# 101001000/ElevenRender

Hardware: AMD Instinct MI355X
Metric: Msamples/sec (rays traced x bounces) at 1920x1080, 1M-tri scene (higher is better)
Workload: dtype f32; 1 GPU; C2: 1000000-triangle random soup + 2048x1024 sky HDRI, 1920x1080, max_bounces 8, 1 step = 1 spp pass (config total 256 spp), seed 12345; schedule=stream

## Files before the change

### elevenrender_amd/abi.py

```python
import ctypes as C
import os

import numpy as np

_HERE = os.path.dirname(os.path.abspath(__file__))
LIB_PATH = os.environ.get("ELEVEN_HIP_LIB") or os.path.join(_HERE, "libeleven_hip.so")

ER_OK = 0
ER_ERR_INVALID_ARG, ER_ERR_NO_DEVICE, ER_ERR_HIP, ER_ERR_STATE, ER_ERR_OOM = -1, -2, -3, -4, -5
PASS_BEAUTY, PASS_DENOISE, PASS_NORMAL, PASS_TANGENT, PASS_BITANGENT, PASS_COUNT = 0, 1, 2, 3, 4, 5
PASS_NAMES = {"beauty": 0, "denoise": 1, "normal": 2, "tangent": 3, "bitangent": 4}
FLAG_POINT_LIGHTS, FLAG_COUNTERS, FLAG_MEGAKERNEL, FLAG_PROFILE, FLAG_FUSED, FLAG_WAVEFRONT, FLAG_GPU_BUILD, FLAG_MIS, FLAG_STREAM = 1, 2, 4, 8, 16, 32, 64, 128, 256
FLAG_HOST_BUILD = 512
FLAG_MESH_LIGHTS = 1024
MAX_BOUNCES = 65535
UPDATE_CAMERA, UPDATE_GEOMETRY = 1, 2
EDIT_CAMERA, EDIT_GEOMETRY, EDIT_MATERIALS, EDIT_TEXTURES, EDIT_HDRI = 1, 2, 4, 8, 16
REBUILD_NEVER, REBUILD_ALWAYS, REBUILD_AUTO = 0, 1, 2
TOPO_REMOVE, TOPO_APPEND = 1, 2
FEATURE_ALBEDO, FEATURE_DEPTH, FEATURE_COUNT = 0, 1, 2
FEATURE_NAMES = {"albedo": 0, "depth": 1}
ID_NONE, ID_SLOTS = 0xFFFFFFFF, 4
ID_TRIANGLE, ID_OBJECT, ID_MATERIAL, ID_KIND_COUNT = 0, 1, 2, 3
ID_KIND_NAMES = {"triangle": 0, "object": 1, "material": 2}
# ... 142 lines not shown

class ErAccelCost(C.Structure):
    _fields_ = [("node_area", C.c_double), ("leaf_area", C.c_double), ("tri_area", C.c_double), ("cost", C.c_double), ("ms", C.c_float), ("builder", C.c_uint32)]


class ErUpdatePolicy(C.Structure):
    _fields_ = [("mode", C.c_uint32), ("max_cost_ratio", C.c_float)]


class ErRebuildInfo(C.Structure):
    _fields_ = [("mode", C.c_uint32), ("max_cost_ratio", C.c_float), ("rebuilds", C.c_uint32), ("last_decision", C.c_uint32), ("cost_built", C.c_double),
                ("cost_refit", C.c_double), ("cost_after", C.c_double), ("cost_ms", C.c_float), ("rebuild_ms", C.c_float)]


class ErCostSumsDebug(C.Structure):
    _fields_ = [("node_area", C.c_double), ("leaf_area", C.c_double), ("tri_area", C.c_double), ("cost", C.c_double), ("ms", C.c_float), ("reserved", C.c_uint32)]


class ErTexEntry(C.Structure):
    _fields_ = [("width", C.c_int32), ("height", C.c_int32), ("channels", C.c_int32), ("filter", C.c_int32), ("offset", C.c_uint32)]


class ErTexturePlan(C.Structure):
    _fields_ = [("texture_count", C.c_uint32), ("fused_count", C.c_uint32), ("fused_any", C.c_uint32), ("reserved", C.c_uint32), ("hdri", ErTexEntry),
                ("pool_floats", C.c_uint64)]


class ErTextureDump(C.Structure):
    _fields_ = [("texture_count", C.c_uint32), ("material_count", C.c_uint32), ("fused_count", C.c_uint32), ("cdf_count", C.c_uint32), ("guide_count", C.c_uint32),
                ("tex_pow2", C.c_uint32), ("fused_any", C.c_uint32), ("hdri_buckets", C.c_int32), ("hdri_radiance_sum", C.c_float), ("hdri_tex", ErTexEntry),
                ("pool_floats", C.c_uint64)]


TEX_DTYPE = np.dtype([("width", "<i4"), ("height", "<i4"), ("channels", "<i4"), ("filter", "<i4"), ("offset", "<u4")])
FUSED_DTYPE = np.dtype([("width", "<i4"), ("height", "<i4"), ("filter", "<i4"), ("offset", "<u4")])
assert TEX_DTYPE.itemsize == 20 and FUSED_DTYPE.itemsize == 16


class ErFeatureInfo(C.Structure):
    _fields_ = [("valid", C.c_uint32), ("samples", C.c_uint32), ("rays", C.c_uint64), ("ms", C.c_float)]


class ErDenoiseGuided(C.Structure):
    _fields_ = [("levels", C.c_uint32), ("colour_sigma", C.c_float), ("albedo_sigma", C.c_float), ("depth_sigma", C.c_float)]


class ErIdInfo(C.Structure):
    _fields_ = [("valid", C.c_uint32), ("samples", C.c_uint32), ("rays", C.c_uint64), ("ms", C.c_float), ("objects", C.c_uint32),
                ("overflow_pixels", C.c_uint32 * ID_KIND_COUNT)]


class ErHistoryParams(C.Structure):
    _fields_ = [("depth_tolerance", C.c_float), ("max_weight", C.c_float)]


class ErHistoryInfo(C.Structure):
    _fields_ = [("captured", C.c_uint32), ("resolved", C.c_uint32), ("moved_objects", C.c_uint32), ("pixels_valid", C.c_uint64), ("pixels_partial", C.c_uint64),
                ("pixels_offscreen", C.c_uint64), ("pixels_rejected", C.c_uint64), ("pixels_sky", C.c_uint64), ("capture_ms", C.c_float), ("resolve_ms", C.c_float)]


class ErVarianceInfo(C.Structure):
    _fields_ = [("folds", C.c_uint32), ("reserved", C.c_uint32), ("pixels_folded", C.c_uint64), ("pixels_known", C.c_uint64), ("fold_ms", C.c_float),
                ("filter_ms", C.c_float)]


class ErDenoiseVariance(C.Structure):
    _fields_ = [("levels", C.c_uint32), ("colour_sigma", C.c_float), ("albedo_sigma", C.c_float), ("depth_sigma", C.c_float)]


class ErHistoryVarianceInfo(C.Structure):
    _fields_ = [("captured", C.c_uint32), ("resolved", C.c_uint32), ("pixels_known_captured", C.c_uint64), ("pixels_known_history", C.c_uint64),
                ("pixels_known_blended", C.c_uint64), ("filter_ms", C.c_float)]


class ErPick(C.Structure):
    _fields_ = [("hit", C.c_uint32), ("triangle", C.c_uint32), ("object", C.c_uint32), ("material", C.c_uint32), ("distance", C.c_float),
                ("position", C.c_float * 3), ("uv", C.c_float * 2)]


class ErStreamInfo(C.Structure):
    _fields_ = [("waves", C.c_uint32), ("tracers", C.c_uint32), ("large_regions", C.c_uint32), ("deal_pending", C.c_uint32), ("launches", C.c_uint32),
                ("pixels_per_cu", C.c_uint32), ("lanes_busy", C.c_double), ("launch_ms", C.c_double), ("cost_spread", C.c_double),
                ("spec_started", C.c_uint64), ("spec_right", C.c_uint64), ("spec_wrong", C.c_uint64),
                ("form", C.c_uint32), ("reserved", C.c_uint32)]


class ErStreamBalance(C.Structure):
    _fields_ = [("blocks", C.c_uint32), ("most", C.c_uint32), ("levelled", C.c_uint32), ("counting", C.c_uint32), ("cost_tiles", C.c_uint32), ("cap", C.c_uint32),
                ("launch_ticks", C.c_uint64)]


class ErStreamForm(C.Structure):
    _fields_ = [("waves", C.c_uint32), ("tracers", C.c_uint32), ("adapt", C.c_uint32), ("keep", C.c_uint32), ("spec", C.c_uint32), ("reserved", C.c_uint32)]


class ErAccelDump(C.Structure):
    _fields_ = [("tri_count", C.c_uint32), ("node_count", C.c_uint32), ("node8_count", C.c_uint32), ("node8_pieces", C.c_uint32),
                ("attr_pieces", C.c_uint32), ("max_depth", C.c_uint32), ("max_depth8", C.c_uint32), ("builder", C.c_uint32),
                ("lo", C.c_float * 3), ("hi", C.c_float * 3), ("lift_bound", C.c_float), ("max_lift", C.c_float)]


NODE_DTYPE = np.dtype([("lo0", "<f4", 3), ("hi0", "<f4", 3), ("lo1", "<f4", 3), ("hi1", "<f4", 3), ("c0", "<i4"), ("c1", "<i4"), ("pad", "<i4", 2)])
NODE8_DTYPE = np.dtype([("p", "<f4", 3), ("e", "u1", 3), ("imask", "u1"), ("child_base", "<u4"), ("tri_base", "<u4"), ("tri_present", "<u4"),
                        ("reserved", "<u4"), ("qlo", "u1", (3, 8)), ("qhi", "u1", (3, 8))])
ISECT_DTYPE = np.dtype([("v0", "<f4", 3), ("tri_id", "<i4"), ("v1", "<f4", 3), ("lift", "<f4"), ("v2", "<f4", 3), ("sign", "<f4")])
assert NODE_DTYPE.itemsize == 64 and NODE8_DTYPE.itemsize == 80 and ISECT_DTYPE.itemsize == 48


def attr_dtype(pieces):
    dt = np.dtype([("n", "<f4", (3, 3)), ("t", "<f4", (3, 3)), ("uv", "<f4", (3, 2)), ("material", "<i4"), ("pad", "<u4", 4 * pieces - 25)])
    assert dt.itemsize == 16 * pieces
    return dt


def accel_dump_dict(info, **arrays):
    d = {n: int(getattr(info, n)) for n in ("tri_count", "node_count", "node8_count", "max_depth", "max_depth8", "builder")}
    d["lo"], d["hi"] = np.array(list(info.lo), np.float32), np.array(list(info.hi), np.float32)
    d["lift_bound"], d["max_lift"] = np.float32(info.lift_bound), np.float32(info.max_lift)
    d.update(arrays)
    return d


def debug_bvh_dump(vertices, normals, threads=0):
    lib = load()
    v = np.ascontiguousarray(vertices, np.float32).reshape(-1, 3, 3)
    nn = np.ascontiguousarray(normals, np.float32).reshape(-1, 3, 3)
    assert v.shape == nn.shape
    n = len(v)
    info = ErAccelDump()
    args = (_fptr(v), _fptr(nn), n, threads, C.byref(info))
    check(lib.er_debug_bvh_dump(*args, None, 0, None, 0, None, 0, None, 0))
    assert info.node8_pieces * 16 == NODE8_DTYPE.itemsize
    nodes, nodes8 = np.zeros(info.node_count, NODE_DTYPE), np.zeros(info.node8_count, NODE8_DTYPE)
    s2t, lift = np.zeros(n, np.uint32), np.zeros(n, np.float32)
    vp = lambda a: a.ctypes.data_as(C.c_void_p)
    check(lib.er_debug_bvh_dump(*args, vp(nodes), nodes.nbytes, vp(nodes8), nodes8.nbytes, s2t.ctypes.data_as(C.POINTER(C.c_uint32)), s2t.nbytes,
                                _fptr(lift), lift.nbytes))
    return accel_dump_dict(info, nodes=nodes, nodes8=nodes8, slot_to_tri=s2t, tri_lift=lift)


def debug_spill_levels(spilled, n, usable):
    buf = np.ascontiguousarray(spilled, np.uint32)
    levels = np.zeros(n, np.uint32)
    check(load().er_debug_spill_levels(buf.ctypes.data_as(C.c_void_p), buf.nbytes, n, usable, levels.ctypes.data_as(C.POINTER(C.c_uint32))))
    return levels


def debug_transform_apply(m, vertices, normals, tangents):
    lib = load()
    mm = np.ascontiguousarray(m, np.float32).reshape(12)
    v, n, t = (np.ascontiguousarray(a, np.float32).reshape(-1, 3, 3) for a in (vertices, normals, tangents))
    assert v.shape == n.shape == t.shape
    out = [np.empty_like(v) for _ in range(3)]
    check(lib.er_debug_transform_apply(_fptr(mm), len(v), _fptr(v), _fptr(n), _fptr(t), *(_fptr(o) for o in out)))
    return tuple(out)


def debug_id_rank(ids):
    lib = load()
    a = np.ascontiguousarray(ids, np.uint32).reshape(-1)
    oi, oc, distinct = np.zeros(ID_SLOTS, np.uint32), np.zeros(ID_SLOTS, np.uint32), C.c_uint32()
    up = lambda x: x.ctypes.data_as(C.POINTER(C.c_uint32))
    check(lib.er_debug_id_rank(up(a) if a.size else None, a.size, up(oi), up(oc), C.byref(distinct)))
    return oi, oc, distinct.value


def debug_history_camera(camera):
# ... 461 lines not shown
```

### elevenrender_amd/csrc/er_api.cpp

```cpp
#include <algorithm>
#include <chrono>

#include "er_api_stages.h"
#include <thread>
#include <system_error>

using namespace erh;

int er_abi_version(void) { return ER_ABI_VERSION; }
const char* er_last_error(void) { return g_err.c_str(); }

int er_device_count(void) {
    int n = 0;
    if (hipGetDeviceCount(&n) != hipSuccess) return 0;
    return n;
}

static int er_device_info_impl(int index, ErDeviceInfo* out) {
    if (!out) return fail(ER_ERR_INVALID_ARG, "er_device_info: out is NULL");
    int n = er_device_count();
    if (index < 0 || index >= n) return fail(ER_ERR_NO_DEVICE, "er_device_info: no such HIP device");
    hipDeviceProp_t p;
    HIP_TRY(hipGetDeviceProperties(&p, index));
    memset(out, 0, sizeof(*out));
// ... 369 lines not shown

static int begin_planes(ErScene* s, BeginStaging& B) {
    int rc;
    const size_t npx = (size_t)s->x_res * s->y_res;
    if ((rc = upload(s->d_passes, nullptr, npx * ER_PASS_COUNT, s->stream)) != ER_OK) return rc;
    if ((rc = upload(s->d_samples, nullptr, npx, s->stream)) != ER_OK) return rc;
    if ((rc = upload(s->d_rng, nullptr, npx, s->stream)) != ER_OK) return rc;
    B.owned = s->tiles_of(s->params.rank, s->params.world);
    if ((rc = upload(s->d_owned, B.owned.data(), B.owned.size(), s->stream)) != ER_OK) return rc;
    if ((rc = upload(s->d_counters, nullptr, 1, s->stream)) != ER_OK) return rc;
    HIP_TRY(hipMemsetAsync(s->d_counters.p, 0, sizeof(DevCounters), s->stream));
    return ER_OK;
}

static int begin_choose_schedule(ErScene* s, BeginStaging& B, uint32_t cus) {
    const uint32_t all = ER_FLAG_MEGAKERNEL | ER_FLAG_FUSED | ER_FLAG_WAVEFRONT | ER_FLAG_STREAM;
    uint32_t forced = s->params.flags & all;
    if (forced == ER_FLAG_FUSED) forced = ER_FLAG_STREAM;
    if (forced & (forced - 1)) return fail(ER_ERR_INVALID_ARG, "er_render_begin: more than one schedule flag");
    uint32_t sched = forced;
    if (forced == 0 || forced == ER_FLAG_STREAM) B.deal = stream_deal_owned(B.owned, s->tiles_x(), cus);
    if (forced == 0) {
        sched = ((size_t)B.deal.most * 64u > ER_STREAM_MAX_RING || s->x_res > 65535u || s->y_res > 65535u) ? ER_FLAG_WAVEFRONT : ER_FLAG_STREAM;
    }
    s->params.flags = (s->params.flags & ~all) | sched;
    return ER_OK;
}

static int begin_wavefront(ErScene* s, const std::vector<uint32_t>& owned, uint32_t cus, bool query_on) {
    int rc;
    uint32_t pools = 3;
    if (const char* e = getenv("ER_WF_POOLS")) pools = (uint32_t)std::min(8, std::max(1, atoi(e)));
    pools = std::min<uint32_t>(pools, std::max<uint32_t>(1u, (uint32_t)owned.size()));
    const size_t pool_tiles = (owned.size() + pools - 1) / pools;
    const size_t qcap = pool_tiles * 64;
    size_t slots = owned.size() * 64;
    const size_t sh = query_on ? 2 : 1;
    const size_t qs_cap = qcap * sh;
    const size_t q_words = 2 * qcap + 2 * qs_cap;
    if ((rc = upload(s->d_wf4, nullptr, slots * (7 + 4 * sh), s->stream)) != ER_OK) return rc;
    if ((rc = upload(s->d_wf1, nullptr, slots * (3 + 3 * sh) + q_words * pools + (size_t)WF_COUNTS * pools, s->stream)) != ER_OK) return rc;
    WfState W{};
    float4* f = s->d_wf4.p;
    W.ray_o = f; W.ray_d = f + slots; W.light = f + 2 * slots; W.reduc = f + 3 * slots;
    W.aov_n = f + 4 * slots; W.aov_t = f + 5 * slots; W.aov_b = f + 6 * slots;
    W.sh_o = f + 7 * slots; W.sh_d = W.sh_o + sh * slots; W.c_vis = W.sh_d + sh * slots; W.c_occ = W.c_vis + sh * slots;
    uint32_t* u = s->d_wf1.p;
    W.hit = (int*)u; W.left = u + slots; W.hit2 = (int*)(u + 2 * slots);
    W.occluded = (int*)(u + 3 * slots); W.occ_a = W.occluded + sh * slots; W.occ_b = W.occ_a + sh * slots;
    uint32_t* qbase = u + (3 + 3 * sh) * slots;
    uint32_t* cbase = qbase + q_words * pools;
    W.pools = pools;
    W.slots = (uint32_t)slots;
    s->trace_blocks = cus * 12;
    s->shade_blocks = cus * 5;
    if (const char* e = getenv("ER_TRACE_WAVES_PER_CU")) s->trace_blocks = cus * (uint32_t)std::max(1, atoi(e));
    if (const char* e = getenv("ER_SHADE_WAVES_PER_CU")) s->shade_blocks = cus * (uint32_t)std::max(1, atoi(e));
    const size_t trace_spill = (size_t)s->trace_blocks * ER_STACK8 * 64;
    const size_t spill_per_pool = trace_spill + (size_t)s->shade_blocks * ER_BVH_MAX_DEPTH * 32;
    if ((rc = upload(s->d_spill, nullptr, spill_per_pool * pools, s->stream)) != ER_OK) return rc;
    s->wf.clear();
    for (uint32_t p2 = 0; p2 < pools; p2++) {
        W.pool = p2;
        uint32_t* q = qbase + (size_t)p2 * q_words;
        W.q[0] = q; W.q[1] = q + qcap; W.qs[0] = q + 2 * qcap; W.qs[1] = q + 2 * qcap + qs_cap;
        W.counts = cbase + (size_t)p2 * WF_COUNTS;
        W.spill = s->d_spill.p + (size_t)p2 * spill_per_pool;
        W.shade_stack = (int*)(W.spill + trace_spill);
        s->wf.push_back(W);
    }
    for (uint32_t p2 = 1; p2 < pools; p2++) {
        hipStream_t st;
        HIP_TRY(hipStreamCreateWithFlags(&st, hipStreamNonBlocking));
        s->pool_streams.push_back(st);
    }
    for (uint32_t p2 = 0; p2 < pools; p2++) {
        hipEvent_t e;
        HIP_TRY(hipEventCreateWithFlags(&e, hipEventDisableTiming));
        s->pool_events.push_back(e);
    }
    return ER_OK;
}

static int begin_descriptor(ErScene* s, uint32_t owned_tiles) {
    const ErGpuBvhDevice& g = s->kept.accel;
    const float lift_bound = g.lift_bound;
    float scene_scale = 0;
    for (int a = 0; a < 3; a++) scene_scale = std::max(scene_scale, std::max(std::fabs(g.lo[a]), std::fabs(g.hi[a])));
    scene_scale = std::max(scene_scale, std::max(std::fabs(s->camera.position.x), std::max(std::fabs(s->camera.position.y), std::fabs(s->camera.position.z))));

    DevScene& D = s->dev;
    memset(&D, 0, sizeof(D));
    D.nodes = s->d_nodes.p;
    D.nodes8 = s->d_nodes8.p;
    D.tri_isect = s->d_nodes8.p + g.n8_pieces;
    D.tri_base_pieces = (uint32_t)g.n8_pieces;
    D.tri_attr = s->d_attr.p;
    D.tri_count = s->tri_count;
    D.node_count = (uint32_t)(g.nodes_f4 / 4);
    D.node8_count = g.nodes8_count;
    D.prune_margin = lift_bound + 1e-5f * scene_scale;
    D.max_lift = lift_bound;
    D.scene_scale = scene_scale;
    D.materials = s->d_materials.p;
    D.mat_pre = s->d_mat_pre.p;
    D.textures = s->d_textures.p;
    D.tex_pool = s->d_tex_pool.p;
    D.mat_fused = s->d_mat_fused.p;
    D.fused_any = s->fused_any ? 1u : 0u;
    D.hdri_tex = s->kept.hdri;
    D.hdri_cdf = s->d_cdf.p;
    D.hdri_guide = s->d_guide.p;
    D.hdri_buckets = s->kept.buckets;
    D.hdri_radiance_sum = s->hdri_radiance_sum;
    D.hdri_trig = getenv("ER_HDRI_TRIG_ON_DEVICE") ? nullptr : s->d_guide.p + s->kept.trig_at;
    D.cam = s->camera;
    D.x_res = s->x_res;
    D.y_res = s->y_res;
    D.tiles_x = s->tiles_x();
    D.tiles_y = s->tiles_y();
    D.max_bounces = s->params.max_bounces;
    {
        auto pow2 = [](int32_t v) { return v > 0 && (v & (v - 1)) == 0; };
        bool all = pow2(s->kept.hdri.width) && pow2(s->kept.hdri.height);
        for (const HostTex& t : s->textures) all = all && pow2(t.width) && pow2(t.height);
        D.tex_pow2 = all ? 1u : 0u;
        if (const char* e = getenv("ER_TEX_POW2")) D.tex_pow2 = (atoi(e) != 0 && all) ? 1u : 0u;
    }
    D.trace_every_query = 0u;
    if (const char* e = getenv("ER_TRACE_EVERY_QUERY")) D.trace_every_query = atoi(e) != 0 ? 1u : 0u;
    D.ext_flags = s->params.flags & (ER_FLAG_POINT_LIGHTS | ER_FLAG_MIS);
    D.lights = s->d_lights.p;
    D.light_count = (uint32_t)s->point_lights.size();
    if (s->light_emitters > 0) {
        D.ext_flags = (D.ext_flags & ~(uint32_t)ER_FLAG_POINT_LIGHTS) | ER_FLAG_MESH_LIGHTS;
        D.mesh_lights = s->d_light_tab.p;
        D.emitter_count = s->light_emitters;
    }
    D.passes = s->d_passes.p;
    D.samples = s->d_samples.p;
    D.rng = s->d_rng.p;
    D.owned_tiles = s->d_owned.p;
    D.owned_tile_count = owned_tiles;
    D.counters = s->d_counters.p;
    D.tile_cost = ((s->params.flags & ER_FLAG_STREAM) && s->st.counting) ? s->st.d_tile_cost.p : nullptr;
    D.px_draws = (s->params.flags & ER_FLAG_STREAM) ? s->st.d_px_draws.p : nullptr;
    {
        const erd::CamTrig t = erd::camera_trig(D.cam);
        D.cam_cx = t.cx; D.cam_sx = t.sx; D.cam_cy = t.cy; D.cam_sy = t.sy; D.cam_cz = t.cz; D.cam_sz = t.sz;
        D.cam_trig_valid = getenv("ER_CAM_TRIG_ON_DEVICE") ? 0u : 1u;
    }
    return upload(s->d_dev, &D, 1, s->stream);
}

int begin_render_state(ErScene* s, BeginStaging& B, hipEvent_t uploads_done) {
    int rc;
    const uint32_t cus = s->kept.cus;
    const bool query_on = s->query_on();
    if ((rc = begin_planes(s, B)) != ER_OK) return rc;
    if ((rc = begin_choose_schedule(s, B, cus)) != ER_OK) return rc;
    if (s->params.flags & ER_FLAG_STREAM) rc = stream_begin(s, B.owned, B.deal, cus, query_on);
    else if (s->params.flags & ER_FLAG_WAVEFRONT) rc = begin_wavefront(s, B.owned, cus, query_on);
    if (rc != ER_OK) return rc;
    if (uploads_done) HIP_TRY(hipEventRecord(uploads_done, s->stream));
    if ((rc = begin_descriptor(s, (uint32_t)B.owned.size())) != ER_OK) return rc;

    er_launch_setup(s->dev, s->stream);
    HIP_TRY(hipGetLastError());
    HIP_TRY(hipStreamSynchronize(s->stream));
    return ER_OK;
}

}

static int er_render_begin_impl(ErScene* s, const ErRenderParams* p) {
    if (!s || !p) return fail(ER_ERR_INVALID_ARG, "er_render_begin: NULL argument");
    std::lock_guard<std::mutex> lk(s->mtx);
    int rc;
    ErDeviceInfo info;
    if ((rc = begin_check(p, info)) != ER_OK) return rc;
    if ((rc = begin_open(s, p)) != ER_OK) return rc;
    const char* who = "er_render_begin";
    s->kept.cus = std::max(1u, info.compute_units);
    s->kept.flags = p->flags;
    EventPair ev;
    HIP_TRY(hipEventCreate(&ev.a));
    HIP_TRY(hipEventCreate(&ev.b));
    BeginStaging B;
    if ((rc = begin_accel(s, B, ev.a, who)) != ER_OK) return rc;
    if ((rc = begin_materials(s, B)) != ER_OK) return rc;
    if ((rc = begin_textures(s, B, who)) != ER_OK) return rc;
    if ((rc = begin_emitters(s, B, who)) != ER_OK) return rc;
    if ((rc = begin_render_state(s, B, ev.b)) != ER_OK) return rc;
    float up_ms = 0;
    (void)hipEventElapsedTime(&up_ms, ev.a, ev.b);

    accel_publish(s, up_ms);
    s->begun = true;
    return ER_OK;
}

static int wavefront_enqueue(ErScene* s, const DevScene& D, uint32_t n, bool count) {
    const uint64_t iters64 = (uint64_t)n * ((uint64_t)s->params.max_bounces + 1u);
    if (iters64 > 0xFFFFFFFFull)
        return fail(ER_ERR_INVALID_ARG, "er_render_samples: " + std::to_string(n) + " samples of " + std::to_string(s->params.max_bounces) +
                                            " bounces are more than 4294967295 iterations of the wavefront schedule in one call");
    const uint32_t iters = (uint32_t)iters64;
    const uint32_t pools = (uint32_t)s->wf.size();
    const bool prof = (s->params.flags & ER_FLAG_PROFILE) != 0;
    if (prof) {
        const size_t need = s->prof_used / 3 + (size_t)iters * pools;
        while (s->prof_events.size() < 3 * need) {
            hipEvent_t e;
            HIP_TRY(hipEventCreate(&e));
            s->prof_events.push_back(e);
        }
        if (s->d_ray_log.n < need) {
            DevBuf<uint32_t> bigger;
            int rc2 = upload(bigger, nullptr, need * 2, s->stream);
            if (rc2 != ER_OK) return rc2;
            if (s->d_ray_log.p && s->prof_used) {
                HIP_TRY(hipStreamSynchronize(s->stream));
                HIP_TRY(hipMemcpy(bigger.p, s->d_ray_log.p, (s->prof_used / 3) * sizeof(uint32_t), hipMemcpyDeviceToDevice));
            }
            s->d_ray_log.release();
            s->d_ray_log = bigger;
        }
    }
    if (pools > 1) {
        HIP_TRY(hipEventRecord(s->pool_events[0], s->stream));
        for (uint32_t p = 1; p < pools; p++) HIP_TRY(hipStreamWaitEvent(s->pool_streams[p - 1], s->pool_events[0], 0));
    }
    auto pool_stream = [&](uint32_t p) { return p == 0 ? s->stream : s->pool_streams[p - 1]; };
    for (uint32_t p = 0; p < pools; p++) er_launch_wf_begin(D, s->wf[p], n, pool_stream(p));
    for (uint32_t it = 0; it < iters; it++) {
        for (uint32_t p = 0; p < pools; p++) {
            hipStream_t st = pool_stream(p);
            uint32_t* ray_log = prof ? s->d_ray_log.p + s->prof_used / 3 : nullptr;
            if (prof) HIP_TRY(hipEventRecord(s->prof_events[s->prof_used++], st));
            er_launch_wf_trace(D, s->wf[p], it & 1, count, s->trace_blocks, ray_log, st);
            if (prof) HIP_TRY(hipEventRecord(s->prof_events[s->prof_used++], st));
            er_launch_wf_shade(D, s->wf[p], it & 1, count, s->shade_blocks, st);
            if (prof) HIP_TRY(hipEventRecord(s->prof_events[s->prof_used++], st));
        }
    }
    for (uint32_t p = 1; p < pools; p++) {
        HIP_TRY(hipEventRecord(s->pool_events[p], s->pool_streams[p - 1]));
        HIP_TRY(hipStreamWaitEvent(s->stream, s->pool_events[p], 0));
    }
    return ER_OK;
}

static int enqueue_samples(ErScene* s, uint32_t n) {
    const DevScene& D = s->ad_on ? s->ad_dev : s->dev;
    const bool count = (s->params.flags & ER_FLAG_COUNTERS) != 0;
    int rc = ER_OK;
    if (!(s->params.flags & (ER_FLAG_MEGAKERNEL | ER_FLAG_STREAM))) {
        if (n > 0) rc = wavefront_enqueue(s, D, n, count);
    } else {
        const bool prof = (s->params.flags & ER_FLAG_PROFILE) && n > 0;
        if (prof) {
            while (s->prof_events.size() < s->prof_used + 3) {
                hipEvent_t e;
                HIP_TRY(hipEventCreate(&e));
                s->prof_events.push_back(e);
            }
            HIP_TRY(hipEventRecord(s->prof_events[s->prof_used++], s->stream));
// ... 481 lines not shown
```

### elevenrender_amd/csrc/er_api_edit.cpp

```cpp
#include <algorithm>
#include <chrono>

#include "er_api_stages.h"
#include "er_topology_host.h"

using namespace erh;

static_assert(ER_TOPO_REMOVE == ER_TOPO_HOST_REMOVE && ER_TOPO_APPEND == ER_TOPO_HOST_APPEND, "er_topology_host.h restates the two bits");

static_assert(ER_EDIT_CAMERA == ER_UPDATE_CAMERA && ER_EDIT_GEOMETRY == ER_UPDATE_GEOMETRY, "an ErSceneUpdate's bits are the first two of an ErSceneEdit");

namespace {

const uint32_t LOOK_BITS = ER_EDIT_MATERIALS | ER_EDIT_TEXTURES | ER_EDIT_HDRI;

struct XformList {
    uint32_t count = 0;
    const ErObjectTransform* x = nullptr;
    std::vector<ErXformEntry> entries;
    uint32_t moved = 0;
};


int edit_refit(ErScene* s, bool new_normals, bool new_tangents, const ErSparseList* sp, const XformList* xf, const char* who) {
// ... 284 lines not shown
                continue;
            }
            if ((rc = check_tex(t, "scene texture")) != ER_OK) return rc;
        }
    }
    const ErMaterial* mats = s->materials.data();
    size_t nmat = s->materials.size();
    bool ids_differ = false;
    if (what & ER_EDIT_MATERIALS) {
        if (e->material_count == 0 || !e->materials) return fail(ER_ERR_INVALID_ARG, pre + "ER_EDIT_MATERIALS needs at least one material");
        mats = e->materials;
        nmat = e->material_count;
        if ((rc = check_texture_ids(mats, nmat, ntex, who)) != ER_OK) return rc;
        if (tc) rc = topo_check_material_ids(s, e->material_id, true, *tc, nmat, who);
        else rc = check_material_ids(e->material_id ? e->material_id : s->material_id.data(), n, nmat, who);
        if (rc != ER_OK) return rc;
        ids_differ = nmat != s->materials.size();
        for (size_t m = 0; m < nmat && !ids_differ; m++) {
            int32_t a[7], b[7];
            texture_ids(mats[m], a);
            texture_ids(s->materials[m], b);
            ids_differ = memcmp(a, b, sizeof(a)) != 0;
        }
    }
    if (tc && !(what & ER_EDIT_MATERIALS) && (rc = topo_check_material_ids(s, nullptr, false, *tc, nmat, who)) != ER_OK) return rc;
    if ((what & ER_EDIT_HDRI) && (rc = check_tex(e->hdri.texture, "hdri")) != ER_OK) return rc;
    W.rebuild_pool = (what & ER_EDIT_TEXTURES) != 0 || ids_differ;
    {
        const TexDecl hd = (what & ER_EDIT_HDRI) ? TexDecl{e->hdri.texture.width, e->hdri.texture.height, e->hdri.texture.channels, e->hdri.texture.filter}
                                                 : TexDecl{s->hdri_tex.width, s->hdri_tex.height, s->hdri_tex.channels, s->hdri_tex.filter};
        uint64_t pool_floats = 0;
        if (W.rebuild_pool) {
            std::vector<TexDecl> decl(ntex);
            for (size_t i = 0; i < ntex; i++) {
                const bool keep = !(what & ER_EDIT_TEXTURES) || !e->textures[i].data;
                decl[i] = keep ? TexDecl{s->textures[i].width, s->textures[i].height, s->textures[i].channels, s->textures[i].filter}
                               : TexDecl{e->textures[i].width, e->textures[i].height, e->textures[i].channels, e->textures[i].filter};
            }
            TexPlan P;
            er_texture_plan(decl.data(), ntex, mats, nmat, hd, P);
            pool_floats = P.pool_floats;
        } else if (what & ER_EDIT_HDRI) {
            pool_floats = (uint64_t)s->kept.hdri.offset + (uint64_t)hd.width * (uint64_t)hd.height * (uint64_t)hd.channels;
        }
        if ((rc = check_pool_floats(pool_floats, who)) != ER_OK) return rc;
    }
    if (what & ER_EDIT_MATERIALS) W.materials.assign(e->materials, e->materials + e->material_count);
    if (what & ER_EDIT_TEXTURES) {
        W.textures.resize(ntex);
        W.kept.assign(ntex, 0);
        for (size_t i = 0; i < ntex; i++) {
            if (!e->textures[i].data) { W.kept[i] = 1; continue; }
            if ((rc = copy_tex(e->textures[i], W.textures[i], "scene texture")) != ER_OK) return rc;
        }
    }
    if (what & ER_EDIT_HDRI) {
        if ((rc = copy_tex(e->hdri.texture, W.hdri, "hdri")) != ER_OK) return rc;
        if (e->hdri.cdf) {
            W.cdf.assign(e->hdri.cdf, e->hdri.cdf + (size_t)W.hdri.width * W.hdri.height + 1);
            W.radiance_sum = e->hdri.radiance_sum;
        } else {
            host_generate_cdf(W.hdri, W.cdf, W.radiance_sum);
        }
    }
    return ER_OK;
}

void edit_replace(ErScene* s, const ErSceneEdit* e, const ErSparseList* sp, const XformList* xf, EditWork& W) noexcept {
    const uint32_t what = e->what;
    const size_t n = s->tri_count, n9 = n * 9;
    if (what & ER_EDIT_CAMERA) s->camera = e->camera;
    if ((what & ER_EDIT_GEOMETRY) && sp) {
        s->flush_poses();
        er_sparse_patch(*sp, s->vertices.data(), s->normals.data(), s->tangents.data());
    } else if ((what & ER_EDIT_GEOMETRY) && xf) {
        er_objects_mark(s->objects, xf->entries.data(), (uint32_t)xf->entries.size());
    } else if (what & ER_EDIT_GEOMETRY) {
        if (e->normals && e->tangents) s->objects.forget_pending();
        else s->flush_poses();
        std::copy(e->vertices, e->vertices + n9, s->vertices.begin());
        if (e->normals) std::copy(e->normals, e->normals + n9, s->normals.begin());
        if (e->tangents) std::copy(e->tangents, e->tangents + n9, s->tangents.begin());
    }
    if (what & ER_EDIT_MATERIALS) {
        s->materials.swap(W.materials);
        if (e->material_id) std::copy(e->material_id, e->material_id + n, s->material_id.begin());
    }
    if (what & ER_EDIT_TEXTURES) {
        for (size_t i = 0; i < W.textures.size(); i++)
            if (W.kept[i]) std::swap(W.textures[i], s->textures[i]);
        s->textures.swap(W.textures);
    }
    if (what & ER_EDIT_HDRI) {
        std::swap(s->hdri_tex, W.hdri);
        s->hdri_cdf.swap(W.cdf);
        s->hdri_radiance_sum = W.radiance_sum;
    }
}

int edit_locked(ErScene* s, const ErSceneEdit* e, const ErSparseList* sp, XformList* xf, uint32_t known, const char* who, std::chrono::steady_clock::time_point t0) {
    int rc;
    EditWork W;
    if ((rc = edit_check(s, e, sp, xf, known, who, W)) != ER_OK) return rc;
    HIP_TRY(hipSetDevice(s->device));
    HIP_TRY(hipStreamSynchronize(s->stream));
    edit_replace(s, e, sp, xf, W);
    if ((e->what & ER_EDIT_GEOMETRY) || ((e->what & ER_EDIT_MATERIALS) && e->material_id)) s->store.release();
    s->feat.valid = false;
    for (auto& set : s->unpacked_feat) set.clear();
    s->ids_invalidate();
    if (((e->what & ER_EDIT_GEOMETRY) && !xf) || (e->what & LOOK_BITS)) s->history_invalidate();
    s->variance_reset();
    uint32_t stage = 0;
    float stage_ms = 0;
    const bool sparse_geometry = sp && (e->what & ER_EDIT_GEOMETRY);
    if (sparse_geometry) {
        const uint32_t calls = s->sparse.calls;
        s->sparse = ErSparseInfo{};
        s->sparse.calls = calls;
    }
    const bool xform_geometry = xf && (e->what & ER_EDIT_GEOMETRY);
    if (xform_geometry) {
        const uint32_t calls = s->xform.calls;
        s->xform = ErSparseInfo{};
        s->xform.calls = calls;
    }
    if ((rc = edit_device(s, e, sp, xf, W.rebuild_pool, who, stage, stage_ms)) != ER_OK) {
        s->begun = false;
        return rc;
    }
    s->upd.updates++;
    if (sparse_geometry) {
        s->sparse.calls++;
        s->sparse.moved = sp->count;
        if (s->accel.builder != 2u) s->sparse.path = 3u;
    }
    if (xform_geometry) {
        s->xform.calls++;
        s->xform.moved = xf->moved;
        s->xform_objects = xf->count;
        if (s->accel.builder != 2u) s->xform.path = 3u;
    }
    if ((e->what & ER_EDIT_GEOMETRY) && s->accel.builder == 2u) s->upd.refits++;
    const float wall_ms = std::chrono::duration<float, std::milli>(std::chrono::steady_clock::now() - t0).count();
    if (e->what & LOOK_BITS) {
        s->edit.edits++;
        s->edit.texture_stage = stage;
        s->edit.texture_stage_ms = stage_ms;
        s->edit.pool_floats = s->d_tex_pool.n;
        s->edit.edit_ms = wall_ms;
    } else {
        s->upd.update_ms = wall_ms;
    }
    return ER_OK;
}

}

static int er_render_update_impl(ErScene* s, const ErSceneUpdate* u) {
    if (!s || !u) return fail(ER_ERR_INVALID_ARG, "er_render_update: NULL argument");
    const auto t0 = std::chrono::steady_clock::now();
    std::lock_guard<std::mutex> lk(s->mtx);
    if (!s->begun) return fail(ER_ERR_STATE, "er_render_update: er_render_begin has not succeeded");
    ErSceneEdit e{};
    e.what = u->what; e.camera = u->camera; e.vertices = u->vertices; e.normals = u->normals; e.tangents = u->tangents;
    return edit_locked(s, &e, nullptr, nullptr, ER_UPDATE_CAMERA | ER_UPDATE_GEOMETRY, "er_render_update", t0);
// ... 263 lines not shown
```

### elevenrender_amd/csrc/er_bounce.inc

```
#ifndef ER_BOUNCE_FUSE
#define ER_BOUNCE_FUSE true
#endif
#ifndef ER_BOUNCE_SKIP_EQUAL
#define ER_BOUNCE_SKIP_EQUAL true
#endif
#ifndef ER_BOUNCE_KEEP_LAST
#define ER_BOUNCE_KEEP_LAST false
#endif
{
    const bool er_skip_equal = (ER_BOUNCE_SKIP_EQUAL) && S.trace_every_query == 0u;
    const int hw = S.hdri_tex.width, hh = S.hdri_tex.height;
    const bool er_mis = EXT && (S.ext_flags & ER_FLAG_MIS) != 0;
#ifdef ER_BOUNCE_MESH
    constexpr bool er_mesh = EXT && (ER_BOUNCE_MESH);
#else
    constexpr bool er_mesh = false;
#endif
    if (hslot < 0) {
        float u, v;
        spherical_mapping(-1 * ray.d, u, v);
        if (EXT) {
            F3 er_env = tex_filtered(S, S.hdri_tex, u, v);
            if (er_mis && prev_pdf >= 0.0f) {
                const int er_mx = ermath::f2i(u * hw), er_my = ermath::f2i(v * hh);
                const float er_ms = (S.hdri_trig != nullptr && (unsigned)er_my < (unsigned)hh) ? hdri_trig_rows(S)[er_my].sin_row : hdri_pdf_sine(S.hdri_tex, er_my);
                const float er_ph = hdri_pdf_of(S, tex_coords(S, S.hdri_tex, er_mx, er_my), er_ms);
                er_env = er_env * (1.0f / (1.0f + er_ph / prev_pdf));
                if (COUNT) c_texels++;
            }
            light = light + reduction * er_env;
        } else {
            light = light + reduction * tex_filtered(S, S.hdri_tex, u, v);
        }
        if (COUNT) c_texels++;
        done = true;
    } else {
        c_shaded++;
        ER_TP(2);
        HitFull hit;
        full_hit(S, (uint32_t)hslot, ray, hit);
        const ErMaterial& mat = S.materials[hit.material];
        HitData hd;
        generate_hit_data<COUNT, ER_BOUNCE_FUSE>(S, mat, hit, hd, c_texels);
        int shader = mat.albedo_shader_id;
        if (shader != -1) {
            hd.albedo = f3s(0);
            if (shader >= 0 && shader < 4) hd.albedo = f3(1, 1, 0);
        }
        if (rng_next(rs) <= hd.opacity) {
            F3 wo = ray.d * -1.0f;
            F3 N = hd.normal;
            c_hdri++;
            ER_TP(3);
            int count = er_cdf_search(S.hdri_cdf, hw * hh, S.hdri_guide, S.hdri_buckets, rng_next(rs));
            const bool hw_pow2 = (hw & (hw - 1)) == 0 && hw > 0 && count >= 0;
            const int er_cx = hw_pow2 ? (int)((unsigned)count & (unsigned)(hw - 1)) : count % hw;
            const int er_cy = hw_pow2 ? (int)((unsigned)count >> (31 - __builtin_clz((unsigned)hw))) : count / hw;
            float tcx = (float)er_cx, tcy = (float)er_cy;
            float d1 = rng_next(rs), d2 = rng_next(rs), d3 = rng_next(rs);
            const bool er_lights = EXT && !er_mesh && (S.ext_flags & ER_FLAG_POINT_LIGHTS) != 0 && S.light_count > 0;
            float er_rl = 0.0f;
            if (er_lights) er_rl = rng_next(rs);
            float er_mp = 0.0f, er_mu1 = 0.0f, er_mu2 = 0.0f;
            if (er_mesh) { er_mp = rng_next(rs); er_mu1 = rng_next(rs); er_mu2 = rng_next(rs); }
            ER_TP(4);
            const bool er_last = !(ER_BOUNCE_KEEP_LAST) && bounce + 1u >= S.max_bounces;
            F3 wibrdf = f3s(0);
            if (!er_last) wibrdf = DisneySample(hd, wo, N, d1, d2, d3);
            float er_px, er_pz, er_py, er_a, er_sin;
            int er_ix, er_iy;
            if (S.hdri_trig != nullptr && (unsigned)count < (unsigned)(hw * hh)) {
                const HdriCol er_c = hdri_trig_cols(S)[er_cx];
                const HdriRow er_r = hdri_trig_rows(S)[er_cy];
                er_px = er_c.px; er_pz = er_c.pz; er_ix = er_c.ix;
                er_py = er_r.py; er_a = er_r.a; er_iy = er_r.iy; er_sin = er_r.sin_pdf;
            } else {
                float nu = tcx / (float)hw, nv = tcy / (float)hh;
                float iu, iv;
                inverse_transform_uv(S.hdri_tex, nu, nv, iu, iv);
                rsm_column(iu, er_px, er_pz);
                rsm_row(iv, er_py, er_a);
                er_ix = ermath::f2i(iu * hw); er_iy = ermath::f2i(iv * hh);
                er_sin = hdri_pdf_sine(S.hdri_tex, er_iy);
            }
            F3 wihdri = normalized(f3(er_a * er_px, er_py, er_a * er_pz)) * -1.0f;
            F3 hdriValue = tex_coords(S, S.hdri_tex, er_ix, er_iy);
            if (COUNT) c_texels += 2;
            F3 evalh = DisneyEval(hd, wo, N, wihdri);
            float hdripdf = hdri_pdf_of(S, hdriValue, er_sin);
            float absdot = __builtin_fabsf(dot(wihdri, N));
            float er_wnee = 1.0f;
            if (er_mis) er_wnee = 1.0f / (1.0f + DisneyPdf(hd, wo, N, wihdri) / hdripdf);
            F3 er_em = hd.emission;
            if (er_mesh && prev_pdf >= 0.0f && mesh_d >= 0.0f) {
                const float er_ph = mesh_prob(S)[hslot];
                if (er_ph > 0.0f) {
                    F3 er_a, er_b, er_c, er_ng;
                    float er_area;
                    mesh_tri(S, (uint32_t)hslot, er_a, er_b, er_c, er_ng, er_area);
                    const float er_dh = mesh_d + length(hit.position - ray.o);
                    const float er_pl = er_ph * (er_dh * er_dh) / (er_area * __builtin_fabsf(dot(er_ng, ray.d)));
                    er_em = er_em * (1.0f / (1.0f + er_pl / prev_pdf));
                }
            }
            F3 c_vis = er_mis ? reduction * (er_em + (hdriValue * evalh * absdot / hdripdf) * er_wnee)
                              : reduction * (er_em + hdriValue * evalh * absdot / hdripdf);
            const F3 c_occ = er_mis ? reduction * (er_em + (f3s(0) * evalh * absdot / hdripdf) * er_wnee)
                                    : reduction * (er_em + f3s(0) * evalh * absdot / hdripdf);
            if ((evalh.x != 0.0f || evalh.y != 0.0f || evalh.z != 0.0f) && !(er_skip_equal && same_bits(c_vis, c_occ))) {
                Ray sr = make_ray(hd.position + N * 0.001f, wihdri);
                F3 v0, v1, v2;
                float4 qa, qb, qc4;
                load_verts(S, (uint32_t)hslot, v0, v1, v2, qa, qb, qc4);
                float su, sv, st, d_self = __builtin_inff();
                if (tri_mt(v0, v1, v2, sr, su, sv, st)) d_self = candidate_distance(S, (uint32_t)hslot, v0, v1, v2, sr, su, sv, st);
                ER_BOUNCE_HDRI_QUERY(sr, hslot, d_self, c_vis, c_occ);
                pending = true;
            } else {
                light = light + c_vis;
            }
            if (er_lights) {
                int er_k = ermath::f2i((float)S.light_count * er_rl);
                er_k = er_k > (int)S.light_count - 1 ? (int)S.light_count - 1 : er_k;
                const ErPointLight er_L = S.lights[er_k];
                const F3 er_lpos = f3(er_L.position.x, er_L.position.y, er_L.position.z);
                const F3 er_toL = er_lpos - hd.position;
                const F3 er_dir = normalized(er_toL);
                const float er_dist = length(er_toL);
                const Ray er_lr = make_ray(hd.position + er_dir * 0.001f, er_dir);
                const float er_limit = length(er_lpos - er_lr.o);
                const F3 er_value = f3(er_L.radiance.x, er_L.radiance.y, er_L.radiance.z) / (er_dist * er_dist);
                const F3 er_evall = DisneyEval(hd, wo, N, er_dir);
                const float er_lpdf = ((float)S.light_count) / (2.0f * PIF);
                if (er_evall.x != 0.0f || er_evall.y != 0.0f || er_evall.z != 0.0f) {
                    const F3 er_pl = er_value * er_evall * __builtin_fabsf(dot(er_dir, N)) / er_lpdf;
                    const F3 er_lv = reduction * er_pl, er_lo = reduction * f3s(0);
                    if (er_skip_equal && !pending && same_bits(er_lv, er_lo)) {
                        light = light + er_lv;
                    } else {
                        ER_BOUNCE_LIGHT_QUERY(er_lr, -1, er_limit, er_lv, er_lo);
                        lpending = true;
                    }
                }
            }
            if (er_mesh && bounce + 1u < S.max_bounces) {
                const uint32_t er_k = mesh_slot(S, mesh_pick(S, er_mp));
                if ((int)er_k != hslot) {
                    F3 er_a, er_b, er_c, er_ng;
                    float er_area;
                    mesh_tri(S, er_k, er_a, er_b, er_c, er_ng, er_area);
                    const float er_su = __builtin_sqrtf(er_mu1);
                    const float er_b1 = er_su * (1.0f - er_mu2), er_b2 = er_su * er_mu2;
                    const F3 er_p = er_a * (1.0f - er_su) + er_b * er_b1 + er_c * er_b2;
                    const F3 er_toL = er_p - hd.position;
                    const F3 er_dir = normalized(er_toL);
                    const float er_dist = length(er_toL);
                    const float er_cosl = dot(er_ng, er_dir);
                    const F3 er_evall = er_cosl != 0.0f ? DisneyEval(hd, wo, N, er_dir) : f3s(0);
                    if (er_evall.x != 0.0f || er_evall.y != 0.0f || er_evall.z != 0.0f) {
                        const float4* er_q = S.tri_attr + (size_t)er_k * ER_ATTR_PIECES;
                        const float4 er_q4 = er_q[4], er_q5 = er_q[5];
                        const ErMaterial& er_m = S.materials[__builtin_bit_cast(int, er_q[6].x)];
                        const float er_tu = er_q4.z + (er_q5.x - er_q4.z) * er_b1 + (er_q5.z - er_q4.z) * er_b2;
                        const float er_tv = er_q4.w + (er_q5.y - er_q4.w) * er_b1 + (er_q5.w - er_q4.w) * er_b2;
                        F3 er_le = er_m.emission_tex < 0 ? f3(er_m.emission.x, er_m.emission.y, er_m.emission.z)
                                                         : tex_filtered(S, S.textures[er_m.emission_tex], er_tu, er_tv);
                        const float er_op = er_m.opacity_tex < 0 ? er_m.opacity : tex_filtered(S, S.textures[er_m.opacity_tex], er_tu, er_tv).x;
                        er_le = er_le * clampf(er_op, 0.0f, 1.0f);
                        if (COUNT) c_texels += (er_m.emission_tex < 0 ? 0 : 1) + (er_m.opacity_tex < 0 ? 0 : 1);
                        const float er_lpdf = mesh_prob(S)[er_k] * (er_dist * er_dist) / (er_area * __builtin_fabsf(er_cosl));
                        const float er_wl = 1.0f / (1.0f + DisneyPdf(hd, wo, N, er_dir) / er_lpdf);
                        const F3 er_ml = er_le * er_evall * __builtin_fabsf(dot(er_dir, N)) / er_lpdf * er_wl;
                        const F3 er_lv = reduction * er_ml, er_lo = reduction * f3s(0);
                        if (er_skip_equal && !pending && same_bits(er_lv, er_lo)) {
                            light = light + er_lv;
                        } else {
                            const Ray er_lr = make_ray(hd.position + er_dir * 0.001f, er_dir);
                            ER_BOUNCE_LIGHT_QUERY(er_lr, (int)er_k, length(er_p - er_lr.o), er_lv, er_lo);
                            lpending = true;
                        }
                    }
                }
            }
            ER_TP(5);
            if (!er_last) {
                float brdfpdf = DisneyPdf(hd, wo, N, wibrdf);
                reduction = reduction * (DisneyEval(hd, wo, N, wibrdf) * __builtin_fabsf(dot(wibrdf, N)) / brdfpdf);
                if (er_mis || er_mesh) prev_pdf = brdfpdf;
                ray = make_ray(hit.position + wibrdf * 0.001f, wibrdf);
            }
            if (bounce == 0) { ER_BOUNCE_FIRST_HIT(hd.normal, hd.tangent, hd.bitangent); }
            if (er_mesh) mesh_d = 0.001f;
        } else {
            if (er_mesh) mesh_d = -1.0f;
            ray = make_ray(hit.position + ray.d * 0.001f, ray.d);
        }
        ER_TP(6);
        bounce++;
        if (bounce >= S.max_bounces) done = true;
    }
}
```

### elevenrender_amd/csrc/er_debug.hip

```cpp
#include "er_debug.h"

#include "er_device.h"
#include "er_shade.h"
#include "er_trav.h"

using namespace erd;

__global__ __launch_bounds__(64) void er_debug_trace_kernel(DevScene S, const float* __restrict__ o, const float* __restrict__ d, uint32_t n,
                                                             const int32_t* __restrict__ self, const float* __restrict__ limit,
                                                             int32_t* __restrict__ tri_out, int32_t* __restrict__ slot_out, float* __restrict__ pos_out,
                                                             float* __restrict__ dist_out, int32_t* __restrict__ info_out, uint2* spill_base) {
    __shared__ uint2 s_stack[WF_LDS_STACK * 64];
    __shared__ int s_stack2[ER_STACK * 64];
    const uint32_t i = blockIdx.x * 64 + threadIdx.x;
    if (i >= n) return;
    uint2* stack = s_stack + threadIdx.x;
    uint2* spill = spill_base + (size_t)blockIdx.x * (ER_STACK8 * 64) + threadIdx.x;
    int* stack2 = s_stack2 + threadIdx.x;
    Ray ray;
    ray.o = f3(o[3 * i], o[3 * i + 1], o[3 * i + 2]);
    ray.d = f3(d[3 * i], d[3 * i + 1], d[3 * i + 2]);
    unsigned cn = 0, ct = 0;
    int info = 0;
    if (self) {
// ... 9 lines not shown
        pos_out[3 * i] = pos_out[3 * i + 1] = pos_out[3 * i + 2] = 0.0f;
        dist_out[i] = __builtin_inff();
        if (slot >= 0) {
            HitFull h;
            full_hit(S, (uint32_t)slot, ray, h);
            tri_out[i] = __builtin_bit_cast(int, S.tri_isect[(size_t)slot * 3].w);
            pos_out[3 * i] = h.position.x; pos_out[3 * i + 1] = h.position.y; pos_out[3 * i + 2] = h.position.z;
            dist_out[i] = length(h.position - ray.o);
        }
    }
    info_out[i] = info;
}

void er_launch_debug_trace(const DevScene& S, const float* o, const float* d, uint32_t n, const int32_t* self, const float* limit, int32_t* tri,
                           int32_t* slot, float* pos, float* dist, int32_t* info, void* spill, hipStream_t stream) {
    if (n == 0) return;
    hipLaunchKernelGGL(er_debug_trace_kernel, dim3((n + 63) / 64), dim3(64), 0, stream, S, o, d, n, self, limit, tri, slot, pos, dist, info, (uint2*)spill);
}
uint32_t er_debug_lds_stack_levels() { return WF_LDS_STACK; }

template <bool EXT, bool MESH>
__global__ __launch_bounds__(64) void er_debug_pixel_kernel(DevScene S, uint32_t idx, ErTraceRec* recs, int max_recs, int* count, uint2* spill) {
    __shared__ uint2 sh_stack[WF_LDS_STACK * 64];
    uint2* s_stack = sh_stack;
    int* s_stack2 = (int*)(spill + (size_t)ER_STACK8 * 64);
    static_assert((size_t)ER_STACK8 * 64 + ((size_t)ER_STACK * 64 * sizeof(int) + sizeof(uint2) - 1) / sizeof(uint2) <= (size_t)ER_DEBUG_PIXEL_SCRATCH,
                  "er_debug_trace_pixel's scratch must hold the spill levels and the exact routine's int stack");
    if (threadIdx.x != 0) return;
    int nrec = 0;
    unsigned c_rays = 0, c_nodes = 0, c_tris = 0, c_shaded = 0, c_texels = 0, c_hdri = 0;
    uint32_t rs = S.rng[idx];
    const uint32_t px = idx % S.x_res, py = idx / S.x_res;
    float c1 = rng_next(rs), c2 = rng_next(rs), c3 = rng_next(rs), c4 = rng_next(rs), c5 = rng_next(rs);
    Ray ray = camera_ray(S.cam, (int)px, (int)py, S.x_res, S.y_res, c1, c2, c3, c4, c5);
    F3 light = f3s(0), reduction = f3s(1), aov_n = f3s(0), aov_t = f3s(0), aov_b = f3s(0);
    uint32_t bounce = 0;
    float prev_pdf = -1.0f;
    float mesh_d = 0.0f;
    while (true) {
        int info;
        c_rays++;
        const int hslot = trav_run_closest<false>(S, s_stack, spill, s_stack2, ray, __builtin_inff(), info, c_nodes, c_tris);
        ErTraceRec* rec = nrec < max_recs ? &recs[nrec++] : nullptr;
        if (rec) {
            rec->bounce = (int32_t)bounce;
            rec->tri = hslot < 0 ? -1 : __builtin_bit_cast(int, S.tri_isect[(size_t)hslot * 3].w);
            rec->shadow_tri = -1; rec->opaque = 0; rec->shadow_occ = -1; rec->light_occ = -1;
            for (int k = 0; k < 3; k++) { rec->position[k] = 0; rec->wi[k] = 0; }
            if (hslot >= 0) {
                HitFull h;
                full_hit(S, (uint32_t)hslot, ray, h);
                rec->position[0] = h.position.x; rec->position[1] = h.position.y; rec->position[2] = h.position.z;
            }
        }
        constexpr bool COUNT = false;
        const Ray traced = ray;
        const uint32_t rs_before = rs;
        bool done = false, pending = false, lpending = false;
#define ER_BOUNCE_HDRI_QUERY(sr, self_slot, d_self, cv, co)                                                                          \
    {                                                                                                                                 \
        int info_;                                                                                                                    \
        c_rays++;                                                                                                                     \
        const bool occ_ = trav_run_shadow<false>(S, s_stack, spill, s_stack2, (sr), (self_slot), (d_self), info_, c_nodes, c_tris);   \
        light = light + (occ_ ? (co) : (cv));                                                                                         \
        if (rec) {                                                                                                                    \
            rec->shadow_occ = occ_ ? 1 : 0;                                                                                           \
                                      \
            const int cs_ = trav_run_closest<false>(S, s_stack, spill, s_stack2, (sr), __builtin_inff(), info_, c_nodes, c_tris);     \
            rec->shadow_tri = cs_ < 0 ? -1 : __builtin_bit_cast(int, S.tri_isect[(size_t)cs_ * 3].w);                                 \
        }                                                                                                                             \
    }
#define ER_BOUNCE_LIGHT_QUERY(lr, self_slot, limit, lv, lo)                                                                          \
    {                                                                                                                                 \
        int info_;                                                                                                                    \
        c_rays++;                                                                                                                     \
        const bool occ_ = trav_run_shadow<false>(S, s_stack, spill, s_stack2, (lr), (self_slot), (limit), info_, c_nodes, c_tris);    \
        light = light + (occ_ ? (lo) : (lv));                                                                                         \
        if (rec) rec->light_occ = occ_ ? 1 : 0;                                                                                       \
    }
#define ER_BOUNCE_FIRST_HIT(n, t, b) aov_n = (n); aov_t = (t); aov_b = (b)
#define ER_BOUNCE_MESH MESH
#define ER_BOUNCE_SKIP_EQUAL false
#define ER_BOUNCE_KEEP_LAST true
#include "er_bounce.inc"
#undef ER_BOUNCE_HDRI_QUERY
#undef ER_BOUNCE_LIGHT_QUERY
#undef ER_BOUNCE_FIRST_HIT
#undef ER_BOUNCE_MESH
#undef ER_BOUNCE_SKIP_EQUAL
#undef ER_BOUNCE_KEEP_LAST
        (void)pending; (void)lpending; (void)traced;
        if (rec) {
            uint32_t r1 = rs_before;
            (void)rng_next(r1);
            rec->opaque = (hslot >= 0 && rs != r1) ? 1 : 0;
            if (hslot >= 0) { rec->wi[0] = ray.d.x; rec->wi[1] = ray.d.y; rec->wi[2] = ray.d.z; }
            rec->light[0] = light.x; rec->light[1] = light.y; rec->light[2] = light.z;
            rec->reduction[0] = reduction.x; rec->reduction[1] = reduction.y; rec->reduction[2] = reduction.z;
        }
        if (done) break;
    }
    const uint32_t sa = S.samples[idx];
    const uint32_t sa2 = accumulate_sample(S, idx, sa, light, aov_n, aov_t, aov_b);
    if (sa2 != sa) S.samples[idx] = sa2;
    S.rng[idx] = rs;
    *count = nrec;
    atomicAdd(&S.counters->paths, 1ull);
    atomicAdd(&S.counters->bounce_samples, (unsigned long long)(bounce + (bounce < S.max_bounces ? 1u : 0u)));
    atomicAdd(&S.counters->rays, (unsigned long long)c_rays);
    atomicAdd(&S.counters->shaded_hits, (unsigned long long)c_shaded);
    atomicAdd(&S.counters->hdri_samples, (unsigned long long)c_hdri);
}

void er_launch_debug_pixel(const DevScene& S, uint32_t idx, ErTraceRec* recs, int max_recs, int* count, void* spill, hipStream_t stream) {
    auto k = er_mesh_active(S) ? er_debug_pixel_kernel<true, true> : er_ext_active(S) ? er_debug_pixel_kernel<true, false> : er_debug_pixel_kernel<false, false>;
    hipLaunchKernelGGL(k, dim3(1), dim3(64), 0, stream, S, idx, recs, max_recs, count, (uint2*)spill);
}

namespace {
ERD HitData hd_from(const float* h) {
    HitData d;
    d.metallic = h[0]; d.roughness = h[1]; d.clearcoatGloss = h[2]; d.clearcoat = h[3]; d.anisotropic = h[4];
    d.transmission = h[5]; d.specular = h[6]; d.specularTint = h[7]; d.sheenTint = h[8]; d.subsurface = h[9];
    d.sheen = h[10]; d.opacity = 1.0f;
    d.albedo = f3(h[11], h[12], h[13]); d.tangent = f3(h[14], h[15], h[16]); d.bitangent = f3(h[17], h[18], h[19]);
    d.emission = f3s(0); d.position = f3s(0); d.normal = f3s(0);
    d.gtr1_log = __builtin_nanf("");
    return d;
}
}

__global__ __launch_bounds__(64) void er_debug_eval_kernel(DevScene S, int kind, const float* __restrict__ in, uint32_t n, uint32_t in_stride,
                                                           float* __restrict__ out, uint32_t out_stride) {
    const uint32_t i = blockIdx.x * 64 + threadIdx.x;
    if (i >= n) return;
    const float* a = in + (size_t)i * in_stride;
    float* o = out + (size_t)i * out_stride;
    auto bits = [](float f) { return __builtin_bit_cast(int, f); };
    auto fbits = [](uint32_t u) { return __builtin_bit_cast(float, u); };
    switch (kind) {
        case ER_FN_RNG: {
            uint32_t st = jenkins_u32((uint32_t)bits(a[0]) + 1u);
            for (int k = 0; k < 16; k++) { o[k] = rng_next(st); o[16 + k] = fbits(st); }
            break;
        }
        case ER_FN_CAMERA_RAY: {
            const Ray r = camera_ray(S.cam, (int)a[0], (int)a[1], S.x_res, S.y_res, a[2], a[3], a[4], a[5], a[6]);
            o[0] = r.o.x; o[1] = r.o.y; o[2] = r.o.z; o[3] = r.d.x; o[4] = r.d.y; o[5] = r.d.z;
            break;
        }
        case ER_FN_TRI_HIT: {
            const int id = bits(a[0]);
            int slot = -1;
            for (uint32_t s = 0; s < S.tri_count; s++)
                if (__builtin_bit_cast(int, S.tri_isect[(size_t)s * 3].w) == id) { slot = (int)s; break; }
            Ray ray;
            ray.o = f3(a[1], a[2], a[3]);
            ray.d = f3(a[4], a[5], a[6]);
            for (int k = 0; k < 18; k++) o[k] = 0.0f;
            if (slot < 0) break;
            F3 v0, v1, v2;
            float4 qa, qb, qc;
            load_verts(S, (uint32_t)slot, v0, v1, v2, qa, qb, qc);
            float u, v, t;
            if (!tri_mt(v0, v1, v2, ray, u, v, t)) break;
            HitFull h;
            full_hit(S, (uint32_t)slot, ray, h);
            o[0] = 1.0f;
            const F3 vs[5] = {h.position, h.normal, h.gnormal, h.tangent, h.bitangent};
            for (int k = 0; k < 5; k++) { o[1 + 3 * k] = vs[k].x; o[2 + 3 * k] = vs[k].y; o[3 + 3 * k] = vs[k].z; }
            o[16] = h.tu; o[17] = h.tv;
            break;
        }
// ... 88 lines not shown
```

### elevenrender_amd/csrc/er_device.h

```cpp
#pragma once
#include <hip/hip_runtime.h>
#include <stdint.h>

#include "../../include/eleven_hip.h"
#include "er_bvh.h"
#include "er_cdf.h"
#include "er_math.h"

#ifdef ER_ISA_MARKS
#define ER_MARK(name) asm volatile("; ER_MARK " name ::: "memory")
#else
#define ER_MARK(name) ((void)0)
#endif

#ifndef ER_TP
#define ER_TP(n) ((void)0)
#endif

#define ER_TILE 8
#define ER_STACK ER_BVH_MAX_DEPTH

struct DevTex {
    int32_t width, height, channels, filter;
    uint32_t offset;
};

struct DevFused {
    int32_t width, height, filter;
    uint32_t offset;
};

struct DevCounters {
    unsigned long long paths, bounce_samples, rays, node_visits, tri_tests, shaded_hits, texel_fetches, hdri_samples;
    unsigned long long trace_wave_steps, trace_busy_lanes, trace_node_lanes, trace_tri_lanes;
};

struct DevScene {
    const float4* nodes;
    const float4* nodes8;
    const float4* tri_isect;
    const float4* tri_attr;
    uint32_t tri_count, node_count;
    uint32_t node8_count;
    uint32_t tri_base_pieces;
    float prune_margin;
    float max_lift, scene_scale;
    const ErMaterial* materials;
    const float4* mat_pre;
    const DevTex* textures;
    const DevFused* mat_fused;
    uint32_t fused_any;
    const float* tex_pool;
    DevTex hdri_tex;
    const float* hdri_cdf;
    const uint32_t* hdri_guide;
    int32_t hdri_buckets;
    float hdri_radiance_sum;
    ErCamera cam;
    uint32_t x_res, y_res, tiles_x, tiles_y;
    uint32_t max_bounces;
    uint32_t tex_pow2;
    float cam_cx, cam_sx, cam_cy, cam_sy, cam_cz, cam_sz;
    uint32_t cam_trig_valid;
    uint32_t trace_every_query;
    uint32_t ext_flags;
    union { const ErPointLight* lights; const float* mesh_lights; };
    union { uint32_t light_count; uint32_t emitter_count; };
    float4* passes;
    uint32_t* samples;
    uint32_t* rng;
    const uint32_t* owned_tiles;
    uint32_t owned_tile_count;
    DevCounters* counters;
    uint32_t* tile_cost;
    uint32_t* px_draws;
    const uint32_t* hdri_trig;
};

__host__ __device__ __forceinline__ size_t er_pass_index(size_t npx, int pass, size_t idx) {
    return pass == ER_PASS_DENOISE ? 4 * npx + idx : idx * 4 + (size_t)(pass == ER_PASS_BEAUTY ? 0 : pass - 1);
}


namespace erd {

#define ERD __device__ __forceinline__

const float PIF = 3.14159265358979323846f;

struct F3 { float x, y, z; };
ERD F3 f3(float x, float y, float z) { F3 r; r.x = x; r.y = y; r.z = z; return r; }
ERD F3 f3s(float s) { return f3(s, s, s); }
ERD F3 operator+(F3 a, F3 b) { return f3(a.x + b.x, a.y + b.y, a.z + b.z); }
ERD F3 operator-(F3 a, F3 b) { return f3(a.x - b.x, a.y - b.y, a.z - b.z); }
ERD F3 operator*(F3 a, float s) { return f3(a.x * s, a.y * s, a.z * s); }
ERD F3 operator*(float s, F3 a) { return f3(a.x * s, a.y * s, a.z * s); }
ERD F3 operator/(F3 a, float s) { return f3(a.x / s, a.y / s, a.z / s); }
ERD F3 operator*(F3 a, F3 b) { return f3(b.x * a.x, b.y * a.y, b.z * a.z); }
ERD bool same_bits(F3 a, F3 b) {
    return ((__builtin_bit_cast(uint32_t, a.x) ^ __builtin_bit_cast(uint32_t, b.x)) | (__builtin_bit_cast(uint32_t, a.y) ^ __builtin_bit_cast(uint32_t, b.y)) |
            (__builtin_bit_cast(uint32_t, a.z) ^ __builtin_bit_cast(uint32_t, b.z))) == 0u;
}
ERD F3 addf(F3 a, float s) { return f3(a.x + s, a.y + s, a.z + s); }
ERD float dot(F3 a, F3 b) { return a.x * b.x + a.y * b.y + a.z * b.z; }
ERD F3 cross(F3 a, F3 b) {
    return f3((a.y * b.z - a.z * b.y), -(a.x * b.z - a.z * b.x), (a.x * b.y - a.y * b.x));
}
ERD float length(F3 a) { return __builtin_sqrtf(a.x * a.x + a.y * a.y + a.z * a.z); }
ERD F3 normalized(F3 a) {
    float l = length(a);
    if (l == 0) return a;
    return a / l;
}
ERD float clampf(float a, float b, float c) { return a < b ? b : a > c ? c : a; }
ERD float lerpf(float a, float b, float c) { return a + c * (b - a); }
ERD F3 lerpv(F3 a, F3 b, float c) { return f3(lerpf(a.x, b.x, c), lerpf(a.y, b.y, c), lerpf(a.z, b.z, c)); }
ERD float minf(float a, float b) { return a < b ? a : b; }
ERD float maxf(float a, float b) { return a > b ? a : b; }
__host__ __device__ __forceinline__ void limitUV(float& u, float& v) {
    u += (float)(-(int)(u > 1) + -(int)(u < 0));
    v += (float)(-(int)(v > 1) + -(int)(v < 0));
}

struct Ray { F3 o, d; };
ERD Ray make_ray(F3 o, F3 d) {
    Ray r;
    r.o = o;
    float l = length(d);
    if (l != 0) { d.x /= l; d.y /= l; d.z /= l; }
    r.d = d;
    return r;
}

ERD uint32_t jenkins_u32(uint32_t seed) {
    uint32_t hash = 0;
#pragma unroll
    for (int i = 0; i < 4; i++) {
        hash += (seed >> (i * 8)) & 0xFF;
        hash += (hash << 10);
        hash ^= (hash >> 6);
    }
    hash += (hash << 3);
    hash ^= (hash >> 11);
    hash += (hash << 15);
    return hash;
}
ERD float rng_next(uint32_t& state) {
    state ^= state << 13;
    state ^= state >> 17;
    state ^= state << 5;
    return (float)state / 4294967296.0f;
}

struct CamTrig { float cx, sx, cy, sy, cz, sz; };
__host__ __device__ inline CamTrig camera_trig(const ErCamera& cam) {
    using namespace ermath;
    const float k = 3.14159265358979323846f / 180.0f;
    const float rx = cam.rotation.x * k, ry = cam.rotation.y * k, rz = cam.rotation.z * k;
    CamTrig t;
// ... 526 lines not shown
```

### elevenrender_amd/csrc/er_scene.h

```cpp
#pragma once
#include <hip/hip_runtime.h>

#include <atomic>
#include <cmath>
#include <cstdio>
#include <cstdlib>
#include <cstring>
#include <map>
#include <set>
#include <memory>
#include <mutex>
#include <new>
#include <string>
#include <vector>

#include "../../include/eleven_hip.h"
#include "er_bvh.h"
#include "er_devbuf.h"
#include "er_device.h"
#include "er_gpu_build.h"
#include "er_kernels.h"
#include "er_wavefront.h"
#include "er_stream.h"
#include "er_stream_host.h"
// ... 30 lines not shown
    } catch (...) {
        return fail(ER_ERR_STATE, std::string(who) + ": unknown exception");
    }
}

inline std::atomic<uint64_t> g_host_alloc_limit{0};
inline void host_reserve(uint64_t bytes) {
    const uint64_t lim = g_host_alloc_limit.load();
    if (lim && bytes > lim) throw std::bad_alloc();
}

struct EventPair {
    hipEvent_t a = nullptr, b = nullptr;
    ~EventPair() {
        if (a) (void)hipEventDestroy(a);
        if (b) (void)hipEventDestroy(b);
    }
};

#define HIP_TRY(expr)                                                                                   \
    do {                                                                                                \
        hipError_t e__ = (expr);                                                                        \
        if (e__ != hipSuccess)                                                                          \
            return fail(e__ == hipErrorOutOfMemory ? ER_ERR_OOM : ER_ERR_HIP,                           \
                        std::string(#expr) + ": " + hipGetErrorString(e__));                            \
    } while (0)

struct HostTex {
    int32_t width, height, channels, filter;
    std::vector<float> data;
};

inline void host_tex_coords(const HostTex& t, int x, int y, float out[3]) {
    x %= t.width;
    y %= t.height;
    if (x < 0) x *= -1;
    if (y < 0) y *= -1;
    out[0] = out[1] = out[2] = 0.0f;
    const float* d = t.data.data();
    if (t.channels == 1) {
        out[0] = out[1] = out[2] = d[y * t.width + x];
    } else if (t.channels == 2) {
        out[0] = d[t.channels * (y * t.width + x) + 0];
        out[1] = d[t.channels * (y * t.width + x) + 1];
    } else if (t.channels >= 3) {
        out[0] = d[t.channels * (y * t.width + x) + 0];
        out[1] = d[t.channels * (y * t.width + x) + 1];
        out[2] = d[t.channels * (y * t.width + x) + 2];
    }
}

inline void host_generate_cdf(const HostTex& t, std::vector<float>& cdf, float& radianceSum) {
    int c = 0;
    radianceSum = 0;
    cdf.assign((size_t)t.width * t.height + 1, 0.0f);
    float p[3];
    for (int j = 0; j < t.height; j++)
        for (int i = 0; i < t.width; i++) {
            host_tex_coords(t, i, j, p);
            radianceSum += p[0] + p[1] + p[2];
        }
    for (int j = 0; j < t.height; j++)
        for (int i = 0; i < t.width; i++) {
            host_tex_coords(t, i, j, p);
            cdf[c + 1] = cdf[c] + (p[0] + p[1] + p[2]) / radianceSum;
            c++;
        }
}

}

using erh::DevBuf;
using erh::HostTex;

struct ErScene {
    uint32_t tri_count = 0;
    std::vector<float> vertices, normals, tangents, uvs, tangent_sign;
    std::vector<int32_t> material_id;
    std::vector<ErMaterial> materials;
    std::vector<HostTex> textures;
    HostTex hdri_tex;
    std::vector<float> hdri_cdf;
    float hdri_radiance_sum = 0;
    ErCamera camera;
    std::vector<ErPointLight> point_lights;
    uint32_t x_res = 0, y_res = 0;

    bool begun = false;
    int device = 0;
    ErRenderParams params{};
    hipStream_t stream = nullptr;
    hipEvent_t ev_start = nullptr, ev_stop = nullptr;
    bool timing_open = false;
    DevScene dev{};
    ErAccelInfo accel{};
    float accel_lo[3] = {0, 0, 0}, accel_hi[3] = {0, 0, 0};
    uint32_t accel_depth2 = 0;
    struct Kept {
        ErGpuBvhDevice accel;
        DevTex hdri{};
        int buckets = 0;
        size_t trig_at = 0;
        uint32_t cus = 0, flags = 0;
    } kept;
    ErRefitTopo refit_topo;
    ErUpdateInfo upd{};
    ErEditInfo edit{};
    ErSparseInfo sparse{};
    ErObjectTable objects;
    ErXformDev xform_dev;
    ErSparseInfo xform{};
    uint32_t xform_objects = 0;
    ErGeomStore store;
    ErTopologyInfo topo{};
    void flush_poses() noexcept { er_objects_flush(objects, vertices.data(), normals.data(), tangents.data()); }
    uint64_t accel_version = 0, cost_version = ~0ull;
    ErAccelCost cost_kept{};
    bool baseline_known = false;
    double baseline_cost = 0;
    ErUpdatePolicy policy{ER_REBUILD_NEVER, 0.0f};
    ErRebuildInfo rebuild{};
    size_t tex_pool_cap = 0;
    DevBuf<float4> d_nodes, d_nodes8, d_attr, d_passes;
    DevBuf<float4> d_plane;
    DevBuf<ErMaterial> d_materials;
    DevBuf<float4> d_mat_pre;
    DevBuf<ErPointLight> d_lights;
    DevBuf<float> d_light_tab;
    uint32_t light_emitters = 0;
    float light_total = 0.0f;
    DevBuf<DevTex> d_textures;
    DevBuf<float> d_tex_pool, d_cdf;
    DevBuf<uint32_t> d_samples, d_rng, d_owned;
    DevBuf<DevCounters> d_counters;
    std::vector<uint8_t> tex_mode;
    bool fused_any = false;
    DevBuf<DevFused> d_mat_fused;
    DevBuf<DevScene> d_dev;
    DevBuf<float4> d_wf4;
    DevBuf<uint32_t> d_wf1;
    DevBuf<uint2> d_spill;
    DevBuf<uint32_t> d_guide;
    StreamHost st;
    uint32_t rendered = 0;
    bool ad_on = false;
    float ad_threshold = 0;
    uint32_t ad_interval = 0, ad_next = 0, ad_tests = 0, ad_cur = 0;
    bool ad_snapped = false;
    float ad_max_error = -1.0f;
    uint64_t ad_pixel_samples = 0, ad_active_px = 0;
    std::vector<uint32_t> ad_active, ad_tile_samples;
    DevBuf<uint32_t> d_ad_list[2], d_ad_keep;
    DevBuf<float4> d_ad_snap;
    DevBuf<float> d_ad_err;
    DevScene ad_dev{};
    std::vector<WfState> wf;
    std::vector<hipStream_t> pool_streams;
    std::vector<hipEvent_t> pool_events;

    uint32_t trace_blocks = 0, shade_blocks = 0;
    std::vector<hipEvent_t> prof_events;
    DevBuf<uint32_t> d_ray_log;
    size_t prof_used = 0;
    ErProfile profile{};
    std::map<uint32_t, DevBuf<uint32_t>> d_rank_tiles;
    DevBuf<float4> d_gather_mine;
// ... 144 lines not shown
```

### elevenrender_amd/csrc/er_stream.h

```cpp
#pragma once
#include <hip/hip_runtime_api.h>
#include <stddef.h>
#include <stdint.h>

#include <vector>

struct DevScene;

#ifndef ER_STREAM_SLOTS
#define ER_STREAM_SLOTS 1024u
#endif

#ifndef ER_STREAM_SUPER_TILE_DEFAULT
#define ER_STREAM_SUPER_TILE_DEFAULT 8u
#endif
#ifndef ER_STREAM_SUPER_TILE_LARGE
#define ER_STREAM_SUPER_TILE_LARGE 16u
#endif
#ifndef ER_STREAM_COST_SPREAD_MAX
#define ER_STREAM_COST_SPREAD_MAX 0.04
#endif
#ifndef ER_STREAM_ADAPT_MIN_MS
#define ER_STREAM_ADAPT_MIN_MS 4.0
#endif
#ifndef ER_STREAM_SMALL_SHARE
#define ER_STREAM_SMALL_SHARE 1152u
#endif
#ifndef ER_STREAM_TEN_TRACERS_SHARE
#define ER_STREAM_TEN_TRACERS_SHARE 704u
#endif
#ifndef ER_STREAM_SPEC_SHARE
#define ER_STREAM_SPEC_SHARE 2304u
#endif
#ifndef ER_STREAM_SPEC_MIN_TRIS
#define ER_STREAM_SPEC_MIN_TRIS 1000u
#endif
#ifndef ER_STREAM_SPEC_LONG_DEFAULT
#define ER_STREAM_SPEC_LONG_DEFAULT 12
#endif
#ifndef ER_STREAM_KEEP_SHARE
#define ER_STREAM_KEEP_SHARE 6000u
#endif
#ifndef ER_STREAM_SPEC_KEEP_DEFAULT
#define ER_STREAM_SPEC_KEEP_DEFAULT 2
#endif
#define ER_STREAM_MAX_RING 32768u

enum ErStreamCtl : uint32_t {
    ER_SC_STATUS = 0,
    ER_SC_ITERS = 1,
    ER_SC_BUSY = 3,
    ER_SC_START = 5,
    ER_SC_END = 7,
    ER_SC_SPEC = 23,
    ER_SC_WORDS = 26,
    ER_SC_WG_END = 27
};
constexpr uint32_t ER_STREAM_CTL_LEAD = 1;
static_assert((ER_STREAM_CTL_LEAD + ER_SC_ITERS) % 2u == 0u && ER_SC_BUSY % 2u == 1u && ER_SC_START % 2u == 1u && ER_SC_END % 2u == 1u && ER_SC_WG_END % 2u == 1u && ER_SC_WG_END >= ER_SC_WORDS,
              "the 64-bit control words are 8-byte aligned");
constexpr uint32_t er_stream_ctl_words(uint32_t blocks) { return ER_SC_WG_END + 2u * blocks; }

struct ErStreamLaunch {
    const DevScene* S = nullptr;
    const DevScene* S_dev = nullptr;
    void* records = nullptr;
    uint32_t slots = 0;
    bool lights = false;
    void* spill = nullptr;
    const uint32_t* deal = nullptr;
    uint32_t deal_count = 0;
    void* ring = nullptr;
    uint32_t ring_cap = 0;
    uint32_t* status = nullptr;
    uint32_t n_samples = 0;
    bool count = false;
    uint32_t blocks = 0;
    uint32_t tracers = 0;
    uint32_t waves = 16;
    bool spec = false;
    bool keep = false;
    hipStream_t stream = nullptr;
};
void er_launch_stream_mesh(const ErStreamLaunch& L);
void er_launch_stream(const ErStreamLaunch& L);
struct ErStreamLaunchForm { uint32_t form, waves, bits; };
ErStreamLaunchForm er_stream_launch_form(uint32_t max_bounces, uint32_t tri_count, uint32_t waves, bool spec, bool keep);
uint32_t er_stream_deal_tiles(const uint32_t* owned, uint32_t count, uint32_t tiles_x, uint32_t blocks, bool xcd_aware, std::vector<uint32_t>& out, uint32_t edge = 0);
uint32_t er_stream_level_by_cost(const std::vector<uint32_t>& deal, uint32_t tiles_x, uint32_t blocks, const uint32_t* cost, size_t cost_n, uint32_t cap, std::vector<uint32_t>& out);
uint32_t er_stream_record_bytes(bool lights);
size_t er_stream_spill_entries(uint32_t blocks);
hipError_t er_probe_stream(const char** which);
```

### elevenrender_amd/csrc/er_stream.hip

```cpp
#include <algorithm>
#include <cstdlib>
#include "er_device.h"
#include "er_kernels.h"
#include "er_wavefront.h"
#include "er_trav.h"
#include "er_shade.h"
#include "er_stream.h"
#include "er_ring.h"

using namespace erd;

#ifdef ER_TIME_PROBE
#define ER_TPS(n)                                                                                       \
    {                                                                                                    \
        const unsigned long long tp_now = __builtin_amdgcn_s_memtime();                                  \
        if (tp_sec < 10u && (threadIdx.x & 63) == 0) atomicAdd(&s_tp[tp_sec], (unsigned)((tp_now - tp_last) >> 4)); \
        tp_last = tp_now;                                                                                \
        tp_sec = (n);                                                                                    \
    }
#undef ER_TP
#define ER_TP(n) ER_TPS(n)
#else
#define ER_TPS(n) ((void)0)
#endif

#ifdef ER_STAGE_PROBE
#define ER_SP(x) x
__device__ __forceinline__ uint32_t sp_now() { return (uint32_t)wall_clock64(); }
__device__ __forceinline__ void sp_add(unsigned long long* c, uint32_t d) { atomicAdd(c, (unsigned long long)d); }
#else
#define ER_SP(x)
#endif

#ifdef ER_TRACER_PROBE
#define ER_TRP(i)                                                           \
    {                                                                       \
        const unsigned long long trp_now = __builtin_amdgcn_s_memtime();    \
        trp[i] += (uint32_t)(trp_now - trp_last);                           \
        trp_last = trp_now;                                                 \
    }
#else
#define ER_TRP(i) ((void)0)
#endif

namespace {

#define ST_SLOT_BITS 11
static_assert(ER_STREAM_SLOTS <= (1u << ST_SLOT_BITS) && ST_SLOT_BITS + 2 <= ER_RING_PAYLOAD_BITS, "a local slot must fit the ring payload");
#define ST_SLOT_MASK ((1u << ST_SLOT_BITS) - 1u)
#define ST_FIN 0x100u
#define ST_ESC 0x200u
#define ST_AMB1 0x400u
#define ST_AMB2 0x800u
#ifndef ER_STREAM_LDS_HANDOFF
#define ER_STREAM_LDS_HANDOFF 1
#endif
#define ST_OCC1 0x1000u
#define ST_OCC2 0x2000u
#define ST_HIT2 0x4000u
#define ST_COUNT_MASK 0xFFu
static_assert((ST_COUNT_MASK & (ST_FIN | ST_ESC | ST_AMB1 | ST_AMB2 | ST_OCC1 | ST_OCC2 | ST_HIT2)) == 0u &&
                  (ST_FIN ^ ST_ESC ^ ST_AMB1 ^ ST_AMB2 ^ ST_OCC1 ^ ST_OCC2 ^ ST_HIT2) == (ST_FIN | ST_ESC | ST_AMB1 | ST_AMB2 | ST_OCC1 | ST_OCC2 | ST_HIT2) &&
                  (ST_FIN & (ST_FIN - 1u)) == 0u && (ST_ESC & (ST_ESC - 1u)) == 0u && (ST_AMB1 & (ST_AMB1 - 1u)) == 0u && (ST_AMB2 & (ST_AMB2 - 1u)) == 0u &&
                  (ST_OCC1 & (ST_OCC1 - 1u)) == 0u && (ST_OCC2 & (ST_OCC2 - 1u)) == 0u && (ST_HIT2 & (ST_HIT2 - 1u)) == 0u,
              "the fields of a slot's s_wait word are single bits that overlap neither each other nor the in-flight count");
#define ST_RQ_LOG2 (ER_STREAM_SLOTS > 1024u ? 13u : 12u)
#define ST_SQ_LOG2 (ER_STREAM_SLOTS > 1024u ? 11u : 10u)
static_assert((1u << ST_SQ_LOG2) >= ER_STREAM_SLOTS, "the shade ring must hold every slot once");
static_assert((1u << ST_RQ_LOG2) >= ER_STREAM_SLOTS && (1u << ST_RQ_LOG2) >= 4u * 192u, "ray ring too small");
static_assert((1u << ST_RQ_LOG2) >= 3u * ER_STREAM_SLOTS, "the ray ring must hold three rays per slot");
#ifndef ER_STREAM_SPLIT_WAIT
#define ER_STREAM_SPLIT_WAIT 1
#endif
#ifndef ER_SHADER_PRIO
#define ER_SHADER_PRIO 1
#endif
#ifndef ER_TRACER_PRIO
#define ER_TRACER_PRIO 0
#endif
#ifndef ER_STREAM_TOP_NODES
#define ER_STREAM_TOP_NODES 900
#endif
#ifndef ER_STREAM_TOP_NODES_SPEC_CUT
#define ER_STREAM_TOP_NODES_SPEC_CUT (ER_STREAM_LDS_HANDOFF ? 40 : 0)
#endif
#ifndef ST_MAX_TRACERS
#define ST_MAX_TRACERS 13
#endif
enum { C_LIVE = 0, C_DONE, C_INIT, C_WORDS };
#ifndef ST_IDLE_SLEEP
#define ST_IDLE_SLEEP 16
#endif
#ifndef ST_BATCH_SLEEP
#define ST_BATCH_SLEEP 8
#endif
#define ST_WATCHDOG 300000u
#define ST_ERR_PIXEL 4u
#define ST_ERR_SHADE 8u
#define ST_ERR_RAY 16u
#define ST_ERR_CTX 32u
#define ST_PXBITS_WORDS (ER_STREAM_MAX_RING / 32u)

__device__ __forceinline__ uint32_t st_reserve(uint32_t* counter, bool want) {
    const unsigned long long mask = __ballot(want);
    if (mask == 0) return 0;
    const unsigned lane = threadIdx.x & 63;
    const unsigned leader = __ffsll((long long)mask) - 1;
    uint32_t base = 0;
    if (lane == leader) base = atomicAdd(counter, (uint32_t)__popcll(mask));
    base = (uint32_t)__builtin_amdgcn_readlane((int)base, (int)leader);
    return base + (uint32_t)__popcll(mask & ((1ull << lane) - 1ull));
}

__device__ __forceinline__ uint32_t st_rank(unsigned long long m) {
    return __builtin_amdgcn_mbcnt_hi((uint32_t)(m >> 32), __builtin_amdgcn_mbcnt_lo((uint32_t)m, 0u));
}

template <uint32_t LOG2>
__device__ __forceinline__ void st_push(uint32_t* cells, uint32_t* ctl, bool want, uint32_t payload, uint32_t* status, uint32_t err) {
    const unsigned long long m = __ballot(want);
    if (m == 0) return;
    const unsigned lane = threadIdx.x & 63;
    const uint32_t n = (uint32_t)__popcll(m);
    uint32_t base = 0;
    if (lane == 0) base = er_ring_reserve(ctl, n);
    base = (uint32_t)__builtin_amdgcn_readlane((int)base, 0);
    if (want && !er_ring_put(cells, LOG2, base + st_rank(m), payload)) atomicOr(status, err);
    if (lane == 0) er_ring_publish(ctl, n);
}

__device__ __forceinline__ uint32_t st_take(uint32_t* ctl, uint32_t want, uint32_t& base, unsigned long long seen) {
    uint32_t granted = 0, hb = 0;
    if ((threadIdx.x & 63) == 0 && want > 0) granted = er_ring_grant(ctl, want, hb, seen);
    base = (uint32_t)__builtin_amdgcn_readlane((int)hb, 0);
    return (uint32_t)__builtin_amdgcn_readlane((int)granted, 0);
}

#define ST_STRIDE_PLAIN 256u
#define ST_STRIDE_LIGHTS 384u
struct StState {
    char* base;
    uint2* spill;
    uint32_t slots, stride;
    template <class T, uint32_t OFF, uint32_t LOFF>
    __device__ __forceinline__ T& fld2(uint32_t i) const {
        const bool l = i >= slots;
        return *(T*)(base + (size_t)((l ? i - slots : i) * stride + (l ? LOFF : OFF)));
    }
    template <class T, uint32_t OFF>
    __device__ __forceinline__ T& fld(uint32_t i) const { return *(T*)(base + (size_t)(i * stride + OFF)); }
    __device__ __forceinline__ float4& ray_o(uint32_t i) const { return fld<float4, 0>(i); }
    __device__ __forceinline__ float4& ray_d(uint32_t i) const { return fld<float4, 16>(i); }
    __device__ __forceinline__ float4& sh_o(uint32_t i) const { return fld2<float4, 32, 256>(i); }
    __device__ __forceinline__ float4& sh_d(uint32_t i) const { return fld2<float4, 48, 272>(i); }
    __device__ __forceinline__ int& hit(uint32_t i) const { return fld<int, 64>(i); }
    __device__ __forceinline__ int& hit2(uint32_t i) const { return fld<int, 68>(i); }
    __device__ __forceinline__ int& occluded(uint32_t i) const { return fld2<int, 72, 288>(i); }
    __device__ __forceinline__ int& occ_a(uint32_t i) const { return fld2<int, 76, 292>(i); }
    __device__ __forceinline__ int& occ_b(uint32_t i) const { return fld2<int, 80, 296>(i); }
    __device__ __forceinline__ uint32_t& left(uint32_t i) const { return fld<uint32_t, 84>(i); }
    __device__ __forceinline__ uint32_t& pix(uint32_t i) const { return fld<uint32_t, 88>(i); }
    __device__ __forceinline__ uint32_t& stamp(uint32_t i) const { return fld<uint32_t, 92>(i); }
    __device__ __forceinline__ uint32_t& stamp0(uint32_t i) const { return fld<uint32_t, 208>(i); }
    __device__ __forceinline__ float4& light(uint32_t i) const { return fld<float4, 96>(i); }
    __device__ __forceinline__ float4& reduc(uint32_t i) const { return fld<float4, 112>(i); }
    __device__ __forceinline__ float4& aov_n(uint32_t i) const { return fld<float4, 128>(i); }
    __device__ __forceinline__ float4& aov_t(uint32_t i) const { return fld<float4, 144>(i); }
    __device__ __forceinline__ float4& aov_b(uint32_t i) const { return fld<float4, 160>(i); }
    __device__ __forceinline__ float4& c_vis(uint32_t i) const { return fld2<float4, 176, 304>(i); }
    __device__ __forceinline__ float4& c_occ(uint32_t i) const { return fld2<float4, 192, 320>(i); }

    __device__ __forceinline__ uint32_t& spec_word(uint32_t i) const { return fld<uint32_t, 212>(i); }
    __device__ __forceinline__ uint32_t& spec_link(uint32_t i) const { return fld<uint32_t, 216>(i); }
    __device__ __forceinline__ uint32_t& spec_start(uint32_t i) const { return fld<uint32_t, 220>(i); }
    __device__ __forceinline__ uint32_t& spec_entry(uint32_t i) const { return fld<uint32_t, 224>(i); }
    __device__ __forceinline__ uint32_t& tally_a(uint32_t i) const { return fld<uint32_t, 232>(i); }
    __device__ __forceinline__ uint32_t& tally_rays(uint32_t i) const { return fld<uint32_t, 236>(i); }
    __device__ __forceinline__ uint32_t& tally_tex(uint32_t i) const { return fld<uint32_t, 240>(i); }
    __device__ __forceinline__ uint32_t& tally_nodes(uint32_t i) const { return fld<uint32_t, 244>(i); }
    __device__ __forceinline__ uint32_t& tally_tris(uint32_t i) const { return fld<uint32_t, 248>(i); }

    __device__ __forceinline__ const float4* ray_pair(uint32_t g, uint32_t kind) const {
        return (const float4*)(base + (size_t)(g * stride + (kind == 0u ? 0u : (kind == 1u ? 32u : 256u))));
    }
};
#define ER_SLOT(field, i) W.field(i)

#define ST_LAP_TAG(pos, cap) (((((pos) / (cap)) & 0x7Fu) + 1u) << 24)
#define ST_LEFT_MASK 0x00FFFFFFu
#define ST_DRAWS_MASK 0x7Fu
#define ST_CONF_SHIFT 8
#define ST_VOTE_SHIFT 11
#define ST_MAJ_SHIFT 16
#define ST_LONG_SHIFT 23
enum { SP_NONE = 0, SP_PENDING = 1, SP_PARKED = 2, SP_VALID = 3, SP_INVALID = 4 };

__device__ __forceinline__ bool st_pixel_of(const DevScene& S, const uint32_t* deal, uint32_t deal_count, uint32_t b, uint32_t nb, uint32_t k, uint32_t& px,
                                            uint32_t& py) {
    const uint32_t t = b + (k >> 6) * nb, l = k & 63u;
    if (t >= deal_count) return false;
    const uint32_t tile = deal[t];
    if (tile == 0xFFFFFFFFu) return false;
    px = (tile % S.tiles_x) * ER_TILE + (l & 7u);
    py = (tile / S.tiles_x) * ER_TILE + (l >> 3);
    return px < S.x_res && py < S.y_res;
}

#define ST_PXY(px, py) ((uint32_t)(px) | ((uint32_t)(py) << 16))
__device__ __forceinline__ uint32_t st_pixel_index(const DevScene& S, uint32_t pxy) { return (pxy >> 16) * S.x_res + (pxy & 0xFFFFu); }

template <bool SPECB>
__device__ __forceinline__ uint32_t st_begin_sample(const DevScene& S, const StState& W, uint32_t g, uint32_t pxy, uint32_t left, bool spec = false, uint32_t given = 0u) {
    const uint32_t px = pxy & 0xFFFFu, py = pxy >> 16;
    uint32_t rs = spec ? given : S.rng[py * S.x_res + px];
    const uint32_t rs0 = rs;
    float c1 = rng_next(rs), c2 = rng_next(rs), c3 = rng_next(rs), c4 = rng_next(rs), c5 = rng_next(rs);
    const CamTrig trig = {S.cam_cx, S.cam_sx, S.cam_cy, S.cam_sy, S.cam_cz, S.cam_sz};
    const Ray ray = camera_ray(S.cam, (int)px, (int)py, S.x_res, S.y_res, c1, c2, c3, c4, c5, S.cam_trig_valid ? &trig : nullptr);
    W.pix(g) = pxy;
    ER_SLOT_RESET(g, ray, rs);
    W.left(g) = left;
    if (SPECB) {
        W.spec_word(g) = spec ? (uint32_t)SP_PENDING : (uint32_t)SP_NONE;
        W.spec_link(g) = 0u;
        W.spec_start(g) = given;
        W.tally_a(g) = 0u; W.tally_rays(g) = 1u;
        W.tally_tex(g) = 0u; W.tally_nodes(g) = 0u; W.tally_tris(g) = 0u;
    }
    ER_SP(W.stamp(g) = sp_now(); W.stamp0(g) = W.stamp(g);)
    return rs0;
}

template <bool HANDOFF>
__device__ __forceinline__ int st_verdict(const StState& W, uint32_t rec, uint32_t wflags, uint32_t amb_bit, uint32_t occ_bit) {
    if (!HANDOFF || (wflags & amb_bit) != 0u) return W.occluded(rec);
    return (wflags & occ_bit) != 0u ? 1 : 0;
}

template <uint32_t LOG2>
__device__ __forceinline__ bool st_take_rays(uint32_t* cells, uint32_t* ctl, const StState& W, uint32_t g0, unsigned long long bm0, bool busy, uint32_t* status,
                                             uint32_t& granted, uint32_t& e, float4& o, float4& d) {
    unsigned long long rq_peek = 0;
    granted = 0;
    if (er_ring_peek_count(rq_peek = er_ring_peek(ctl)) == 0) return false;
    uint32_t hb = 0;
    granted = st_take(ctl, 64u - (uint32_t)__popcll(bm0), hb, rq_peek);
    if (granted == 0) return false;
    const uint32_t rank = st_rank(~bm0);
    const bool take = !busy && rank < granted;
    bool got = false;
    if (take) {
        got = er_ring_get(cells, LOG2, hb + rank, e);
        if (!got) atomicOr(status, ST_ERR_RAY);
    }
    __builtin_amdgcn_fence(__ATOMIC_ACQUIRE, "workgroup");
    const float4* rp = got ? W.ray_pair(g0 + (e & ST_SLOT_MASK), e >> ST_SLOT_BITS) : (const float4*)W.base;
    o = rp[0];
    d = rp[1];
    return got;
}

constexpr uint32_t st_lds_pad(uint32_t bytes) { return (bytes + 15u) & ~15u; }
constexpr uint32_t st_lds_bytes(int form, uint32_t top_nodes) {
    const bool spec = form == 2;
    uint32_t b = 0;
    b += st_lds_pad((spec ? (1u << ST_SQ_LOG2) : 1u) * 4u);
    b += 5u * st_lds_pad(ER_RING_WORDS * 4u);
    b += st_lds_pad((1u << ST_RQ_LOG2) * 4u);
    b += 2u * st_lds_pad((1u << ST_SQ_LOG2) * 4u);
    b += st_lds_pad(ER_STREAM_SLOTS * 4u);
    b += st_lds_pad((ER_STREAM_LDS_HANDOFF ? ER_STREAM_SLOTS : 1u) * 4u);
    b += st_lds_pad(ST_PXBITS_WORDS * 4u);
    b += st_lds_pad(C_WORDS * 4u) + st_lds_pad(4u) + st_lds_pad((spec ? 3u : 1u) * 4u);
    b += top_nodes * 5u * 16u;
    b += st_lds_pad(13u * 4u);
    b += ST_MAX_TRACERS * WF_LDS_STACK * 64u * 8u;
    return b;
}
#define ST_LDS_LIMIT (160u * 1024u)

}

template <bool COUNT, bool EXT, bool MESH, uint32_t ST_THREADS, bool FUSE, int FORM>
__global__ __launch_bounds__(ST_THREADS) void er_stream_kernel(const DevScene __attribute__((address_space(4)))* Sp, StState W, const uint32_t* deal, uint32_t deal_count, uint2* ring_base, uint32_t ring_cap,
                                                          uint32_t* status, uint32_t n_samples, uint32_t tracers, uint32_t refill_min, uint32_t batch_min, uint32_t fin_min) {
    const DevScene& S = *(const DevScene*)Sp;
    if (threadIdx.x == 0) atomicMin((unsigned long long*)(status + ER_SC_START), (unsigned long long)wall_clock64());
    constexpr uint32_t RQ_LOG2 = ST_RQ_LOG2, SLOTS = ER_STREAM_SLOTS, TOP_NODES = FORM == 2 ? ER_STREAM_TOP_NODES - ER_STREAM_TOP_NODES_SPEC_CUT : ER_STREAM_TOP_NODES;
    constexpr bool HANDOFF = ER_STREAM_LDS_HANDOFF != 0;
    constexpr bool EARLY_TAKE = HANDOFF;
    static_assert(st_lds_bytes(FORM, TOP_NODES) <= ST_LDS_LIMIT, "this form of er_stream_kernel needs more LDS than a CU has: fewer top nodes (ER_STREAM_TOP_NODES, _SPEC_CUT)");
    constexpr bool SPEC = FORM == 2;
    constexpr bool KEEP = FORM >= 1;
    bool spec_on = false;
    uint32_t spec_need = 0;
    uint32_t spec_slack = 0;
    uint32_t spec_long = 0;
    uint32_t spec_keep = 0;
    if (SPEC) { spec_need = (fin_min >> 8) & 7u; spec_slack = (fin_min >> 12) & 0xFFu; spec_long = (fin_min >> 20) & 0x1FFu; spec_keep = fin_min >> 29; spec_on = spec_need != 0u && S.px_draws != nullptr; fin_min &= 0xFFu; }
    else if (KEEP) { spec_keep = fin_min >> 29; fin_min &= 0xFFu; }
    __shared__ uint32_t s_free[SPEC ? (1u << ST_SQ_LOG2) : 1u];
    __shared__ __attribute__((aligned(8))) uint32_t s_free_ctl[ER_RING_WORDS];
    __shared__ uint32_t s_rq[1u << RQ_LOG2];
    __shared__ uint32_t s_sq[1u << ST_SQ_LOG2];
    __shared__ uint32_t s_fq[1u << ST_SQ_LOG2];
    __shared__ uint32_t s_wait[SLOTS];
    __shared__ int s_hit[HANDOFF ? SLOTS : 1u];
    __shared__ uint32_t s_pxbits[ST_PXBITS_WORDS];
    __shared__ __attribute__((aligned(8))) uint32_t s_rq_ctl[ER_RING_WORDS], s_sq_ctl[ER_RING_WORDS], s_px_ctl[ER_RING_WORDS], s_fq_ctl[ER_RING_WORDS];
    __shared__ uint32_t s_ctl[C_WORDS];
    __shared__ uint32_t s_front;
    __shared__ uint32_t s_spec[SPEC ? 3 : 1];
    __shared__ float4 s_top[TOP_NODES * 5];
#ifdef ER_TIME_PROBE
    __shared__ uint32_t s_tp[13];
    if (threadIdx.x < 13) s_tp[threadIdx.x] = 0;
#endif
    for (uint32_t i = threadIdx.x; i < TOP_NODES * 5u; i += ST_THREADS)
        s_top[i] = i / 5u < S.node8_count ? S.nodes8[(i / 5u) * ER_NODE8_PIECES + i % 5u] : make_float4(0, 0, 0, 0);
    (void)s_hit;
    const int lane = threadIdx.x & 63;
    const uint32_t wave = threadIdx.x >> 6;
    const uint32_t g0 = blockIdx.x * SLOTS;
    volatile er_lds_u32* v_ctl = (volatile er_lds_u32*)s_ctl;
    const unsigned long long below = (1ull << lane) - 1ull;

    for (uint32_t i = threadIdx.x; i < (1u << RQ_LOG2); i += ST_THREADS) s_rq[i] = 0;
    for (uint32_t i = threadIdx.x; i < (1u << ST_SQ_LOG2); i += ST_THREADS) { s_sq[i] = 0; s_fq[i] = 0; }
    for (uint32_t i = threadIdx.x; i < ST_PXBITS_WORDS; i += ST_THREADS) s_pxbits[i] = 0;
    if (SPEC) for (uint32_t i = threadIdx.x; i < (1u << ST_SQ_LOG2); i += ST_THREADS) s_free[i] = 0;
    if (threadIdx.x < ER_RING_WORDS) { s_rq_ctl[threadIdx.x] = 0; s_sq_ctl[threadIdx.x] = 0; s_px_ctl[threadIdx.x] = 0; s_fq_ctl[threadIdx.x] = 0; }
    if (SPEC && threadIdx.x < ER_RING_WORDS) s_free_ctl[threadIdx.x] = 0;
    if (SPEC && threadIdx.x < 3u) s_spec[threadIdx.x] = 0;
    if (KEEP && threadIdx.x == 0) s_front = 0xFFFFFFFFu;
    if (threadIdx.x < C_WORDS) s_ctl[threadIdx.x] = 0;
    __syncthreads();
    uint2* ring = ring_base + (size_t)blockIdx.x * ring_cap;
    for (uint32_t s = threadIdx.x; s < SLOTS; s += ST_THREADS) s_wait[s] = 0;
    for (uint32_t k = threadIdx.x; k < ring_cap; k += ST_THREADS) ring[k] = make_uint2(0u, 0u);
    __syncthreads();
    for (uint32_t k0 = 0; k0 < ring_cap; k0 += ST_THREADS) {
        const uint32_t k = k0 + threadIdx.x;
        uint32_t px = 0, py = 0;
        const bool valid = n_samples > 0 && k < ring_cap && st_pixel_of(S, deal, deal_count, blockIdx.x, gridDim.x, k, px, py);
        const uint32_t v = st_reserve(&s_ctl[C_INIT], valid);
        const bool to_slot = valid && v < SLOTS;
        const uint32_t idx = ST_PXY(px, py);
        if (to_slot) {
            st_begin_sample<SPEC>(S, W, g0 + v, idx, n_samples);
            s_wait[v] = 1u;
        } else if (valid) {
            const uint32_t pos = v - SLOTS;
            atomicOr(&s_pxbits[pos >> 5], 1u << (pos & 31u));
            ring[pos] = make_uint2(idx, n_samples | ST_LAP_TAG(pos, ring_cap));
        }
        __builtin_amdgcn_fence(__ATOMIC_RELEASE, "workgroup");
        const unsigned long long m = __ballot(to_slot);
        if (m) {
            if (lane == (int)(__ffsll((long long)m) - 1)) atomicAdd(&s_ctl[C_LIVE], (uint32_t)__popcll(m));
            st_push<RQ_LOG2>(s_rq, s_rq_ctl, to_slot, v, status, ST_ERR_RAY);
        }
    }
    __syncthreads();
    if (threadIdx.x == 0) {
        const uint32_t nv = s_ctl[C_INIT];
        const uint32_t in_ring = nv > SLOTS ? nv - SLOTS : 0u;
        s_px_ctl[ER_RING_HEAD] = 0;
        s_px_ctl[ER_RING_TAIL] = in_ring;
        s_px_ctl[ER_RING_COUNT] = in_ring;
    }
    __syncthreads();
    if (threadIdx.x == 0 && s_ctl[C_LIVE] == 0) s_ctl[C_DONE] = 1;
    if (SPEC && spec_on) {
        const uint32_t nv = s_ctl[C_INIT], started = nv < SLOTS ? nv : SLOTS;
        for (uint32_t s0 = 0; s0 < SLOTS; s0 += ST_THREADS) {
            const uint32_t sl = s0 + threadIdx.x;
            st_push<ST_SQ_LOG2>(s_free, s_free_ctl, sl < SLOTS && sl >= started && n_samples > 0, sl, status, ST_ERR_SHADE);
        }
    }

    unsigned c_rays = 0, c_nodes = 0, c_tris = 0;
    unsigned c_paths = 0, c_bounce = 0, c_shaded = 0, c_texels = 0, c_hdri = 0;
    unsigned c_wsteps = 0, c_busy = 0, c_nl = 0, c_tl = 0;

    {
        __shared__ uint2 s_stack[ST_MAX_TRACERS * WF_LDS_STACK * 64];
        __syncthreads();
        if (wave < tracers) {
            uint2* spill = W.spill + (size_t)(blockIdx.x * 16u + wave) * ER_SPILL_PER_WAVE + lane;
            uint2* stack = s_stack + (size_t)wave * (WF_LDS_STACK * 64) + lane;
            Trav T;
            trav_begin(T, f3s(0), f3(0, 0, 1), false, -1, 0.0f);
            bool busy = false, done = false, done_occl = false;
#if ER_TRACER_PRIO
            __builtin_amdgcn_s_setprio(ER_TRACER_PRIO);
#endif
            unsigned ray_n0 = 0, ray_t0 = 0;
            uint32_t lsk = 0;
            uint32_t idle = 0, progress = 0;
            uint32_t a_iter = 0, a_busy = 0;
            ER_SP(uint32_t spA = 0; uint32_t spB = 0; uint32_t spC = 0; uint32_t sAB = 0; uint32_t sBC = 0; uint32_t sCD = 0; uint32_t sN = 0;)
#ifdef ER_TRACER_PROBE
            uint32_t trp[7] = {0, 0, 0, 0, 0, 0, 0}, trp_pub = 0, trp_take = 0;
            unsigned long long trp_last = __builtin_amdgcn_s_memtime();
#endif
            while (true) {
                ER_MARK("tracer_loop_top");
                const unsigned long long bm0 = __ballot(busy);
                const bool visit = 64u - (unsigned)__popcll(bm0) >= refill_min || bm0 == 0;
                bool got = false;
                uint32_t got_e = 0, granted = 0;
                float4 got_o, got_d;
                if (EARLY_TAKE && visit) got = st_take_rays<RQ_LOG2>(s_rq, s_rq_ctl, W, g0, bm0, busy, status, granted, got_e, got_o, got_d);
                if (visit && __ballot(done)) {
                    ER_MARK("tracer_publish");
#ifdef ER_TRACER_PROBE
                    trp_pub++;
#endif
                    const uint32_t ls = lsk & ST_SLOT_MASK, kind = lsk >> ST_SLOT_BITS;
                    if (done) {
                        const uint32_t rec = g0 + ls + (kind == 2u ? W.slots : 0u);
                        if (!HANDOFF) { ER_SLOT_WRITE_RESULT(rec, T, done_occl) }
                        else if (T.shadow) {
                            if (!done_occl && (T.overflow || T.s0 >= 0)) { ER_SLOT_WRITE_RESULT(rec, T, false) }
                        } else {
                            s_hit[ls] = trav_hit(T);
                            if (T.overflow || (T.s0 >= 0 && T.s1 >= 0)) W.hit2(rec) = trav_hit2(T);
                        }
                    }
                    if (SPEC && COUNT && done) {
                        atomicAdd(&W.tally_nodes(g0 + ls), c_nodes - ray_n0);
                        atomicAdd(&W.tally_tris(g0 + ls), c_tris - ray_t0);
                        c_nodes = ray_n0; c_tris = ray_t0;
                    }
                    ER_SP(if (done && kind == 0u) { const uint32_t spD = sp_now(); sAB += spB - spA; sBC += spC - spB; sCD += spD - spC; sN++; W.stamp(g0 + ls) = spD; })
                    __builtin_amdgcn_fence(__ATOMIC_RELEASE, "workgroup");
                    bool last = false;
                    uint32_t fin = 0;
                    if (done) {
                        const bool esc = !T.shadow && !T.overflow && T.s0 < 0 && T.s1 < 0;
                        const bool amb = T.shadow && !done_occl && (T.overflow || T.s0 >= 0);
                        const bool occf = HANDOFF && T.shadow && done_occl, hit2f = HANDOFF && !T.shadow && (T.overflow || (T.s0 >= 0 && T.s1 >= 0));
                        const uint32_t add = (esc ? ST_ESC : 0u) + (amb ? (kind == 1u ? ST_AMB1 : ST_AMB2) : 0u) + (occf ? (kind == 1u ? ST_OCC1 : ST_OCC2) : 0u) +
                                             (hit2f ? ST_HIT2 : 0u) - 1u;
                        fin = atomicAdd(&s_wait[ls], add) + add;
                        last = (fin & ST_COUNT_MASK) == 0u;
                    }
                    const bool escaped = last && (fin & ST_ESC) != 0u && (fin & (ST_AMB1 | ST_AMB2)) == 0u;
                    st_push<ST_SQ_LOG2>(s_sq, s_sq_ctl, last && !escaped, ls | ((fin & ST_FIN) ? (1u << ST_SLOT_BITS) : 0u), status, ST_ERR_SHADE);
                    st_push<ST_SQ_LOG2>(s_fq, s_fq_ctl, escaped, ls | (1u << ST_SLOT_BITS), status, ST_ERR_SHADE);
                    done = false;
                    ER_MARK("tracer_publish_end");
                }
                if (!EARLY_TAKE && visit) got = st_take_rays<RQ_LOG2>(s_rq, s_rq_ctl, W, g0, bm0, busy, status, granted, got_e, got_o, got_d);
#ifdef ER_TRACER_PROBE
                if (granted > 0) trp_take++;
#endif
                if (got) {
                    lsk = got_e;
                    const uint32_t kind = got_e >> ST_SLOT_BITS;
                    const bool shadow = kind != 0u;
                    trav_begin(T, f3(got_o.x, got_o.y, got_o.z), f3(got_d.x, got_d.y, got_d.z), shadow, shadow ? __builtin_bit_cast(int, got_o.w) : -1,
                               shadow ? got_d.w : __builtin_inff());
                    if (!SPEC) c_rays++;
                    if (SPEC && COUNT) { ray_n0 = c_nodes; ray_t0 = c_tris; }
                    busy = true;
                    ER_SP(if (kind == 0u) { spA = W.stamp(g0 + (got_e & ST_SLOT_MASK)); spB = sp_now(); })
                }
                ER_MARK("tracer_refill_end");
                const unsigned long long bm = __ballot(busy);
                if (bm == 0) {
                    if (v_ctl[C_DONE]) break;
                    __builtin_amdgcn_s_sleep(ST_IDLE_SLEEP);
                    ER_TRP(6);
                    const uint32_t pr = er_ring_load(&s_rq_ctl[ER_RING_TAIL]) + er_ring_load(&s_sq_ctl[ER_RING_TAIL]) + er_ring_load(&s_fq_ctl[ER_RING_TAIL]);
                    if (pr != progress) { progress = pr; idle = 0; }
                    if (++idle > ST_WATCHDOG) {
                        if (lane == 0) { atomicOr(status, 1u); s_ctl[C_DONE] = 1; }
                        break;
                    }
                    continue;
                }
                idle = 0;
                a_iter++;
                a_busy += (uint32_t)__popcll(bm);
                ER_TRP(0);
#ifdef ER_TIME_PROBE
                const unsigned long long tr0 = __builtin_amdgcn_s_memtime();
#endif
                ER_MARK("tracer_choose");
                bool finished = false, do_step = false;
                TravStep st;
                st.node = false; st.tri = false; st.two = false; st.tslot = 0; st.noff = 0; st.toff = 0;
                if (busy) {
                    uint2* sp_area = spill;
                    if (COUNT) {
                        uint32_t l = (uint32_t)lane;
                        asm volatile("" : "+v"(l));
                        sp_area = W.spill + ((blockIdx.x * 16u + wave) * (uint32_t)ER_SPILL_PER_WAVE + l);
                    }
                    if (S.node_count != 0) do_step = trav_choose(T, S, stack, sp_area, st);
                    finished = !do_step;
                }
                if (COUNT) {
                    c_wsteps++;
                    c_busy += (unsigned)__popcll(bm);
                    c_nl += (unsigned)__popcll(__ballot(st.node));
                    c_tl += (unsigned)__popcll(__ballot(st.tri));
                }
                TravData D;
                ER_MARK("tracer_fetch");
                ER_TRP(1);
                const bool top = st.node && st.noff < (uint32_t)(TOP_NODES * ER_NODE8_PIECES);
#if ER_STREAM_SPLIT_WAIT
                bool occl = false;
                {
                    TravStep sg = st;
                    if (top) sg.node = false;
                    TravRaw R;
                    trav_fetch_issue(S, sg, R);
                    trav_wait_tri(R, D);
                    ER_TRP(2);
                    ER_MARK("tracer_apply");
                    const bool do_tri = busy && do_step;
                    TravStep stt = st;
                    stt.tri = st.tri && do_tri;
                    occl = trav_apply_tri<COUNT>(T, S, stt, D, c_tris);
                    ER_TRP(3);
                    trav_wait_node(R, D);
                    if (top) trav_node_from_lds(D, s_top, st.noff);
                    ER_TRP(4);
                    TravStep sn = st;
                    sn.node = st.node && do_tri && !occl;
                    trav_apply_node<COUNT>(T, S, sn, D, c_nodes);
                }
                if (busy) {
                    if (do_step && occl) finished = true;
                    if (finished) { busy = false; done = true; done_occl = occl; ER_SP(spC = sp_now();) }
                }
#else
                {
                    TravStep sg = st;
                    if (top) sg.node = false;
                    trav_fetch(S, sg, D);
                    if (top) trav_node_from_lds(D, s_top, st.noff);
                }
                ER_MARK("tracer_apply");
                bool occl = false;
                if (busy) {
                    if (do_step && trav_apply<COUNT>(T, S, st, D, c_nodes, c_tris)) { occl = true; finished = true; }
                    if (finished) { busy = false; done = true; done_occl = occl; }
                }
#endif
#ifdef ER_TIME_PROBE
                if (lane == 0) atomicAdd(&s_tp[12], (unsigned)((__builtin_amdgcn_s_memtime() - tr0) >> 4));
#endif
                ER_MARK("tracer_iter_end");
                ER_TRP(5);
            }
            ER_MARK("tracer_loop_end");
#ifdef ER_TRACER_PROBE
            const unsigned trp_rays = wave_sum(c_rays);
            if (lane == 0) {
                unsigned long long* c = (unsigned long long*)&S.counters->node_visits;
                for (int i = 0; i < 7; i++) atomicAdd(&c[i], (unsigned long long)trp[i]);
                atomicAdd(&c[7], (unsigned long long)trp_pub);
                atomicAdd(&c[8], (unsigned long long)trp_take);
                atomicAdd(&S.counters->paths, (unsigned long long)a_iter);
                atomicAdd(&S.counters->bounce_samples, (unsigned long long)a_busy);
                atomicAdd(&S.counters->rays, (unsigned long long)trp_rays);
            }
#endif
            ER_SP({ unsigned long long* spc = (unsigned long long*)&S.counters->node_visits; sp_add(spc + 0, sAB); sp_add(spc + 1, sBC); sp_add(spc + 2, sCD); sp_add(spc + 5, sN); })
            if (lane == 0) {
                atomicAdd((unsigned long long*)(status + ER_SC_ITERS), (unsigned long long)a_iter);
                atomicAdd((unsigned long long*)(status + ER_SC_BUSY), (unsigned long long)a_busy);
            }
        }
    }
    if (wave >= tracers) {
        int* stack = (int*)(W.spill + (size_t)(blockIdx.x * 16u + wave) * ER_SPILL_PER_WAVE) + lane;
        bool have = false;
        uint32_t e = 0;
        uint32_t idle = 0, spins = 0, progress = 0;
        uint32_t slack = 0;
        ER_SP(uint32_t sDE = 0; uint32_t sEF = 0; uint32_t sGE = 0; uint32_t sNG = 0; uint32_t sSS = 0; uint32_t sNS = 0;)
#if ER_SHADER_PRIO
        __builtin_amdgcn_s_setprio(ER_SHADER_PRIO);
#endif
#ifdef ER_TIME_PROBE
        unsigned long long tp_last = __builtin_amdgcn_s_memtime();
        uint32_t tp_sec = 99u;
#endif
        while (true) {
            ER_MARK("shader_loop_top");
            const unsigned long long sq_peek = er_ring_peek(s_sq_ctl), fq_peek = er_ring_peek(s_fq_ctl);
            const uint32_t avail = er_ring_peek_count(sq_peek), favail = er_ring_peek_count(fq_peek);
            if (avail == 0 && favail == 0) {
                if (v_ctl[C_DONE]) break;
                __builtin_amdgcn_s_sleep(ST_IDLE_SLEEP);
                const uint32_t pr = er_ring_load(&s_rq_ctl[ER_RING_TAIL]) + er_ring_load(&s_sq_ctl[ER_RING_TAIL]) + er_ring_load(&s_fq_ctl[ER_RING_TAIL]);
                if (pr != progress) { progress = pr; idle = 0; }
                if (SPEC) slack++;
                if (++idle > ST_WATCHDOG) {
                    if (lane == 0) { atomicOr(status, 2u); s_ctl[C_DONE] = 1; }
                    break;
                }
                continue;
            }
            idle = 0;
            const uint32_t bmin = batch_min & 0xFFu, patience = batch_min >> 8;
            bool fin_mode = favail >= fin_min;
            if (!fin_mode && avail < bmin) {
                if (favail > 0 && (avail == 0 || spins >= patience / 3u)) fin_mode = true;
                else if (spins < patience) {
                    spins++;
                    if (SPEC) slack++;
                    __builtin_amdgcn_s_sleep(ST_BATCH_SLEEP);
                    continue;
                }
            }
            spins = 0;
            const uint32_t waited = slack;
            slack = 0;
            ER_MARK("shader_take");
            ER_TPS(0);
            uint32_t hb = 0;
            const uint32_t granted = fin_mode ? st_take(s_fq_ctl, 64u, hb, fq_peek) : st_take(s_sq_ctl, 64u, hb, sq_peek);
            if (granted == 0) continue;
            have = (uint32_t)lane < granted;
            if (have && !(fin_mode ? er_ring_get(s_fq, ST_SQ_LOG2, hb + (uint32_t)lane, e) : er_ring_get(s_sq, ST_SQ_LOG2, hb + (uint32_t)lane, e))) { have = false; atomicOr(status, ST_ERR_SHADE); }
            __builtin_amdgcn_fence(__ATOMIC_ACQUIRE, "workgroup");
            bool push_closest = false, push_shadow = false, push_light = false, retire = false;
            const uint32_t ls = e & ST_SLOT_MASK;
            const uint32_t slot = g0 + ls;
            const uint32_t wflags = (HANDOFF && have) ? s_wait[ls] : 0u;
            bool want_pixel = false, to_finish = false;
            uint32_t rs = 0, left_after = 0, done_idx = 0;
            bool has_spec = false, wake = false, push_spec = false, keep_own = false;
            uint32_t wake_entry = 0, ls_spec = 0;
            ER_MARK("shader_step");
            ER_TPS(1);
            ER_SP(uint32_t spE = 0;)
            ER_SP(if (have) { spE = sp_now(); if (fin_mode ? (e >> ST_SLOT_BITS) != 0 : (e >> ST_SLOT_BITS) == 0) sDE += spE - W.stamp(slot);
                              else if (fin_mode) { sGE += spE - W.stamp(slot); sNG++; } })
            bool parked = false, discard = false;
            if (SPEC && spec_on && fin_mode && have) {
                uint32_t sw = __hip_atomic_load(&W.spec_word(slot), __ATOMIC_RELAXED, __HIP_MEMORY_SCOPE_WORKGROUP);
                if (sw != (uint32_t)SP_NONE) {
                    if (sw == (uint32_t)SP_PENDING) {
                        W.spec_entry(slot) = e;
                        __builtin_amdgcn_fence(__ATOMIC_RELEASE, "workgroup");
                        sw = atomicCAS(&W.spec_word(slot), (uint32_t)SP_PENDING, (uint32_t)SP_PARKED);
                    }
                    __builtin_amdgcn_fence(__ATOMIC_ACQUIRE, "workgroup");
                    parked = sw == (uint32_t)SP_PENDING;
                    discard = sw == (uint32_t)SP_INVALID;
                    if (!parked) W.spec_word(slot) = (uint32_t)SP_NONE;
                }
            }
            uint32_t cancel_w = (uint32_t)SP_NONE;
            if (SPEC && spec_on && have && !fin_mode) cancel_w = __hip_atomic_load(&W.spec_word(slot), __ATOMIC_RELAXED, __HIP_MEMORY_SCOPE_WORKGROUP);
            if (SPEC && discard) retire = true;
            bool cancel = false;
            unsigned &o_bounce = c_bounce, &o_shaded = c_shaded, &o_hdri = c_hdri, &o_texels = c_texels, &o_nodes = c_nodes, &o_tris = c_tris;
            if (have && !fin_mode) {
                unsigned t_bounce = 0, t_shaded = 0, t_hdri = 0, t_texels = 0, t_nodes = 0, t_tris = 0;
                unsigned &c_bounce = SPEC ? t_bounce : o_bounce, &c_shaded = SPEC ? t_shaded : o_shaded, &c_hdri = SPEC ? t_hdri : o_hdri;
                unsigned &c_texels = SPEC ? t_texels : o_texels, &c_nodes = SPEC ? t_nodes : o_nodes, &c_tris = SPEC ? t_tris : o_tris;
                (void)c_texels;
                const bool fin_only = (e >> ST_SLOT_BITS) != 0;
                ER_SLOT_LOAD(slot);
                if (packed & ER_SLOT_PENDING) ER_SLOT_RESOLVE_QUERY(slot, st_verdict<HANDOFF>(W, slot, wflags, ST_AMB1, ST_OCC1))
                if (EXT && (packed & ER_SLOT_LPENDING)) ER_SLOT_RESOLVE_QUERY(slot + W.slots, st_verdict<HANDOFF>(W, slot + W.slots, wflags, ST_AMB2, ST_OCC2))
                bool pending = false, lpending = false;
                bool done = fin_only;
                Ray ray;
                ray.o = f3s(0);
                ray.d = f3(0, 0, 1);
                float prev_pdf = -1.0f;
                float mesh_d = 0.0f;
                if (!fin_only) {
                    ER_SLOT_LOAD_RAY(slot)
                    int hslot = resolve_closest<COUNT>(S, stack, ray, HANDOFF ? s_hit[ls] : W.hit(slot), (!HANDOFF || (wflags & ST_HIT2) != 0u) ? W.hit2(slot) : -1, c_nodes, c_tris);
                    c_bounce++;
#define ER_BOUNCE_FUSE FUSE
#define ER_BOUNCE_MESH MESH
#include "er_slot_bounce.inc"
                }
                bool alive = true, fin_next = false;
                if (done && (pending || lpending)) {
                    fin_next = true;
                } else if (done) {
                    ER_SLOT_STORE_LIGHT(slot);
                    alive = false;
                    to_finish = true;
                    ER_SP(W.stamp(slot) = sp_now();)
                } else {
                    push_closest = true;
                }
                push_shadow = pending;
                push_light = EXT && lpending;
                if (alive) {
                    ER_SLOT_STORE(slot, !fin_next);
                    s_wait[ls] = (push_closest ? 1u : 0u) + (push_shadow ? 1u : 0u) + (push_light ? 1u : 0u) + (fin_next ? ST_FIN : 0u);
                }
                if (SPEC) {
                    cancel = cancel_w == (uint32_t)SP_INVALID;
                    if (!cancel) {
                        const unsigned long long add = (unsigned long long)(t_bounce | (t_shaded << 10) | (t_hdri << 20)) |
                                                       ((unsigned long long)((push_closest ? 1u : 0u) + (push_shadow ? 1u : 0u) + (push_light ? 1u : 0u)) << 32);
                        __hip_atomic_fetch_add((unsigned long long*)&W.tally_a(slot), add, __ATOMIC_RELAXED, __HIP_MEMORY_SCOPE_WORKGROUP);
                        if (COUNT) {
                            W.tally_tex(slot) += t_texels;
                            atomicAdd(&W.tally_nodes(slot), t_nodes);
                            atomicAdd(&W.tally_tris(slot), t_tris);
                        }
                    } else {
                        push_closest = false; push_shadow = false; push_light = false; to_finish = false;
                        retire = true;
                    }
                }
            }
            if (!fin_mode) {
                if (__ballot(to_finish)) {
                    __builtin_amdgcn_fence(__ATOMIC_RELEASE, "workgroup");
                    st_push<ST_SQ_LOG2>(s_fq, s_fq_ctl, to_finish, ls, status, ST_ERR_SHADE);
                }
            } else if (have && !parked && !discard) {
                ER_TPS(6);
                const uint32_t pxy = W.pix(slot);
                const uint32_t idx = st_pixel_index(S, pxy);
                const float4 L4 = W.light(slot);
                F3 light = f3(L4.x, L4.y, L4.z);
                rs = __builtin_bit_cast(uint32_t, L4.w);
                const float4 R4 = W.reduc(slot);
                const uint32_t packed = __builtin_bit_cast(uint32_t, R4.w);
                if (S.tile_cost) __hip_atomic_fetch_add(&S.tile_cost[(pxy >> 19) * S.tiles_x + ((pxy & 0xFFFFu) >> 3)], (packed & ER_SLOT_BOUNCE_MASK) + 1u, __ATOMIC_RELAXED, __HIP_MEMORY_SCOPE_AGENT);
                if ((e >> ST_SLOT_BITS) != 0) {
                    F3 reduction = f3(R4.x, R4.y, R4.z);
                    uint32_t bounce = packed & ER_SLOT_BOUNCE_MASK;
                    if (packed & ER_SLOT_PENDING) ER_SLOT_ADD_QUERY(slot, st_verdict<HANDOFF>(W, slot, wflags, 0u, ST_OCC1))
                    if (EXT && (packed & ER_SLOT_LPENDING)) ER_SLOT_ADD_QUERY(slot + W.slots, st_verdict<HANDOFF>(W, slot + W.slots, wflags, 0u, ST_OCC2))
                    const float4 d = W.ray_d(slot);
                    Ray ray;
                    ray.o = f3s(0);
                    ray.d = f3(d.x, d.y, d.z);
                    float prev_pdf = EXT ? d.w : -1.0f;
                    float mesh_d = 0.0f;
                    const int hslot = -1;
                    bool done = false, pending = false, lpending = false;
                    c_bounce++;
#define ER_BOUNCE_HDRI_QUERY(sr, self_slot, d_self, cv, co) ((void)(sr), (void)(self_slot), (void)(d_self), (void)(cv), (void)(co))
#define ER_BOUNCE_LIGHT_QUERY(lr, self_slot, limit, lv, lo) ((void)(lr), (void)(self_slot), (void)(limit), (void)(lv), (void)(lo))
#define ER_BOUNCE_FIRST_HIT(n, t, b) ((void)(n), (void)(t), (void)(b))
#include "er_bounce.inc"
#undef ER_BOUNCE_HDRI_QUERY
#undef ER_BOUNCE_LIGHT_QUERY
#undef ER_BOUNCE_FIRST_HIT
                    (void)bounce; (void)done; (void)pending; (void)lpending; (void)prev_pdf; (void)mesh_d;
                }
                const float4 an = W.aov_n(slot), at = W.aov_t(slot), ab = W.aov_b(slot);
                const uint32_t sa = S.samples[idx];
                const uint32_t sa2 = accumulate_sample(S, idx, sa, light, f3(an.x, an.y, an.z), f3(at.x, at.y, at.z), f3(ab.x, ab.y, ab.z));
                if (sa2 != sa) S.samples[idx] = sa2;
                S.rng[idx] = rs;
                c_paths++;
                if (SPEC) {
                    const uint32_t ta = W.tally_a(slot);
                    c_bounce += ta & 0x3FFu; c_shaded += (ta >> 10) & 0x3FFu; c_hdri += (ta >> 20) & 0x3FFu;
                    c_rays += W.tally_rays(slot);
                    if (COUNT) { c_texels += W.tally_tex(slot); c_nodes += W.tally_nodes(slot); c_tris += W.tally_tris(slot); }
                }
                if (SPEC && spec_on) {
                    {
                        const uint32_t ta = W.tally_a(slot);
                        const uint32_t per_opaque = MESH ? 7u : (EXT && (S.ext_flags & ER_FLAG_POINT_LIGHTS) != 0 && S.light_count > 0) ? 5u : 4u;
                        uint32_t nd = 5u + ((ta >> 10) & 0x3FFu) + per_opaque * ((ta >> 20) & 0x3FFu);
                        nd = nd > ST_DRAWS_MASK ? 0u : nd;
                        const uint32_t oldh = S.px_draws[idx];
                        uint32_t cand = oldh & ST_DRAWS_MASK, conf = (oldh >> ST_CONF_SHIFT) & 7u;
                        if (nd != 0u && nd == cand) conf = conf < 7u ? conf + 1u : 7u;
                        else if (conf >= 2u) conf -= 2u;
                        else { cand = nd; conf = nd != 0u ? 1u : 0u; }
                        uint32_t maj = (oldh >> ST_MAJ_SHIFT) & ST_DRAWS_MASK, votes = (oldh >> ST_VOTE_SHIFT) & 7u, mean16 = oldh >> ST_LONG_SHIFT;
                        if (nd != 0u && nd == maj) votes = votes < 7u ? votes + 1u : 7u;
                        else if (votes > 0u) votes--;
                        else { maj = nd; votes = nd != 0u ? 1u : 0u; }
                        const uint32_t its16 = ((ta & 0x3FFu) + ((e >> ST_SLOT_BITS) != 0 ? 1u : 0u)) << 4;
                        mean16 = (uint32_t)((int)mean16 + (((int)(its16 > 511u ? 511u : its16) - (int)mean16) >> 3));
                        S.px_draws[idx] = cand | (conf << ST_CONF_SHIFT) | (votes << ST_VOTE_SHIFT) | (maj << ST_MAJ_SHIFT) | (mean16 << ST_LONG_SHIFT);
                    }
                    const uint32_t link = W.spec_link(slot);
                    if (link) {
                        const uint32_t f = g0 + link - 1u;
                        const bool ok = W.spec_start(f) == rs;
                        __builtin_amdgcn_fence(__ATOMIC_RELEASE, "workgroup");
                        const uint32_t old = atomicExch(&W.spec_word(f), ok ? (uint32_t)SP_VALID : (uint32_t)SP_INVALID);
                        atomicAdd(&s_spec[ok ? 1 : 2], 1u);
                        if (old == (uint32_t)SP_PARKED) {
                            __builtin_amdgcn_fence(__ATOMIC_ACQUIRE, "workgroup");
                            wake = true;
                            wake_entry = W.spec_entry(f);
                        }
                        has_spec = ok;
                    }
                }
                ER_SP(sSS += sp_now() - W.stamp0(slot); sNS++;)
                left_after = W.left(slot) - 1;
                done_idx = pxy;
                want_pixel = true;
                if (KEEP && spec_keep != 0u) {
                    const uint32_t front = atomicMin(&s_front, left_after);
                    keep_own = left_after > 0u && !has_spec && left_after >= front + spec_keep;
                }
            }
            ER_MARK("shader_pixel_ring");
            ER_TPS(7);
            if (__ballot(want_pixel)) {
                const bool back = want_pixel && left_after > 0 && !has_spec && !(KEEP && keep_own);
                const unsigned long long mb = __ballot(back);
                if (mb) {
                    __builtin_amdgcn_fence(__ATOMIC_RELEASE, "workgroup");
                    uint32_t base = 0;
                    if (lane == 0) base = er_ring_reserve(s_px_ctl, (uint32_t)__popcll(mb));
                    base = (uint32_t)__builtin_amdgcn_readlane((int)base, 0);
                    if (back) {
                        const uint32_t pos = base + (uint32_t)__popcll(mb & below), cell = pos & (ring_cap - 1u);
                        if (!er_bits_acquire(s_pxbits, cell)) atomicOr(status, ST_ERR_PIXEL);
                        ring[cell] = make_uint2(done_idx, left_after | ST_LAP_TAG(pos, ring_cap));
                    }
                    __builtin_amdgcn_fence(__ATOMIC_RELEASE, "workgroup");
                    if (lane == 0) er_ring_publish(s_px_ctl, (uint32_t)__popcll(mb));
                }
                bool spawn_want = false;
                uint32_t spawn_rs = 0, spawn_pxy = 0, spawn_left = 0, spawn_draws = 0;
                const bool want_take = want_pixel && !(KEEP && keep_own);
                const unsigned long long mw = __ballot(want_take);
                uint32_t hb2 = 0;
                const uint32_t granted2 = st_take(s_px_ctl, (uint32_t)__popcll(mw), hb2, er_ring_peek(s_px_ctl));
                const uint32_t rank = (uint32_t)__popcll(mw & below);
                if (want_take && rank < granted2) {
                    const uint32_t ppos = hb2 + rank, pcell = ppos & (ring_cap - 1u);
                    const unsigned long long* cell = (const unsigned long long*)(ring + pcell);
                    const uint32_t want_tag = ST_LAP_TAG(ppos, ring_cap);
                    unsigned long long w = 0;
                    uint32_t y = 0, guard = 0;
                    while (true) {
                        w = __hip_atomic_load(cell, __ATOMIC_RELAXED, __HIP_MEMORY_SCOPE_WORKGROUP);
                        y = (uint32_t)(w >> 32);
                        if ((y & ~ST_LEFT_MASK) == want_tag) break;
                        if (++guard >= ER_RING_GUARD) { y = 0; break; }
                        __builtin_amdgcn_s_sleep(1);
                    }
// ... 43 lines not shown
                    if (spawn_want && rk < gf) {
                        got_free = er_ring_get(s_free, ST_SQ_LOG2, hbf + rk, fslot);
                        if (!got_free) atomicOr(status, ST_ERR_SHADE);
                    }
                    __builtin_amdgcn_fence(__ATOMIC_ACQUIRE, "workgroup");
                    if (got_free) {
                        uint32_t sp = spawn_rs;
                        for (uint32_t k = 0; k < spawn_draws; k++) { sp ^= sp << 13; sp ^= sp >> 17; sp ^= sp << 5; }
                        st_begin_sample<SPEC>(S, W, g0 + fslot, spawn_pxy, spawn_left, true, sp);
                        W.spec_link(slot) = fslot + 1u;
                        s_wait[fslot] = 1u;
                        push_spec = true;
                        ls_spec = fslot;
                    }
                    const unsigned long long mgot = __ballot(got_free);
                    if (mgot && lane == (int)(__ffsll((long long)mgot) - 1)) {
                        atomicAdd(&s_ctl[C_LIVE], (uint32_t)__popcll(mgot));
                        atomicAdd(&s_spec[0], (uint32_t)__popcll(mgot));
                    }
                }
            }
            if (SPEC && spec_on && __ballot(wake)) {
                __builtin_amdgcn_fence(__ATOMIC_RELEASE, "workgroup");
                st_push<ST_SQ_LOG2>(s_fq, s_fq_ctl, wake, wake_entry, status, ST_ERR_SHADE);
            }
            ER_MARK("shader_publish");
            ER_TPS(8);
            __builtin_amdgcn_fence(__ATOMIC_RELEASE, "workgroup");
            {
                const unsigned long long mc = __ballot(push_closest), ms = __ballot(push_shadow), ml = EXT ? __ballot(push_light) : 0ull;
                const unsigned long long mx = SPEC ? __ballot(push_spec) : 0ull;
                const unsigned nc = (unsigned)__popcll(mc), ns = (unsigned)__popcll(ms), nl = (unsigned)__popcll(ml) + (unsigned)__popcll(mx);
                ER_SP(if (push_closest) { const uint32_t spF = sp_now(); sEF += spF - spE; W.stamp(slot) = spF; })
                if (nc + ns + nl) {
                    uint32_t base = 0;
                    if (lane == 0) base = er_ring_reserve(s_rq_ctl, nc + ns + nl);
                    base = (uint32_t)__builtin_amdgcn_readlane((int)base, 0);
                    bool ok = true;
                    if (push_closest) ok = er_ring_put(s_rq, RQ_LOG2, base + (uint32_t)__popcll(mc & below), ls) && ok;
                    if (push_shadow) ok = er_ring_put(s_rq, RQ_LOG2, base + nc + (uint32_t)__popcll(ms & below), ls | (1u << ST_SLOT_BITS)) && ok;
                    if (EXT && push_light) ok = er_ring_put(s_rq, RQ_LOG2, base + nc + ns + (uint32_t)__popcll(ml & below), ls | (2u << ST_SLOT_BITS)) && ok;
                    if (SPEC && push_spec) ok = er_ring_put(s_rq, RQ_LOG2, base + nc + ns + (uint32_t)__popcll(ml) + (uint32_t)__popcll(mx & below), ls_spec) && ok;
                    if (!ok) atomicOr(status, ST_ERR_RAY);
                    if (lane == 0) er_ring_publish(s_rq_ctl, nc + ns + nl);
                }
                const unsigned long long mr = __ballot(retire);
                if (SPEC && spec_on && mr) st_push<ST_SQ_LOG2>(s_free, s_free_ctl, retire, ls, status, ST_ERR_SHADE);
                if (mr) {
                    const uint32_t nr = (uint32_t)__popcll(mr);
                    if (lane == 0) {
                        const uint32_t oldl = atomicSub(&s_ctl[C_LIVE], nr);
                        if (oldl == nr) s_ctl[C_DONE] = 1;
                    }
                }
            }
            have = false;
            ER_TPS(9);
#ifdef ER_TIME_PROBE
            if (lane == 0) { atomicAdd(&s_tp[10], 1u); atomicAdd(&s_tp[11], granted); }
#endif
        }
        ER_MARK("shader_loop_end");
        ER_SP({ unsigned long long* spc = (unsigned long long*)&S.counters->node_visits; sp_add(spc + 3, sDE); sp_add(spc + 4, sEF); sp_add(spc + 6, sGE); sp_add(spc + 7, sNG); sp_add(spc + 8, sSS); atomicAdd(&S.counters->paths, (unsigned long long)sNS); })
    }
    ER_MARK("epilogue");
#if defined(ER_STAGE_PROBE) || defined(ER_TRACER_PROBE)
    return;
#endif
#ifdef ER_TIME_PROBE
    __syncthreads();
    if (threadIdx.x == 0) {
        unsigned long long* c = (unsigned long long*)&S.counters->node_visits;
        for (int i = 1; i < 10; i++) atomicAdd(&c[i - 1], (unsigned long long)s_tp[i]);
        atomicAdd(&S.counters->paths, (unsigned long long)s_tp[10]);
        atomicAdd(&S.counters->bounce_samples, (unsigned long long)s_tp[11]);
        atomicAdd(&S.counters->rays, (unsigned long long)s_tp[12]);
    }
    return;
#endif
    if (SPEC) {
        if (lane == 0) {
            const unsigned q0 = atomicExch(&s_spec[0], 0u), q1 = atomicExch(&s_spec[1], 0u), q2 = atomicExch(&s_spec[2], 0u);
            if (q0 | q1 | q2) { atomicAdd(status + ER_SC_SPEC, q0); atomicAdd(status + ER_SC_SPEC + 1, q1); atomicAdd(status + ER_SC_SPEC + 2, q2); }
        }
    }
    unsigned t0 = wave_sum(c_paths), t1 = wave_sum(c_bounce), t2 = wave_sum(c_rays), t3 = wave_sum(c_shaded), t4 = wave_sum(c_hdri);
    unsigned t5 = 0, t6 = 0, t7 = 0;
    if (COUNT) { t5 = wave_sum(c_nodes); t6 = wave_sum(c_tris); t7 = wave_sum(c_texels); }
    if (lane == 0) {
        const unsigned long long t_end = (unsigned long long)wall_clock64();
        atomicMax((unsigned long long*)(status + ER_SC_END + 2 * (blockIdx.x & 7u)), t_end);
        atomicMax((unsigned long long*)(status + ER_SC_WG_END + 2 * blockIdx.x), t_end);
        ER_FLUSH_COUNTERS(true, t0, t1, t2, t3, t4, t5, t6);
        if (COUNT) atomicAdd(&S.counters->texel_fetches, (unsigned long long)t7);
        ER_FLUSH_TRACE_LANES(c_wsteps, c_busy, c_nl, c_tl);
    }
}

#ifndef ER_STREAM_MESH_TU
hipError_t er_probe_stream(const char** which) {
    hipFuncAttributes a;
    *which = "er_stream_kernel";
    hipError_t e = hipFuncGetAttributes(&a, (const void*)er_stream_kernel<false, false, false, 1024u, false, 0>);
    if (e == hipSuccess) e = hipFuncGetAttributes(&a, (const void*)er_stream_kernel<false, false, false, 768u, true, 0>);
    return e != hipSuccess ? e : hipFuncGetAttributes(&a, (const void*)er_stream_kernel<false, false, false, 768u, true, 2>);
}

ErStreamLaunchForm er_stream_launch_form(uint32_t max_bounces, uint32_t tri_count, uint32_t waves, bool spec, bool keep) {
    static const uint32_t spec_flag = [] {
        const char* e = getenv("ER_STREAM_SPEC");
        const char* b = getenv("ER_STREAM_SPEC_SLACK");
        int v = e ? atoi(e) : 2, bl = b ? atoi(b) : 1;
        return ((uint32_t)(v < 0 ? 0 : (v > 7 ? 7 : v)) << 8) | ((uint32_t)(bl < 0 ? 0 : (bl > 255 ? 255 : bl)) << 12);
    }();
    static const uint32_t spec_long16 = [] {
        const char* e = getenv("ER_STREAM_SPEC_LONG");
        int v = e ? atoi(e) : ER_STREAM_SPEC_LONG_DEFAULT;
        return (uint32_t)(v < 0 ? 0 : (v > 16 ? 16 : v));
    }();
    static const uint32_t spec_keep = [] {
        const char* e = getenv("ER_STREAM_SPEC_KEEP");
        int v = e ? atoi(e) : ER_STREAM_SPEC_KEEP_DEFAULT;
        return (uint32_t)(v < 0 ? 0 : (v > 7 ? 7 : v));
    }();
    waves = waves == 12u ? 12u : 16u;
    const uint32_t long_thr = waves == 12u ? max_bounces * spec_long16 : 0u;
    const uint32_t spec_now = (max_bounces <= 1000u && tri_count >= ER_STREAM_SPEC_MIN_TRIS) ? (spec_flag | ((long_thr > 511u ? 0u : long_thr) << 20) | (((waves == 16u && keep) ? spec_keep : 0u) << 29)) : 0u;
    const uint32_t keep_plain = (keep && waves == 16u) ? (spec_keep << 29) : 0u;
    if (spec && spec_now) return {2u, waves, spec_now};
    if (keep_plain) return {1u, waves, keep_plain};
    return {0u, waves, 0u};
}

#endif

#ifdef ER_STREAM_MESH_TU
#define ER_STREAM_LAUNCH er_launch_stream_mesh
#else
#define ER_STREAM_LAUNCH er_launch_stream
#endif
void ER_STREAM_LAUNCH(const ErStreamLaunch& L) {
    const DevScene& S = *L.S;
#ifndef ER_STREAM_MESH_TU
    if (er_mesh_active(S)) {
        er_launch_stream_mesh(L);
        return;
    }
#endif
    static const uint32_t refill_min = [] {
        const char* e = getenv("ER_STREAM_REFILL_MIN");
        int v = e ? atoi(e) : 12;
        return (uint32_t)(v < 1 ? 1 : (v > 64 ? 64 : v));
    }();
    static const uint32_t batch_min = [] {
        const char* e = getenv("ER_STREAM_BATCH_MIN");
        int v = e ? atoi(e) : 64;
        const char* p = getenv("ER_STREAM_BATCH_SPINS");
        int sp = p ? atoi(p) : 3;
        return (uint32_t)(v < 1 ? 1 : (v > 64 ? 64 : v)) | ((uint32_t)(sp < 0 ? 0 : (sp > 100000 ? 100000 : sp)) << 8);
    }();
    static const uint32_t fin_min = [] {
        const char* e = getenv("ER_STREAM_FIN_MIN");
        int v = e ? atoi(e) : 64;
        return (uint32_t)(v < 1 ? 1 : (v > 64 ? 64 : v));
    }();
    if (S.owned_tile_count == 0 || L.n_samples == 0) return;
    const ErStreamLaunchForm form = er_stream_launch_form(S.max_bounces, S.tri_count, L.waves, L.spec, L.keep);
    const uint32_t waves = form.waves, last = fin_min | form.bits;
// ... 47 lines not shown
```

### elevenrender_amd/csrc/er_stream_host.cpp

```cpp
#include <algorithm>
#include <map>

#include "er_scene.h"
#include "../../include/eleven_hip_debug.h"

using namespace erh;

uint32_t er_stream_deal_tiles(const uint32_t* owned, uint32_t count, uint32_t tiles_x, uint32_t blocks, bool xcd_aware, std::vector<uint32_t>& out, uint32_t edge) {
    if (edge == 0u) {
        const char* e = getenv("ER_STREAM_SUPER_TILE");
        const int v = e ? atoi(e) : 0;
        edge = v >= 1 ? (uint32_t)v : ER_STREAM_SUPER_TILE_DEFAULT;
    }
    const uint32_t X = (xcd_aware && blocks % 8u == 0u) ? 8u : 1u, per = blocks / X, S8 = edge;
    const uint32_t super_x = (tiles_x + S8 - 1u) / S8;
    std::map<uint32_t, std::vector<uint32_t>> by_super;
    for (uint32_t i = 0; i < count; i++) {
        const uint32_t tx = owned[i] % tiles_x, ty = owned[i] / tiles_x;
        by_super[X == 1u ? 0u : (ty / S8) * super_x + tx / S8].push_back(owned[i]);
    }
    std::vector<std::vector<uint32_t>> seq(X);
    for (auto& kv : by_super) {
        uint32_t best = 0;
        for (uint32_t x = 1; x < X; x++) if (seq[x].size() < seq[best].size()) best = x;
// ... 59 lines not shown
    std::vector<std::vector<uint32_t>> mine(blocks);
    std::vector<uint64_t> load(per);
    uint32_t most = 0;
    for (uint32_t x = 0; x < X; x++) {
        std::vector<uint32_t>& q = seq[x];
        std::sort(q.begin(), q.end(), [&](uint32_t a, uint32_t b) { const uint64_t ca = c_of(a), cb = c_of(b); return ca != cb ? ca > cb : a < b; });
        std::fill(load.begin(), load.end(), 0);
        for (uint32_t t : q) {
            uint32_t best = per;
            for (uint32_t j = 0; j < per; j++)
                if (mine[(size_t)j * X + x].size() < cap && (best == per || load[j] < load[best])) best = j;
            if (best == per) return keep();
            mine[(size_t)best * X + x].push_back(t);
            load[best] += c_of(t);
        }
    }
    for (auto& m : mine) { std::sort(m.begin(), m.end()); most = std::max<uint32_t>(most, (uint32_t)m.size()); }
    out.assign((size_t)blocks * most, NONE);
    for (uint32_t b = 0; b < blocks; b++)
        for (size_t k = 0; k < mine[b].size(); k++) out[(size_t)b + k * blocks] = mine[b][k];
    return most;
}

bool stream_xcd_aware(size_t owned_tiles, uint32_t blocks) {
    const char* xe = getenv("ER_STREAM_XCD_TILES");
    return xe ? atoi(xe) != 0 : owned_tiles * 64 > (size_t)blocks * ER_STREAM_SLOTS;
}

StreamDeal stream_deal_owned(const std::vector<uint32_t>& owned, uint32_t tiles_x, uint32_t cus) {
    StreamDeal d;
    d.most = er_stream_deal_tiles(owned.data(), (uint32_t)owned.size(), tiles_x, cus, stream_xcd_aware(owned.size(), cus), d.tiles);
    return d;
}

StreamForm stream_choose_form(size_t tiles, uint32_t blocks, bool light_query, uint32_t tri_count, uint32_t flags) {
    StreamForm f;
    const uint32_t large_tracers = (light_query || tri_count > 4000000u) ? 12u : 13u;
    f.tracers = large_tracers;
    f.waves = 16;
    const size_t px_per_cu = tiles * 64 / std::max<uint32_t>(1u, blocks);
    const uint32_t small_tracers = px_per_cu > ER_STREAM_TEN_TRACERS_SHARE ? 10u : 9u;
    if (px_per_cu <= ER_STREAM_SMALL_SHARE) { f.waves = 12; f.tracers = small_tracers; }
    f.adapt = px_per_cu >= 4u * ER_STREAM_SLOTS && !(flags & ER_FLAG_COUNTERS);
    f.keep = px_per_cu <= ER_STREAM_KEEP_SHARE;
    f.spec = px_per_cu <= ER_STREAM_SPEC_SHARE;
    if (const char* e = getenv("ER_STREAM_SPEC_FORM")) f.spec = atoi(e) != 0;
    if (const char* e = getenv("ER_STREAM_KEEP")) f.keep = atoi(e) != 0;
    if (const char* e = getenv("ER_STREAM_WAVES")) { f.waves = atoi(e) == 12 ? 12 : 16; f.tracers = f.waves == 12 ? small_tracers : large_tracers; }
    if (const char* e = getenv("ER_STREAM_TRACERS")) { f.tracers = (uint32_t)std::min(13, std::max(1, atoi(e))); f.adapt = false; }
    if (const char* e = getenv("ER_STREAM_ADAPT")) f.adapt = atoi(e) != 0;
    return f;
}

static void stream_set_form(ErScene* s, size_t tiles) {
    StreamHost& st = s->st;
    st.form = stream_choose_form(tiles, st.blocks, st.lights, s->tri_count, s->params.flags);
    st.tracers_start = st.form.tracers; st.low_streak = 0; st.up_budget = 1;
}

static hipError_t stream_drop_pending_deal(ErScene* s) {
    s->st.deal_pending = false;
    s->st.counting = false;
    s->dev.tile_cost = s->ad_dev.tile_cost = nullptr;
    s->st.deal_large.clear(); s->st.deal_large.shrink_to_fit();
    s->st.deal_base.clear(); s->st.deal_base.shrink_to_fit();
    return hipMemcpyAsync(s->d_dev.p, &s->dev, sizeof(DevScene), hipMemcpyHostToDevice, s->stream);
}

int stream_begin(ErScene* s, const std::vector<uint32_t>& owned, StreamDeal& deal, uint32_t cus, bool light_query) {
    StreamHost& st = s->st;
    int rc;
    st.blocks = cus;
    st.lights = light_query;
    stream_set_form(s, owned.size());
    st.readings = 0;
    const size_t slots = (size_t)st.blocks * ER_STREAM_SLOTS, npx = (size_t)s->x_res * s->y_res;
    if ((rc = upload(s->d_wf4, nullptr, slots * er_stream_record_bytes(light_query) / sizeof(float4), s->stream)) != ER_OK) return rc;
    const size_t ctl_words = ER_STREAM_CTL_LEAD + er_stream_ctl_words(st.blocks);
    if ((rc = upload(s->d_wf1, nullptr, ctl_words, s->stream)) != ER_OK) return rc;
    if ((rc = upload(s->d_spill, nullptr, er_stream_spill_entries(st.blocks), s->stream)) != ER_OK) return rc;
    st.ctl = s->d_wf1.p;
    HIP_TRY(hipMemsetAsync(st.ctl, 0, ctl_words * sizeof(uint32_t), s->stream));
    st.spec[0] = st.spec[1] = st.spec[2] = 0;
    st.launch_start = st.launch_end = 0; st.wg_end.clear();
    const bool xcd_aware = stream_xcd_aware(owned.size(), st.blocks);
    const uint32_t tiles_x = s->tiles_x();
    uint32_t most = deal.most;
    st.deal_off = 0; st.deal_n = (uint32_t)deal.tiles.size();
    st.deal_alt_off = 0; st.deal_alt_n = 0;
    st.deal_base_off = 0; st.deal_lvl_off = 0; st.deal_lvl_cap = 0; st.deal_levelled = false;
    st.counting = false;
    st.deal_base.clear(); st.cost_host.clear();
    st.deal_host = deal.tiles;
    st.xcd_spread = -1.0;
    const char* adapt_knob = getenv("ER_STREAM_ADAPT");
    st.deal_pending = false;
    st.deal_large.clear();
    st.d_tile_cost.release();
    if (xcd_aware && st.blocks % 8u == 0u && owned.size() * 64 / st.blocks >= ER_STREAM_SLOTS * 3u / 2u && !(s->params.flags & ER_FLAG_COUNTERS) &&
        !getenv("ER_STREAM_SUPER_TILE") && !(adapt_knob && atoi(adapt_knob) == 0)) {
        std::vector<uint32_t> large;
        const uint32_t most_large = er_stream_deal_tiles(owned.data(), (uint32_t)owned.size(), tiles_x, st.blocks, xcd_aware, large, ER_STREAM_SUPER_TILE_LARGE);
        if ((size_t)most_large * 64u <= ER_STREAM_MAX_RING) {
            st.deal_alt_off = (uint32_t)deal.tiles.size(); st.deal_alt_n = (uint32_t)large.size();
            deal.tiles.insert(deal.tiles.end(), large.begin(), large.end());
            most = std::max(most, most_large);
            st.deal_large.swap(large);
            const size_t n_tiles = (size_t)tiles_x * s->tiles_y();
            if ((rc = upload(st.d_tile_cost, nullptr, n_tiles, s->stream)) != ER_OK) return rc;
            HIP_TRY(hipMemsetAsync(st.d_tile_cost.p, 0, n_tiles * sizeof(uint32_t), s->stream));
            st.deal_pending = st.counting = true;
        }
    }
    if ((rc = upload(st.d_px_draws, nullptr, npx, s->stream)) != ER_OK) return rc;
    HIP_TRY(hipMemsetAsync(st.d_px_draws.p, 0, npx * sizeof(uint32_t), s->stream));
    if (s->x_res > 65535u || s->y_res > 65535u)
        return fail(ER_ERR_INVALID_ARG, "er_render_begin: ER_FLAG_STREAM carries a pixel as x | y << 16: frames up to 65535 x 65535; use ER_FLAG_WAVEFRONT (the automatic choice does)");
    st.ring_cap = 64u;
    while (st.ring_cap < most * 64u) st.ring_cap <<= 1;
    if (st.ring_cap > ER_STREAM_MAX_RING)
        return fail(ER_ERR_INVALID_ARG, "er_render_begin: ER_FLAG_STREAM serves at most " + std::to_string((size_t)ER_STREAM_MAX_RING * st.blocks) +
                                            " owned pixels per rank; use ER_FLAG_WAVEFRONT (the automatic choice does)");
    if ((rc = upload(st.d_ticket, nullptr, (size_t)st.blocks * (size_t)st.ring_cap * 2, s->stream)) != ER_OK) return rc;
    if (st.counting) { st.deal_lvl_off = (uint32_t)deal.tiles.size(); st.deal_lvl_cap = st.blocks * (st.ring_cap / 64u); }
    if ((rc = upload(st.d_deal, nullptr, deal.tiles.size() + st.deal_lvl_cap, s->stream)) != ER_OK) return rc;
    if (!deal.tiles.empty()) HIP_TRY(hipMemcpyAsync(st.d_deal.p, deal.tiles.data(), deal.tiles.size() * sizeof(uint32_t), hipMemcpyHostToDevice, s->stream));
    return ER_OK;
}

int stream_redeal(ErScene* s) {
    StreamHost& st = s->st;
    const bool large = st.large_deal_in_use();
    if (st.deal_pending || st.counting) HIP_TRY(stream_drop_pending_deal(s));
    const uint32_t count = (uint32_t)s->ad_active.size(), tiles_x = s->tiles_x();
    std::vector<uint32_t> deal;
    uint32_t most = er_stream_deal_tiles(s->ad_active.data(), count, tiles_x, st.blocks, stream_xcd_aware(count, st.blocks), deal, large ? ER_STREAM_SUPER_TILE_LARGE : 0u);
    if ((size_t)most * 64u > st.ring_cap) most = er_stream_deal_tiles(s->ad_active.data(), count, tiles_x, st.blocks, false, deal);
    if ((size_t)most * 64u > st.ring_cap) return fail(ER_ERR_STATE, "er_render_samples: the active tiles do not fit the pixel rings");
    int rc;
    if ((rc = upload(st.d_deal, deal.data(), deal.size(), s->stream)) != ER_OK) return rc;
    st.deal_off = 0; st.deal_n = (uint32_t)deal.size();
    st.deal_alt_off = 0; st.deal_alt_n = 0;
    st.deal_base_off = 0; st.deal_lvl_off = 0; st.deal_lvl_cap = 0; st.deal_levelled = false;
    st.deal_host = deal;
    stream_set_form(s, count);
    HIP_TRY(hipStreamSynchronize(s->stream));
    return ER_OK;
}

static int stream_launch(ErScene* s, uint32_t k) {
    StreamHost& st = s->st;
    HIP_TRY(hipMemsetAsync(st.status() + ER_SC_ITERS, 0, (er_stream_ctl_words(st.blocks) - ER_SC_ITERS) * sizeof(uint32_t), s->stream));
    HIP_TRY(hipMemsetAsync(st.status() + ER_SC_START, 0xFF, 2 * sizeof(uint32_t), s->stream));
    if (k > 0) st.launches++;
    ErStreamLaunch L;
    L.S = &s->dev; L.S_dev = s->d_dev.p;
    L.records = s->d_wf4.p; L.slots = st.blocks * ER_STREAM_SLOTS; L.lights = st.lights;
    L.spill = s->d_spill.p;
    L.deal = st.d_deal.p + st.deal_off; L.deal_count = st.deal_n;
    L.ring = st.d_ticket.p; L.ring_cap = st.ring_cap;
    L.status = st.status();
    L.n_samples = k;
    L.count = (s->params.flags & ER_FLAG_COUNTERS) != 0;
    L.blocks = st.blocks; L.tracers = st.form.tracers; L.waves = st.form.waves; L.spec = st.form.spec; L.keep = st.form.keep;
    L.stream = s->stream;
    er_launch_stream(L);
    return ER_OK;
}

int stream_enqueue(ErScene* s, uint32_t n) {
    StreamHost& st = s->st;
    static const bool split_first = [] { const char* e = getenv("ER_STREAM_SPLIT_FIRST"); return !(e && atoi(e) == 0); }();
    int rc;
    if (st.deal_pending && n >= 2u && split_first) {
        if ((rc = stream_launch(s, 1u)) != ER_OK) return rc;
        HIP_TRY(hipGetLastError());
        HIP_TRY(hipStreamSynchronize(s->stream));
        if ((rc = er_scene_stream_status(s, "er_render_samples")) != ER_OK) return rc;
        st.probe_launch = true;
        stream_adapt(s);
        st.probe_launch = false;
        n -= 1u;
    }
    return stream_launch(s, n);
}

int er_scene_stream_status(ErScene* s, const char* who) {
    StreamHost& st = s->st;
    if (!(s->params.flags & ER_FLAG_STREAM) || !st.ctl) return ER_OK;
    std::vector<uint32_t> w(er_stream_ctl_words(st.blocks), 0u);
    HIP_TRY(hipMemcpy(w.data(), st.status(), w.size() * sizeof(uint32_t), hipMemcpyDeviceToHost));
    if (st.spec_seen != st.launches) {
        st.spec_seen = st.launches;
        for (int k = 0; k < 3; k++) st.spec[k] += w[ER_SC_SPEC + k];
    }
    if (w[ER_SC_STATUS] != 0)
        return fail(ER_ERR_STATE, std::string(who) + ": the streaming schedule stopped without finishing (watchdog status " + std::to_string(w[ER_SC_STATUS]) + "); the planes are incomplete");
    auto u64 = [&](uint32_t i) { return (unsigned long long)w[i] | ((unsigned long long)w[i + 1] << 32); };
    const unsigned long long iters = u64(ER_SC_ITERS), busy = u64(ER_SC_BUSY);
    st.busy = iters ? (double)busy / (64.0 * (double)iters) : 0.0;
    const unsigned long long t0 = u64(ER_SC_START);
    unsigned long long lo = ~0ull, hi = 0;
    for (uint32_t x = 0; x < 8; x++) { const unsigned long long e = u64(ER_SC_END + 2 * x); lo = std::min(lo, e); hi = std::max(hi, e); }
    st.xcd_spread = (t0 != ~0ull && lo > t0 && hi - t0 >= 200000ull) ? (double)(hi - lo) / (double)(hi - t0) : -1.0;
    st.launch_ms = (t0 != ~0ull && hi > t0) ? (double)(hi - t0) * 1e-5 : 0.0;
    st.launch_start = (t0 != ~0ull && hi > t0) ? t0 : 0u; st.launch_end = st.launch_start ? hi : 0u;
    st.wg_end.assign(st.blocks, 0u);
    for (uint32_t b = 0; b < st.blocks; b++) st.wg_end[b] = u64(ER_SC_WG_END + 2 * b);
    return ER_OK;
}

void stream_balance(const ErScene* s, std::vector<uint32_t>& wg_tiles, std::vector<uint64_t>& wg_cost, std::vector<uint64_t>& wg_ticks) {
    const StreamHost& st = s->st;
    wg_tiles.assign(st.blocks, 0u); wg_cost.assign(st.blocks, 0u); wg_ticks.assign(st.blocks, 0u);
    for (size_t i = 0; i < st.deal_host.size() && st.blocks; i++) {
        const uint32_t t = st.deal_host[i];
        if (t == 0xFFFFFFFFu) continue;
        wg_tiles[i % st.blocks]++;
        if (t < st.cost_host.size()) wg_cost[i % st.blocks] += st.cost_host[t];
    }
    for (uint32_t b = 0; b < st.blocks && b < st.wg_end.size(); b++)
        if (st.launch_start && st.wg_end[b] > st.launch_start) wg_ticks[b] = st.wg_end[b] - st.launch_start;
}

static void stream_print_balance(const ErScene* s) {
    const StreamHost& st = s->st;
    std::vector<uint32_t> tiles; std::vector<uint64_t> cost, ticks;
    stream_balance(s, tiles, cost, ticks);
    double t_sum = 0, t_max = 0, t_min = 0, c_sum = 0, c_max = 0, c_min = 0;
    uint32_t n = 0, n_max = 0, n_min = 0;
    for (uint32_t b = 0; b < st.blocks; b++) {
        if (!tiles[b] || !ticks[b]) continue;
        const double t = (double)ticks[b], c = (double)cost[b];
        if (!n) { t_max = t_min = t; c_max = c_min = c; n_max = n_min = tiles[b]; }
        t_sum += t; t_max = std::max(t_max, t); t_min = std::min(t_min, t);
        c_sum += c; c_max = std::max(c_max, c); c_min = std::min(c_min, c);
        n_max = std::max(n_max, tiles[b]); n_min = std::min(n_min, tiles[b]);
        n++;
    }
    if (!n || t_sum <= 0) return;
    const double t_mean = t_sum / n, c_mean = c_sum / n;
    fprintf(stderr, "[er_stream] workgroups of a launch of %.3f ms: finished max/mean %.4f min/mean %.4f, idle tail S %.4f", t_max * 1e-5, t_max / t_mean, t_min / t_mean, (t_max - t_mean) / t_max);
    if (c_mean > 0) fprintf(stderr, "; counted cost max/mean %.4f min/mean %.4f", c_max / c_mean, c_min / c_mean);
    fprintf(stderr, " (%s deal, %u ... %u tiles; measured times: printed, nothing is decided on them)\n", st.deal_levelled ? "cost-levelled" : "count", n_min, n_max);
}

void stream_adapt(ErScene* s) {
    StreamHost& st = s->st;
    if (!(s->params.flags & ER_FLAG_STREAM)) return;
    const bool verbose = getenv("ER_STREAM_VERBOSE") != nullptr;
    if (st.adapted == st.launches) return;
    st.adapted = st.launches;
    if (verbose && !st.form.adapt) fprintf(stderr, "[er_stream] tracer lanes %.3f full at %u + %u waves (fixed split)\n", st.busy, st.form.tracers, st.form.waves - st.form.tracers);
    const bool counted = st.deal_pending || st.counting;
    bool have_cost = false;
    if (counted) {
        std::vector<uint32_t> cost(st.d_tile_cost.n);
        have_cost = hipMemcpy(cost.data(), st.d_tile_cost.p, cost.size() * sizeof(uint32_t), hipMemcpyDeviceToHost) == hipSuccess;
        if (have_cost) st.cost_host.swap(cost);
    }
    if (verbose) stream_print_balance(s);
    if (st.deal_pending) {
        const std::vector<uint32_t>& cost = st.cost_host;
        if (have_cost) {
            double x[8] = {0, 0, 0, 0, 0, 0, 0, 0};
            const std::vector<uint32_t>& L = st.deal_large;
            for (size_t i = 0; i < L.size(); i++)
                if (L[i] != 0xFFFFFFFFu && L[i] < cost.size()) x[(i % st.blocks) % 8u] += (double)cost[L[i]];
            double lo = x[0], hi = x[0], sum = 0;
            for (double v : x) { lo = std::min(lo, v); hi = std::max(hi, v); sum += v; }
            const double spread = sum > 0 ? (hi - lo) / (sum / 8.0) : 0.0;
            const char* lim_env = getenv("ER_STREAM_COST_SPREAD_MAX");
            const double limit = lim_env ? atof(lim_env) : (double)ER_STREAM_COST_SPREAD_MAX;
            const bool take = sum > 0 && spread <= limit;
            st.cost_spread = spread;
            if (verbose) fprintf(stderr, "[er_stream] counted work of the XCDs' shares on super-tiles of %u: %.4f of the mean apart (limit %.4f) -> %s\n", (unsigned)ER_STREAM_SUPER_TILE_LARGE, spread,
                                 limit, take ? "large regions" : "the default deal stays");
            if (take) { st.deal_off = st.deal_base_off = st.deal_alt_off; st.deal_n = st.deal_alt_n; st.deal_host = st.deal_large; }
        }
        st.deal_pending = false;
        st.deal_base = st.deal_host;
        st.deal_large.clear(); st.deal_large.shrink_to_fit();
    }
    if (counted) {
        const char* lv = getenv("ER_STREAM_COST_LEVEL");
        const bool level = !(lv && atoi(lv) == 0) && have_cost && st.deal_lvl_cap != 0u && !st.deal_base.empty();
        if (level) {
            std::vector<uint32_t> lvl;
            er_stream_level_by_cost(st.deal_base, s->tiles_x(), st.blocks, st.cost_host.data(), st.cost_host.size(), st.ring_cap / 64u, lvl);
            if (lvl == st.deal_base) {
                st.deal_off = st.deal_base_off; st.deal_n = (uint32_t)st.deal_base.size(); st.deal_levelled = false;
                st.deal_host = st.deal_base;
            } else if (lvl.size() <= st.deal_lvl_cap &&
                       hipMemcpyAsync(st.d_deal.p + st.deal_lvl_off, lvl.data(), lvl.size() * sizeof(uint32_t), hipMemcpyHostToDevice, s->stream) == hipSuccess) {
                (void)hipStreamSynchronize(s->stream);
                st.deal_off = st.deal_lvl_off; st.deal_n = (uint32_t)lvl.size(); st.deal_levelled = true;
                st.deal_host.swap(lvl);
            }
        }
        if (!level || !st.probe_launch) (void)stream_drop_pending_deal(s);
        (void)hipStreamSynchronize(s->stream);
    }
    if (verbose && st.xcd_spread >= 0.0)
        fprintf(stderr, "[er_stream] XCDs finished %.3f of the launch apart (a measured time: printed, nothing is decided on it)\n", st.xcd_spread);
    if (!st.form.adapt || st.busy <= 0.0 || st.probe_launch) return;
    const uint32_t lo = st.form.waves == 12 ? 7u : 10u;
    const uint32_t before = st.form.tracers;
    const char* forced = getenv("ER_STREAM_FORCE_BUSY");
    double busy = st.busy;
    if (forced) {
        const char* q = forced;
        for (uint32_t k = 0; k < st.readings; k++) { const char* c = strchr(q, ','); if (!c) break; q = c + 1; }
        busy = atof(q);
    }
    st.readings++;
    if (!forced && st.launch_ms < ER_STREAM_ADAPT_MIN_MS) {
        if (verbose) fprintf(stderr, "[er_stream] tracer lanes %.3f full in a launch of %.2f ms: too short to be a reading\n", st.busy, st.launch_ms);
        return;
    }
    if (busy < 0.85) {
        if (++st.low_streak >= 2u && st.form.tracers > lo) { st.form.tracers--; st.low_streak = 0; }
    } else {
        st.low_streak = 0;
        if (busy > 0.93 && st.up_budget > 0u && st.form.tracers < st.tracers_start) { st.form.tracers++; st.up_budget--; }
    }
    if (verbose) fprintf(stderr, "[er_stream] tracer lanes %.3f full%s at %u + %u waves -> %u + %u\n", busy, forced ? " (forced reading)" : "", before, st.form.waves - before, st.form.tracers, st.form.waves - st.form.tracers);
}

void stream_fill_info(const ErScene* s, ErStreamInfo* out) {
    const StreamHost& st = s->st;
    out->waves = st.form.waves; out->tracers = st.form.tracers;
    out->large_regions = st.large_deal_in_use() ? 1u : 0u;
    out->deal_pending = st.deal_pending ? 1u : 0u;
    out->launches = (uint32_t)st.launches;
    out->pixels_per_cu = (uint32_t)((size_t)s->dev.owned_tile_count * 64 / std::max<uint32_t>(1u, st.blocks));
    out->lanes_busy = st.busy; out->launch_ms = st.launch_ms; out->cost_spread = st.cost_spread;
    out->spec_started = st.spec[0]; out->spec_right = st.spec[1]; out->spec_wrong = st.spec[2];
    out->form = er_stream_launch_form(s->dev.max_bounces, s->tri_count, st.form.waves, st.form.spec, st.form.keep).form;
}
```

### elevenrender_amd/csrc/er_stream_host.h

```cpp
#pragma once
#include <stdint.h>

#include <vector>

#include "er_devbuf.h"
#include "er_stream.h"

struct ErScene;
struct ErStreamInfo;

struct StreamForm {
    uint32_t waves = 16, tracers = 0;
    bool adapt = false, keep = false, spec = false;
};
StreamForm stream_choose_form(size_t tiles, uint32_t blocks, bool light_query, uint32_t tri_count, uint32_t flags);
bool stream_xcd_aware(size_t owned_tiles, uint32_t blocks);

struct StreamDeal {
    std::vector<uint32_t> tiles;
    uint32_t most = 0;
};
StreamDeal stream_deal_owned(const std::vector<uint32_t>& owned, uint32_t tiles_x, uint32_t cus);

struct StreamHost {
    uint32_t blocks = 0;
    uint32_t ring_cap = 0;
    bool lights = false;
    StreamForm form;
    uint32_t tracers_start = 0;
    uint32_t low_streak = 0;
    uint32_t up_budget = 1;
    uint32_t readings = 0;
    uint32_t* ctl = nullptr;
    uint32_t* status() const { return ctl + ER_STREAM_CTL_LEAD; }
    double busy = 0.0;
    double launch_ms = 0.0;
    uint64_t launch_start = 0, launch_end = 0;
    std::vector<uint64_t> wg_end;
    double xcd_spread = 0.0;
    double cost_spread = -1.0;
    uint64_t spec[3] = {0, 0, 0};
    uint64_t spec_seen = 0;
    uint64_t launches = 0, adapted = 0;
    bool probe_launch = false;
    erh::DevBuf<uint32_t> d_deal, d_ticket;
    uint32_t deal_off = 0, deal_n = 0;
    uint32_t deal_alt_off = 0, deal_alt_n = 0;
    uint32_t deal_base_off = 0;
    uint32_t deal_lvl_off = 0, deal_lvl_cap = 0;
    bool deal_levelled = false;
    bool counting = false;
    std::vector<uint32_t> deal_base;
    std::vector<uint32_t> deal_host;
    std::vector<uint32_t> cost_host;
    bool deal_pending = false;
    erh::DevBuf<uint32_t> d_tile_cost;
    std::vector<uint32_t> deal_large;
    erh::DevBuf<uint32_t> d_px_draws;

    bool large_deal_in_use() const { return deal_alt_n != 0u && deal_base_off == deal_alt_off; }
    void release() {
        d_deal.release(); d_ticket.release(); d_tile_cost.release(); d_px_draws.release();
        ctl = nullptr;
    }
};

int stream_begin(ErScene* s, const std::vector<uint32_t>& owned, StreamDeal& deal, uint32_t cus, bool light_query);
int stream_redeal(ErScene* s);
int stream_enqueue(ErScene* s, uint32_t n);
void stream_adapt(ErScene* s);
void stream_fill_info(const ErScene* s, ErStreamInfo* out);
void stream_balance(const ErScene* s, std::vector<uint32_t>& wg_tiles, std::vector<uint64_t>& wg_cost, std::vector<uint64_t>& wg_ticks);
```

### include/eleven_hip_debug.h

```cpp
#ifndef ELEVEN_HIP_DEBUG_H
#define ELEVEN_HIP_DEBUG_H
#include <stdint.h>
#ifdef __cplusplus
extern "C" {
#endif

typedef struct ErBvhCheck {
    uint32_t node_count, leaf_count, max_depth, max_leaf_size;
    uint32_t tris_in_leaves;
    uint32_t duplicate_tris;
    uint32_t uncontained;
    uint32_t unreachable_nodes;
    float lift_bound;
    float build_ms;
    double sah_cost;
} ErBvhCheck;

int er_debug_bvh_check(const float* vertices, const float* normals, uint32_t tri_count, int threads, ErBvhCheck* out);

typedef struct ErAccelDump {
    uint32_t tri_count;
    uint32_t node_count;
    uint32_t node8_count;
    uint32_t node8_pieces;
    uint32_t attr_pieces;
    uint32_t max_depth;
    uint32_t max_depth8;
    uint32_t builder;
    float lo[3], hi[3];
    float lift_bound;
    float max_lift;
} ErAccelDump;

struct ErScene;
int er_debug_read_accel(struct ErScene* scene, ErAccelDump* info, void* nodes, uint64_t nodes_cap, void* nodes8, uint64_t nodes8_cap,
                        void* isect, uint64_t isect_cap, void* attr, uint64_t attr_cap);

int er_debug_bvh_dump(const float* vertices, const float* normals, uint32_t tri_count, int threads, ErAccelDump* info, void* nodes, uint64_t nodes_cap,
                      void* nodes8, uint64_t nodes8_cap, uint32_t* slot_to_tri, uint64_t slot_cap, float* tri_lift, uint64_t lift_cap);

typedef struct ErCostSumsDebug {
    double node_area, leaf_area, tri_area, cost;
    float ms; uint32_t reserved;
} ErCostSumsDebug;
int er_debug_accel_cost_terms(struct ErScene* scene, ErCostSumsDebug* sums, double* node_terms, uint64_t node_cap, float* tri_terms, uint64_t tri_cap);
int er_debug_accel_cost_host(const void* nodes8, uint32_t node8_count, uint32_t node8_pieces, const void* isect, uint32_t tri_count, ErCostSumsDebug* sums,
                             double* node_terms, uint64_t node_cap, float* tri_terms, uint64_t tri_cap);

int er_debug_cdf_search(const float* cdf, int length, const float* values, int32_t* out, int count);

struct ErScene;
int er_debug_closest_hit(struct ErScene* scene, const float* origins, const float* dirs, uint32_t n, int32_t* tri_ids, float* positions, float* distances);

int er_debug_trace_rays(struct ErScene* scene, const float* origins, const float* dirs, uint32_t n, const int32_t* self_slots,
                        const float* limits, int32_t* tri_ids, int32_t* slots, float* positions, float* distances, int32_t* info);

int er_debug_trace_rays_levels(struct ErScene* scene, const float* origins, const float* dirs, uint32_t n, const int32_t* self_slots,
                               const float* limits, int32_t* tri_ids, int32_t* slots, float* positions, float* distances, int32_t* info,
                               uint32_t* spill_levels, uint32_t* lds_levels, uint32_t* stack_levels);

int er_debug_spill_levels(const void* spilled, uint64_t spilled_bytes, uint32_t n, uint32_t usable, uint32_t* levels);

typedef struct ErTraceRec {
    int32_t bounce;
    int32_t tri;
    int32_t shadow_tri;
    int32_t opaque;
    float position[3];
    float wi[3];
    float light[3];
    float reduction[3];
    int32_t shadow_occ;
    int32_t light_occ;
} ErTraceRec;

int er_debug_trace_pixel(struct ErScene* scene, uint32_t idx, ErTraceRec* recs, int max_recs, int* count);

int er_debug_read_light_table(struct ErScene* scene, int32_t* tri_index, float* cdf, uint32_t cap);
int er_debug_read_light_table_prob(struct ErScene* scene, int32_t* tri_index, float* cdf, float* prob, uint32_t cap);

int er_debug_read_hdri_trig(struct ErScene* scene, uint32_t* cols, uint32_t col_cap, uint32_t* rows, uint32_t row_cap);
int er_debug_hdri_trig_host(int32_t width, int32_t height, uint32_t* cols, uint32_t* rows);

enum { ER_FN_RNG = 0, ER_FN_CAMERA_RAY, ER_FN_TRI_HIT, ER_FN_DISNEY_EVAL, ER_FN_DISNEY_PDF, ER_FN_DISNEY_SAMPLE, ER_FN_SPHERICAL,
       ER_FN_REV_SPHERICAL, ER_FN_TEXTURE, ER_FN_HDRI_SEARCH, ER_FN_HDRI_PDF, ER_FN_MATH, ER_FN_MESH_PICK, ER_FN_COUNT };
int er_debug_eval(struct ErScene* scene, int kind, const float* in, uint32_t n, uint32_t in_stride, float* out, uint32_t out_stride);

struct ErComm;
int er_debug_comm_create_local(uint32_t world, struct ErComm** out);

typedef struct ErStreamInfo {
    uint32_t waves, tracers;
    uint32_t large_regions;
    uint32_t deal_pending;
    uint32_t launches;
    uint32_t pixels_per_cu;
    double lanes_busy;
    double launch_ms;
    double cost_spread;
    uint64_t spec_started, spec_right, spec_wrong;
    uint32_t form;
    uint32_t reserved;
} ErStreamInfo;
int er_debug_stream_info(struct ErScene* s, ErStreamInfo* out);

int er_debug_gather_buffers(struct ErScene* s, uint32_t peer, void** in_ptr, uint64_t* in_bytes, void** mine_ptr, uint64_t* mine_bytes);

int er_debug_comm_loopback(struct ErComm* c, uint64_t bytes, double* ms);

int er_debug_stream_deal(const uint32_t* owned, uint32_t count, uint32_t tiles_x, uint32_t blocks, int xcd_aware, uint32_t edge, uint32_t* out, uint32_t out_cap,
                         uint32_t* most);

int er_debug_stream_level(const uint32_t* deal, uint32_t deal_n, uint32_t tiles_x, uint32_t blocks, const uint32_t* cost, uint32_t cost_n, uint32_t cap,
                          uint32_t* out, uint32_t out_cap, uint32_t* most);

typedef struct ErStreamBalance {
    uint32_t blocks;
    uint32_t most;
    uint32_t levelled;
    uint32_t counting;
    uint32_t cost_tiles;
    uint32_t cap;
    uint64_t launch_ticks;
} ErStreamBalance;
int er_debug_stream_balance(struct ErScene* s, ErStreamBalance* info, uint64_t* wg_ticks, uint32_t* wg_tiles, uint64_t* wg_cost, uint32_t wg_cap,
                            uint32_t* deal, uint32_t deal_cap, uint32_t* tile_cost, uint32_t cost_cap);

typedef struct ErStreamForm {
    uint32_t waves, tracers;
    uint32_t adapt;
    uint32_t keep, spec;
    uint32_t reserved;
} ErStreamForm;
int er_debug_stream_form(uint32_t tiles, uint32_t blocks, int light_query, uint32_t tri_count, uint32_t flags, ErStreamForm* out);

typedef struct ErTexEntry { int32_t width, height, channels, filter; uint32_t offset; } ErTexEntry;
typedef struct ErFusedEntry { int32_t width, height, filter; uint32_t offset; } ErFusedEntry;
typedef struct ErTexturePlan {
    uint32_t texture_count;
    uint32_t fused_count;
    uint32_t fused_any, reserved;
    ErTexEntry hdri;
    uint64_t pool_floats;
} ErTexturePlan;
struct ErSceneDesc;
int er_debug_texture_plan(const struct ErSceneDesc* desc, ErTexturePlan* plan, uint8_t* modes, uint64_t modes_cap, ErTexEntry* table, uint64_t table_cap,
                          ErFusedEntry* fused, uint64_t fused_cap);

typedef struct ErTextureDump {
    uint32_t texture_count, material_count, fused_count, cdf_count, guide_count;
    uint32_t tex_pow2, fused_any;
    int32_t hdri_buckets;
    float hdri_radiance_sum;
    ErTexEntry hdri_tex;
    uint64_t pool_floats;
} ErTextureDump;
int er_debug_read_textures(struct ErScene* scene, ErTextureDump* info, void* table, uint64_t table_cap, void* pool, uint64_t pool_cap, void* fused, uint64_t fused_cap,
                           void* mat_pre, uint64_t mat_pre_cap, void* materials, uint64_t materials_cap, void* cdf, uint64_t cdf_cap, void* guide, uint64_t guide_cap);

void er_debug_set_host_alloc_limit(uint64_t bytes);

void er_debug_set_gpu_build_failure(int kind);

int er_debug_transform_apply(const float m[12], uint32_t count, const float* vertices, const float* normals, const float* tangents,
                             float* out_vertices, float* out_normals, float* out_tangents);

int er_debug_id_rank(const uint32_t* ids, uint32_t count, uint32_t* out_ids, uint32_t* out_counts, uint32_t* distinct);

int er_debug_history_camera(const void* camera , float out[12]);
int er_debug_history_project(const float cam[12], uint32_t x_res, uint32_t y_res, uint32_t count, const float* points, float* out_xy, uint32_t* out_ok);
int er_debug_history_back_matrix(const float m_capture[12], const float m_now[12], float out[12]);
int er_debug_history_taps(const float cam[12], uint32_t x_res, uint32_t y_res, float depth_tolerance, uint32_t count, const uint32_t* hit, const uint32_t* object,
                          const float* P, const uint32_t* moved, const float* back, const uint32_t* old_hit, const uint32_t* old_object, const float* old_dist,
                          const float* old_cw, float* out_rgbw, uint32_t* out_state, uint32_t* out_class);
int er_debug_history_capture(uint32_t count, const float* beauty, const uint32_t* samples, const float* hist, float max_weight, float* out);
int er_debug_history_blend(uint32_t count, const float* beauty, const uint32_t* samples, const float* hist, float* out);

int er_debug_variance_mark(uint32_t count, const float* beauty, const uint32_t* samples, float* state);
int er_debug_variance_fold(uint32_t count, const float* beauty, const uint32_t* samples, float* state, uint32_t* folded);
int er_debug_variance_value(uint32_t count, const float* state, const uint32_t* samples, float* out);
int er_debug_variance_split(uint32_t count, const float* value, const float* albedo, float* ve);
int er_debug_variance_level_px(uint32_t w, uint32_t h, uint32_t step, float kc, float ka, float kz, const float* e, const float* ve, const float* normal, const float* albedo,
                               const float* depth, float* out_e, float* out_ve);

int er_debug_history_variance_current(uint32_t count, const float* state, float* out);
// ... 14 lines not shown
```

Before: 2121 Msamples/s.

## Skip HDRI light sampling for zero-throughput paths and queue them separately

```diff
diff --git a/elevenrender_amd/abi.py b/elevenrender_amd/abi.py
--- a/elevenrender_amd/abi.py
+++ b/elevenrender_amd/abi.py
@@ -248,7 +248,7 @@
     _fields_ = [("waves", C.c_uint32), ("tracers", C.c_uint32), ("large_regions", C.c_uint32), ("deal_pending", C.c_uint32), ("launches", C.c_uint32),
                 ("pixels_per_cu", C.c_uint32), ("lanes_busy", C.c_double), ("launch_ms", C.c_double), ("cost_spread", C.c_double),
                 ("spec_started", C.c_uint64), ("spec_right", C.c_uint64), ("spec_wrong", C.c_uint64),
-                ("form", C.c_uint32), ("reserved", C.c_uint32)]
+                ("form", C.c_uint32), ("dead_rule", C.c_uint32), ("dead_steps", C.c_uint64)]
 
 
 class ErStreamBalance(C.Structure):
diff --git a/elevenrender_amd/csrc/er_api.cpp b/elevenrender_amd/csrc/er_api.cpp
--- a/elevenrender_amd/csrc/er_api.cpp
+++ b/elevenrender_amd/csrc/er_api.cpp
@@ -475,6 +475,36 @@
     return ER_OK;
 }
 
+static bool dead_step_scene_ok(const ErScene* s) {
+    auto in01 = [](float v) { return v >= 0.0f && v <= 1.0f; };
+    for (const ErMaterial& m : s->materials)
+        if (!(in01(m.clearcoat_gloss) && in01(m.clearcoat) && in01(m.anisotropic) && in01(m.specular) && in01(m.specular_tint) && in01(m.sheen_tint) &&
+              in01(m.subsurface) && in01(m.sheen)))
+            return false;
+    const HostTex& t = s->hdri_tex;
+    const int w = t.width, h = t.height;
+    if (w <= 0 || h <= 0 || t.channels < 1 || t.data.size() < (size_t)w * h * t.channels) return false;
+    const double sum = s->hdri_radiance_sum;
+    if (!(sum > 0.0 && sum <= 1e30)) return false;
+    for (float v : t.data)
+        if (std::signbit(v) || !(v <= 1e6f)) return false;
+    const DevTex dt{w, h, t.channels, t.filter, 0u};
+    std::vector<int> col((size_t)w + 1);
+    for (int x = -1; x < w; x++) col[(size_t)(x + 1)] = erd::hdri_col_entry(dt, x).ix;
+    for (int y = 0; y < h; y++) {
+        const erd::HdriRow r = erd::hdri_row_entry(dt, y);
+        if (!(r.sin_pdf >= 0.0f)) return false;
+        for (int x = 0; x <= w; x++) {
+            float p[3];
+            host_tex_coords(t, col[(size_t)x], r.iy, p);
+            const double share = ((double)p[0] + p[1] + p[2]) / sum;
+            if (!(share >= 1e-30)) return false;
+            if (r.sin_pdf > 0.0f && !(share * w * h / (2.0 * 3.14159265358979323846 * r.sin_pdf) >= 1e-6)) return false;
+        }
+    }
+    return true;
+}
+
 static int begin_descriptor(ErScene* s, uint32_t owned_tiles) {
     const ErGpuBvhDevice& g = s->kept.accel;
     const float lift_bound = g.lift_bound;
@@ -522,6 +552,12 @@
     }
     D.trace_every_query = 0u;
     if (const char* e = getenv("ER_TRACE_EVERY_QUERY")) D.trace_every_query = atoi(e) != 0 ? 1u : 0u;
+    {
+        const char* e = getenv("ER_DEAD_STEP");
+        const bool wanted = !(e && atoi(e) == 0) && D.trace_every_query == 0u;
+        if (wanted && s->dead_scene_ok < 0) s->dead_scene_ok = dead_step_scene_ok(s) ? 1 : 0;
+        D.dead_step = (wanted && s->dead_scene_ok == 1) ? 1u : 0u;
+    }
     D.ext_flags = s->params.flags & (ER_FLAG_POINT_LIGHTS | ER_FLAG_MIS);
     D.lights = s->d_lights.p;
     D.light_count = (uint32_t)s->point_lights.size();
@@ -576,6 +612,7 @@
     const char* who = "er_render_begin";
     s->kept.cus = std::max(1u, info.compute_units);
     s->kept.flags = p->flags;
+    s->dead_scene_ok = -1;
     EventPair ev;
     HIP_TRY(hipEventCreate(&ev.a));
     HIP_TRY(hipEventCreate(&ev.b));
diff --git a/elevenrender_amd/csrc/er_api_edit.cpp b/elevenrender_amd/csrc/er_api_edit.cpp
--- a/elevenrender_amd/csrc/er_api_edit.cpp
+++ b/elevenrender_amd/csrc/er_api_edit.cpp
@@ -390,6 +390,7 @@
         if (e->normals) std::copy(e->normals, e->normals + n9, s->normals.begin());
         if (e->tangents) std::copy(e->tangents, e->tangents + n9, s->tangents.begin());
     }
+    if (what & (ER_EDIT_MATERIALS | ER_EDIT_HDRI)) s->dead_scene_ok = -1;
     if (what & ER_EDIT_MATERIALS) {
         s->materials.swap(W.materials);
         if (e->material_id) std::copy(e->material_id, e->material_id + n, s->material_id.begin());
diff --git a/elevenrender_amd/csrc/er_bounce.inc b/elevenrender_amd/csrc/er_bounce.inc
--- a/elevenrender_amd/csrc/er_bounce.inc
+++ b/elevenrender_amd/csrc/er_bounce.inc
@@ -7,8 +7,15 @@
 #ifndef ER_BOUNCE_KEEP_LAST
 #define ER_BOUNCE_KEEP_LAST false
 #endif
+#ifndef ER_BOUNCE_DEAD
+#define ER_BOUNCE_DEAD true
+#endif
+#ifndef ER_BOUNCE_DEAD_HIT
+#define ER_BOUNCE_DEAD_HIT() ((void)0)
+#endif
 {
     const bool er_skip_equal = (ER_BOUNCE_SKIP_EQUAL) && S.trace_every_query == 0u;
+    const bool er_dead = (ER_BOUNCE_DEAD) && S.dead_step != 0u && reduction.x == 0.0f && reduction.y == 0.0f && reduction.z == 0.0f;
     const int hw = S.hdri_tex.width, hh = S.hdri_tex.height;
     const bool er_mis = EXT && (S.ext_flags & ER_FLAG_MIS) != 0;
 #ifdef ER_BOUNCE_MESH
@@ -36,6 +43,7 @@
         done = true;
     } else {
         c_shaded++;
+        if (er_dead) { ER_BOUNCE_DEAD_HIT(); }
         ER_TP(2);
         HitFull hit;
         full_hit(S, (uint32_t)hslot, ray, hit);
@@ -52,11 +60,27 @@
             F3 N = hd.normal;
             c_hdri++;
             ER_TP(3);
-            int count = er_cdf_search(S.hdri_cdf, hw * hh, S.hdri_guide, S.hdri_buckets, rng_next(rs));
-            const bool hw_pow2 = (hw & (hw - 1)) == 0 && hw > 0 && count >= 0;
-            const int er_cx = hw_pow2 ? (int)((unsigned)count & (unsigned)(hw - 1)) : count % hw;
-            const int er_cy = hw_pow2 ? (int)((unsigned)count >> (31 - __builtin_clz((unsigned)hw))) : count / hw;
-            float tcx = (float)er_cx, tcy = (float)er_cy;
+            const float er_ucdf = rng_next(rs);
+            bool er_short = false;
+            if (er_dead && !(EXT && S.ext_flags != 0u)) {
+                const float er_nv = dot(N, wo);
+                const F3 er_t = hd.tangent, er_b = hd.bitangent;
+                er_short = mat.normal_tex < 0 && (er_nv <= 0.0f || er_nv >= 0.01f) && dot(N, N) <= 4.0f && dot(wo, wo) <= 4.0f &&
+                           dot(er_t, er_t) <= 4.0f && dot(er_b, er_b) <= 16.0f && __builtin_fabsf(dot(N, cross(er_t, er_b))) >= 0.01f &&
+                           hd.metallic >= 0.0f && hd.metallic <= 1.0f && hd.roughness >= 0.0f && hd.roughness <= 1.0f &&
+                           hd.albedo.x >= 0.0f && hd.albedo.x <= 16.0f && hd.albedo.y >= 0.0f && hd.albedo.y <= 16.0f && hd.albedo.z >= 0.0f && hd.albedo.z <= 16.0f &&
+                           ((__builtin_bit_cast(uint32_t, hd.emission.x) | __builtin_bit_cast(uint32_t, hd.emission.y) | __builtin_bit_cast(uint32_t, hd.emission.z)) >> 31) == 0u &&
+                           hd.emission.x <= 1e30f && hd.emission.y <= 1e30f && hd.emission.z <= 1e30f;
+            }
+            int count = -1, er_cx = 0, er_cy = 0;
+            float tcx = 0.0f, tcy = 0.0f;
+            if (!er_short) {
+                count = er_cdf_search(S.hdri_cdf, hw * hh, S.hdri_guide, S.hdri_buckets, er_ucdf);
+                const bool hw_pow2 = (hw & (hw - 1)) == 0 && hw > 0 && count >= 0;
+                er_cx = hw_pow2 ? (int)((unsigned)count & (unsigned)(hw - 1)) : count % hw;
+                er_cy = hw_pow2 ? (int)((unsigned)count >> (31 - __builtin_clz((unsigned)hw))) : count / hw;
+                tcx = (float)er_cx; tcy = (float)er_cy;
+            }
             float d1 = rng_next(rs), d2 = rng_next(rs), d3 = rng_next(rs);
             const bool er_lights = EXT && !er_mesh && (S.ext_flags & ER_FLAG_POINT_LIGHTS) != 0 && S.light_count > 0;
             float er_rl = 0.0f;
@@ -67,6 +91,9 @@
             const bool er_last = !(ER_BOUNCE_KEEP_LAST) && bounce + 1u >= S.max_bounces;
             F3 wibrdf = f3s(0);
             if (!er_last) wibrdf = DisneySample(hd, wo, N, d1, d2, d3);
+            if (er_short) {
+                if (COUNT) c_texels += 2;
+            } else {
             float er_px, er_pz, er_py, er_a, er_sin;
             int er_ix, er_iy;
             if (S.hdri_trig != nullptr && (unsigned)count < (unsigned)(hw * hh)) {
@@ -182,6 +209,7 @@
                     }
                 }
             }
+            }
             ER_TP(5);
             if (!er_last) {
                 float brdfpdf = DisneyPdf(hd, wo, N, wibrdf);
diff --git a/elevenrender_amd/csrc/er_debug.hip b/elevenrender_amd/csrc/er_debug.hip
--- a/elevenrender_amd/csrc/er_debug.hip
+++ b/elevenrender_amd/csrc/er_debug.hip
@@ -115,6 +115,7 @@
 #define ER_BOUNCE_MESH MESH
 #define ER_BOUNCE_SKIP_EQUAL false
 #define ER_BOUNCE_KEEP_LAST true
+#define ER_BOUNCE_DEAD false
 #include "er_bounce.inc"
 #undef ER_BOUNCE_HDRI_QUERY
 #undef ER_BOUNCE_LIGHT_QUERY
@@ -122,6 +123,7 @@
 #undef ER_BOUNCE_MESH
 #undef ER_BOUNCE_SKIP_EQUAL
 #undef ER_BOUNCE_KEEP_LAST
+#undef ER_BOUNCE_DEAD
         (void)pending; (void)lpending; (void)traced;
         if (rec) {
             uint32_t r1 = rs_before;
diff --git a/elevenrender_amd/csrc/er_device.h b/elevenrender_amd/csrc/er_device.h
--- a/elevenrender_amd/csrc/er_device.h
+++ b/elevenrender_amd/csrc/er_device.h
@@ -75,6 +75,7 @@
     uint32_t* tile_cost;
     uint32_t* px_draws;
     const uint32_t* hdri_trig;
+    uint32_t dead_step;
 };
 
 __host__ __device__ __forceinline__ size_t er_pass_index(size_t npx, int pass, size_t idx) {
diff --git a/elevenrender_amd/csrc/er_scene.h b/elevenrender_amd/csrc/er_scene.h
--- a/elevenrender_amd/csrc/er_scene.h
+++ b/elevenrender_amd/csrc/er_scene.h
@@ -136,6 +136,7 @@
     HostTex hdri_tex;
     std::vector<float> hdri_cdf;
     float hdri_radiance_sum = 0;
+    int dead_scene_ok = -1;
     ErCamera camera;
     std::vector<ErPointLight> point_lights;
     uint32_t x_res = 0, y_res = 0;
diff --git a/elevenrender_amd/csrc/er_stream.h b/elevenrender_amd/csrc/er_stream.h
--- a/elevenrender_amd/csrc/er_stream.h
+++ b/elevenrender_amd/csrc/er_stream.h
@@ -53,11 +53,12 @@
     ER_SC_START = 5,
     ER_SC_END = 7,
     ER_SC_SPEC = 23,
-    ER_SC_WORDS = 26,
-    ER_SC_WG_END = 27
+    ER_SC_DEAD = 27,
+    ER_SC_WORDS = 29,
+    ER_SC_WG_END = 29
 };
 constexpr uint32_t ER_STREAM_CTL_LEAD = 1;
-static_assert((ER_STREAM_CTL_LEAD + ER_SC_ITERS) % 2u == 0u && ER_SC_BUSY % 2u == 1u && ER_SC_START % 2u == 1u && ER_SC_END % 2u == 1u && ER_SC_WG_END % 2u == 1u && ER_SC_WG_END >= ER_SC_WORDS,
+static_assert((ER_STREAM_CTL_LEAD + ER_SC_ITERS) % 2u == 0u && ER_SC_BUSY % 2u == 1u && ER_SC_START % 2u == 1u && ER_SC_END % 2u == 1u && ER_SC_DEAD % 2u == 1u && ER_SC_WG_END % 2u == 1u && ER_SC_WG_END >= ER_SC_WORDS,
               "the 64-bit control words are 8-byte aligned");
 constexpr uint32_t er_stream_ctl_words(uint32_t blocks) { return ER_SC_WG_END + 2u * blocks; }
 
diff --git a/elevenrender_amd/csrc/er_stream.hip b/elevenrender_amd/csrc/er_stream.hip
--- a/elevenrender_amd/csrc/er_stream.hip
+++ b/elevenrender_amd/csrc/er_stream.hip
@@ -58,15 +58,18 @@
 #define ST_OCC1 0x1000u
 #define ST_OCC2 0x2000u
 #define ST_HIT2 0x4000u
+#define ST_DEAD 0x8000u
 #define ST_COUNT_MASK 0xFFu
-static_assert((ST_COUNT_MASK & (ST_FIN | ST_ESC | ST_AMB1 | ST_AMB2 | ST_OCC1 | ST_OCC2 | ST_HIT2)) == 0u &&
-                  (ST_FIN ^ ST_ESC ^ ST_AMB1 ^ ST_AMB2 ^ ST_OCC1 ^ ST_OCC2 ^ ST_HIT2) == (ST_FIN | ST_ESC | ST_AMB1 | ST_AMB2 | ST_OCC1 | ST_OCC2 | ST_HIT2) &&
+static_assert((ST_COUNT_MASK & (ST_FIN | ST_ESC | ST_AMB1 | ST_AMB2 | ST_OCC1 | ST_OCC2 | ST_HIT2 | ST_DEAD)) == 0u &&
+                  (ST_FIN ^ ST_ESC ^ ST_AMB1 ^ ST_AMB2 ^ ST_OCC1 ^ ST_OCC2 ^ ST_HIT2 ^ ST_DEAD) == (ST_FIN | ST_ESC | ST_AMB1 | ST_AMB2 | ST_OCC1 | ST_OCC2 | ST_HIT2 | ST_DEAD) &&
+                  (ST_DEAD & (ST_DEAD - 1u)) == 0u &&
                   (ST_FIN & (ST_FIN - 1u)) == 0u && (ST_ESC & (ST_ESC - 1u)) == 0u && (ST_AMB1 & (ST_AMB1 - 1u)) == 0u && (ST_AMB2 & (ST_AMB2 - 1u)) == 0u &&
                   (ST_OCC1 & (ST_OCC1 - 1u)) == 0u && (ST_OCC2 & (ST_OCC2 - 1u)) == 0u && (ST_HIT2 & (ST_HIT2 - 1u)) == 0u,
               "the fields of a slot's s_wait word are single bits that overlap neither each other nor the in-flight count");
 #define ST_RQ_LOG2 (ER_STREAM_SLOTS > 1024u ? 13u : 12u)
 #define ST_SQ_LOG2 (ER_STREAM_SLOTS > 1024u ? 11u : 10u)
 static_assert((1u << ST_SQ_LOG2) >= ER_STREAM_SLOTS, "the shade ring must hold every slot once");
+static_assert((1u << ST_SQ_LOG2) >= ER_STREAM_SLOTS, "the dead ring (s_dq, 1 << ST_SQ_LOG2 cells like s_sq) must hold every slot once");
 static_assert((1u << ST_RQ_LOG2) >= ER_STREAM_SLOTS && (1u << ST_RQ_LOG2) >= 4u * 192u, "ray ring too small");
 static_assert((1u << ST_RQ_LOG2) >= 3u * ER_STREAM_SLOTS, "the ray ring must hold three rays per slot");
 #ifndef ER_STREAM_SPLIT_WAIT
@@ -83,6 +86,12 @@
 #endif
 #ifndef ER_STREAM_TOP_NODES_SPEC_CUT
 #define ER_STREAM_TOP_NODES_SPEC_CUT (ER_STREAM_LDS_HANDOFF ? 40 : 0)
+#endif
+#ifndef ST_DEAD_RING
+#define ST_DEAD_RING(form) ((form) == 0)
+#endif
+#ifndef ER_STREAM_TOP_NODES_DEAD_CUT
+#define ER_STREAM_TOP_NODES_DEAD_CUT 40
 #endif
 #ifndef ST_MAX_TRACERS
 #define ST_MAX_TRACERS 13
@@ -179,6 +188,7 @@
     __device__ __forceinline__ uint32_t& tally_tex(uint32_t i) const { return fld<uint32_t, 240>(i); }
     __device__ __forceinline__ uint32_t& tally_nodes(uint32_t i) const { return fld<uint32_t, 244>(i); }
     __device__ __forceinline__ uint32_t& tally_tris(uint32_t i) const { return fld<uint32_t, 248>(i); }
+    __device__ __forceinline__ uint32_t& tally_dead(uint32_t i) const { return fld<uint32_t, 252>(i); }
 
     __device__ __forceinline__ const float4* ray_pair(uint32_t g, uint32_t kind) const {
         return (const float4*)(base + (size_t)(g * stride + (kind == 0u ? 0u : (kind == 1u ? 32u : 256u))));
@@ -225,7 +235,7 @@
         W.spec_link(g) = 0u;
         W.spec_start(g) = given;
         W.tally_a(g) = 0u; W.tally_rays(g) = 1u;
-        W.tally_tex(g) = 0u; W.tally_nodes(g) = 0u; W.tally_tris(g) = 0u;
+        W.tally_tex(g) = 0u; W.tally_nodes(g) = 0u; W.tally_tris(g) = 0u; W.tally_dead(g) = 0u;
     }
     ER_SP(W.stamp(g) = sp_now(); W.stamp0(g) = W.stamp(g);)
     return rs0;
@@ -268,10 +278,11 @@
     b += 5u * st_lds_pad(ER_RING_WORDS * 4u);
     b += st_lds_pad((1u << ST_RQ_LOG2) * 4u);
     b += 2u * st_lds_pad((1u << ST_SQ_LOG2) * 4u);
+    b += st_lds_pad((ST_DEAD_RING(form) ? (1u << ST_SQ_LOG2) : 1u) * 4u) + st_lds_pad(ER_RING_WORDS * 4u);
     b += st_lds_pad(ER_STREAM_SLOTS * 4u);
     b += st_lds_pad((ER_STREAM_LDS_HANDOFF ? ER_STREAM_SLOTS : 1u) * 4u);
     b += st_lds_pad(ST_PXBITS_WORDS * 4u);
-    b += st_lds_pad(C_WORDS * 4u) + st_lds_pad(4u) + st_lds_pad((spec ? 3u : 1u) * 4u);
+    b += st_lds_pad(C_WORDS * 4u) + st_lds_pad(4u) + st_lds_pad((spec ? 4u : 1u) * 4u);
     b += top_nodes * 5u * 16u;
     b += st_lds_pad(13u * 4u);
     b += ST_MAX_TRACERS * WF_LDS_STACK * 64u * 8u;
@@ -286,7 +297,8 @@
                                                           uint32_t* status, uint32_t n_samples, uint32_t tracers, uint32_t refill_min, uint32_t batch_min, uint32_t fin_min) {
     const DevScene& S = *(const DevScene*)Sp;
     if (threadIdx.x == 0) atomicMin((unsigned long long*)(status + ER_SC_START), (unsigned long long)wall_clock64());
-    constexpr uint32_t RQ_LOG2 = ST_RQ_LOG2, SLOTS = ER_STREAM_SLOTS, TOP_NODES = FORM == 2 ? ER_STREAM_TOP_NODES - ER_STREAM_TOP_NODES_SPEC_CUT : ER_STREAM_TOP_NODES;
+    constexpr uint32_t RQ_LOG2 = ST_RQ_LOG2, SLOTS = ER_STREAM_SLOTS, TOP_NODES = FORM == 2 ? ER_STREAM_TOP_NODES - ER_STREAM_TOP_NODES_SPEC_CUT : (ST_DEAD_RING(FORM) ? ER_STREAM_TOP_NODES - ER_STREAM_TOP_NODES_DEAD_CUT : ER_STREAM_TOP_NODES);
+    constexpr bool DEADQ = ST_DEAD_RING(FORM);
     constexpr bool HANDOFF = ER_STREAM_LDS_HANDOFF != 0;
     constexpr bool EARLY_TAKE = HANDOFF;
     static_assert(st_lds_bytes(FORM, TOP_NODES) <= ST_LDS_LIMIT, "this form of er_stream_kernel needs more LDS than a CU has: fewer top nodes (ER_STREAM_TOP_NODES, _SPEC_CUT)");
@@ -304,13 +316,15 @@
     __shared__ uint32_t s_rq[1u << RQ_LOG2];
     __shared__ uint32_t s_sq[1u << ST_SQ_LOG2];
     __shared__ uint32_t s_fq[1u << ST_SQ_LOG2];
+    __shared__ uint32_t s_dq[DEADQ ? (1u << ST_SQ_LOG2) : 1u];
+    __shared__ __attribute__((aligned(8))) uint32_t s_dq_ctl[ER_RING_WORDS];
     __shared__ uint32_t s_wait[SLOTS];
     __shared__ int s_hit[HANDOFF ? SLOTS : 1u];
     __shared__ uint32_t s_pxbits[ST_PXBITS_WORDS];
     __shared__ __attribute__((aligned(8))) uint32_t s_rq_ctl[ER_RING_WORDS], s_sq_ctl[ER_RING_WORDS], s_px_ctl[ER_RING_WORDS], s_fq_ctl[ER_RING_WORDS];
     __shared__ uint32_t s_ctl[C_WORDS];
     __shared__ uint32_t s_front;
-    __shared__ uint32_t s_spec[SPEC ? 3 : 1];
+    __shared__ uint32_t s_spec[SPEC ? 4 : 1];
     __shared__ float4 s_top[TOP_NODES * 5];
 #ifdef ER_TIME_PROBE
     __shared__ uint32_t s_tp[13];
@@ -329,9 +343,11 @@
     for (uint32_t i = threadIdx.x; i < (1u << ST_SQ_LOG2); i += ST_THREADS) { s_sq[i] = 0; s_fq[i] = 0; }
     for (uint32_t i = threadIdx.x; i < ST_PXBITS_WORDS; i += ST_THREADS) s_pxbits[i] = 0;
     if (SPEC) for (uint32_t i = threadIdx.x; i < (1u << ST_SQ_LOG2); i += ST_THREADS) s_free[i] = 0;
+    if (DEADQ) for (uint32_t i = threadIdx.x; i < (1u << ST_SQ_LOG2); i += ST_THREADS) s_dq[i] = 0;
+    if (threadIdx.x < ER_RING_WORDS) s_dq_ctl[threadIdx.x] = 0;
     if (threadIdx.x < ER_RING_WORDS) { s_rq_ctl[threadIdx.x] = 0; s_sq_ctl[threadIdx.x] = 0; s_px_ctl[threadIdx.x] = 0; s_fq_ctl[threadIdx.x] = 0; }
     if (SPEC && threadIdx.x < ER_RING_WORDS) s_free_ctl[threadIdx.x] = 0;
-    if (SPEC && threadIdx.x < 3u) s_spec[threadIdx.x] = 0;
+    if (SPEC && threadIdx.x < 4u) s_spec[threadIdx.x] = 0;
     if (KEEP && threadIdx.x == 0) s_front = 0xFFFFFFFFu;
     if (threadIdx.x < C_WORDS) s_ctl[threadIdx.x] = 0;
     __syncthreads();
@@ -382,6 +398,7 @@
     unsigned c_rays = 0, c_nodes = 0, c_tris = 0;
     unsigned c_paths = 0, c_bounce = 0, c_shaded = 0, c_texels = 0, c_hdri = 0;
     unsigned c_wsteps = 0, c_busy = 0, c_nl = 0, c_tl = 0;
+    uint32_t dead_w = 0;
 
     {
         __shared__ uint2 s_stack[ST_MAX_TRACERS * WF_LDS_STACK * 64];
@@ -447,7 +464,9 @@
                         last = (fin & ST_COUNT_MASK) == 0u;
                     }
                     const bool escaped = last && (fin & ST_ESC) != 0u && (fin & (ST_AMB1 | ST_AMB2)) == 0u;
-                    st_push<ST_SQ_LOG2>(s_sq, s_sq_ctl, last && !escaped, ls | ((fin & ST_FIN) ? (1u << ST_SLOT_BITS) : 0u), status, ST_ERR_SHADE);
+                    const bool deadq = DEADQ && last && (fin & (ST_DEAD | ST_ESC | ST_FIN)) == ST_DEAD;
+                    st_push<ST_SQ_LOG2>(s_sq, s_sq_ctl, last && !escaped && !deadq, ls | ((fin & ST_FIN) ? (1u << ST_SLOT_BITS) : 0u), status, ST_ERR_SHADE);
+                    if (DEADQ) st_push<ST_SQ_LOG2>(s_dq, s_dq_ctl, deadq, ls, status, ST_ERR_SHADE);
                     st_push<ST_SQ_LOG2>(s_fq, s_fq_ctl, escaped, ls | (1u << ST_SLOT_BITS), status, ST_ERR_SHADE);
                     done = false;
                     ER_MARK("tracer_publish_end");
@@ -473,7 +492,7 @@
                     if (v_ctl[C_DONE]) break;
                     __builtin_amdgcn_s_sleep(ST_IDLE_SLEEP);
                     ER_TRP(6);
-                    const uint32_t pr = er_ring_load(&s_rq_ctl[ER_RING_TAIL]) + er_ring_load(&s_sq_ctl[ER_RING_TAIL]) + er_ring_load(&s_fq_ctl[ER_RING_TAIL]);
+                    const uint32_t pr = er_ring_load(&s_rq_ctl[ER_RING_TAIL]) + er_ring_load(&s_sq_ctl[ER_RING_TAIL]) + er_ring_load(&s_fq_ctl[ER_RING_TAIL]) + (DEADQ ? er_ring_load(&s_dq_ctl[ER_RING_TAIL]) : 0u);
                     if (pr != progress) { progress = pr; idle = 0; }
                     if (++idle > ST_WATCHDOG) {
                         if (lane == 0) { atomicOr(status, 1u); s_ctl[C_DONE] = 1; }
@@ -595,11 +614,14 @@
         while (true) {
             ER_MARK("shader_loop_top");
             const unsigned long long sq_peek = er_ring_peek(s_sq_ctl), fq_peek = er_ring_peek(s_fq_ctl);
-            const uint32_t avail = er_ring_peek_count(sq_peek), favail = er_ring_peek_count(fq_peek);
+            const unsigned long long dq_peek = DEADQ ? er_ring_peek(s_dq_ctl) : 0ull;
+            const uint32_t sq_avail = er_ring_peek_count(sq_peek), favail = er_ring_peek_count(fq_peek), davail = DEADQ ? er_ring_peek_count(dq_peek) : 0u;
+            const bool dead_mode_if = DEADQ && davail > sq_avail;
+            const uint32_t avail = dead_mode_if ? davail : sq_avail;
             if (avail == 0 && favail == 0) {
                 if (v_ctl[C_DONE]) break;
                 __builtin_amdgcn_s_sleep(ST_IDLE_SLEEP);
-                const uint32_t pr = er_ring_load(&s_rq_ctl[ER_RING_TAIL]) + er_ring_load(&s_sq_ctl[ER_RING_TAIL]) + er_ring_load(&s_fq_ctl[ER_RING_TAIL]);
+                const uint32_t pr = er_ring_load(&s_rq_ctl[ER_RING_TAIL]) + er_ring_load(&s_sq_ctl[ER_RING_TAIL]) + er_ring_load(&s_fq_ctl[ER_RING_TAIL]) + (DEADQ ? er_ring_load(&s_dq_ctl[ER_RING_TAIL]) : 0u);
                 if (pr != progress) { progress = pr; idle = 0; }
                 if (SPEC) slack++;
                 if (++idle > ST_WATCHDOG) {
@@ -626,10 +648,11 @@
             ER_MARK("shader_take");
             ER_TPS(0);
             uint32_t hb = 0;
-            const uint32_t granted = fin_mode ? st_take(s_fq_ctl, 64u, hb, fq_peek) : st_take(s_sq_ctl, 64u, hb, sq_peek);
+            const bool dead_mode = DEADQ && !fin_mode && dead_mode_if;
+            const uint32_t granted = fin_mode ? st_take(s_fq_ctl, 64u, hb, fq_peek) : (dead_mode ? st_take(s_dq_ctl, 64u, hb, dq_peek) : st_take(s_sq_ctl, 64u, hb, sq_peek));
             if (granted == 0) continue;
             have = (uint32_t)lane < granted;
-            if (have && !(fin_mode ? er_ring_get(s_fq, ST_SQ_LOG2, hb + (uint32_t)lane, e) : er_ring_get(s_sq, ST_SQ_LOG2, hb + (uint32_t)lane, e))) { have = false; atomicOr(status, ST_ERR_SHADE); }
+            if (have && !(fin_mode ? er_ring_get(s_fq, ST_SQ_LOG2, hb + (uint32_t)lane, e) : (dead_mode ? er_ring_get(s_dq, ST_SQ_LOG2, hb + (uint32_t)lane, e) : er_ring_get(s_sq, ST_SQ_LOG2, hb + (uint32_t)lane, e)))) { have = false; atomicOr(status, ST_ERR_SHADE); }
             __builtin_amdgcn_fence(__ATOMIC_ACQUIRE, "workgroup");
             bool push_closest = false, push_shadow = false, push_light = false, retire = false;
             const uint32_t ls = e & ST_SLOT_MASK;
@@ -675,6 +698,7 @@
                 if (EXT && (packed & ER_SLOT_LPENDING)) ER_SLOT_RESOLVE_QUERY(slot + W.slots, st_verdict<HANDOFF>(W, slot + W.slots, wflags, ST_AMB2, ST_OCC2))
                 bool pending = false, lpending = false;
                 bool done = fin_only;
+                bool dead_hit = false;
                 Ray ray;
                 ray.o = f3s(0);
                 ray.d = f3(0, 0, 1);
@@ -686,8 +710,11 @@
                     c_bounce++;
 #define ER_BOUNCE_FUSE FUSE
 #define ER_BOUNCE_MESH MESH
+#define ER_BOUNCE_DEAD_HIT() dead_hit = true
 #include "er_slot_bounce.inc"
-                }
+#undef ER_BOUNCE_DEAD_HIT
+                }
+                if (!SPEC) dead_w += (uint32_t)__popcll(__ballot(dead_hit));
                 bool alive = true, fin_next = false;
                 if (done && (pending || lpending)) {
                     fin_next = true;
@@ -703,7 +730,8 @@
                 push_light = EXT && lpending;
                 if (alive) {
                     ER_SLOT_STORE(slot, !fin_next);
-                    s_wait[ls] = (push_closest ? 1u : 0u) + (push_shadow ? 1u : 0u) + (push_light ? 1u : 0u) + (fin_next ? ST_FIN : 0u);
+                    const bool dead_next = DEADQ && push_closest && S.dead_step != 0u && !(EXT && S.ext_flags != 0u) && reduction.x == 0.0f && reduction.y == 0.0f && reduction.z == 0.0f;
+                    s_wait[ls] = (push_closest ? 1u : 0u) + (push_shadow ? 1u : 0u) + (push_light ? 1u : 0u) + (fin_next ? ST_FIN : 0u) + (dead_next ? ST_DEAD : 0u);
                 }
                 if (SPEC) {
                     cancel = cancel_w == (uint32_t)SP_INVALID;
@@ -711,6 +739,7 @@
                         const unsigned long long add = (unsigned long long)(t_bounce | (t_shaded << 10) | (t_hdri << 20)) |
                                                        ((unsigned long long)((push_closest ? 1u : 0u) + (push_shadow ? 1u : 0u) + (push_light ? 1u : 0u)) << 32);
                         __hip_atomic_fetch_add((unsigned long long*)&W.tally_a(slot), add, __ATOMIC_RELAXED, __HIP_MEMORY_SCOPE_WORKGROUP);
+                        if (dead_hit) W.tally_dead(slot) += 1u;
                         if (COUNT) {
                             W.tally_tex(slot) += t_texels;
                             atomicAdd(&W.tally_nodes(slot), t_nodes);
@@ -770,6 +799,7 @@
                     const uint32_t ta = W.tally_a(slot);
                     c_bounce += ta & 0x3FFu; c_shaded += (ta >> 10) & 0x3FFu; c_hdri += (ta >> 20) & 0x3FFu;
                     c_rays += W.tally_rays(slot);
+                    { const uint32_t td = W.tally_dead(slot); if (td) atomicAdd(&s_spec[3], td); }
                     if (COUNT) { c_texels += W.tally_tex(slot); c_nodes += W.tally_nodes(slot); c_tris += W.tally_tris(slot); }
                 }
                 if (SPEC && spec_on) {
@@ -979,8 +1009,10 @@
         if (lane == 0) {
             const unsigned q0 = atomicExch(&s_spec[0], 0u), q1 = atomicExch(&s_spec[1], 0u), q2 = atomicExch(&s_spec[2], 0u);
             if (q0 | q1 | q2) { atomicAdd(status + ER_SC_SPEC, q0); atomicAdd(status + ER_SC_SPEC + 1, q1); atomicAdd(status + ER_SC_SPEC + 2, q2); }
+            dead_w = atomicExch(&s_spec[3], 0u);
         }
     }
+    if (lane == 0 && dead_w) atomicAdd((unsigned long long*)(status + ER_SC_DEAD), (unsigned long long)dead_w);
     unsigned t0 = wave_sum(c_paths), t1 = wave_sum(c_bounce), t2 = wave_sum(c_rays), t3 = wave_sum(c_shaded), t4 = wave_sum(c_hdri);
     unsigned t5 = 0, t6 = 0, t7 = 0;
     if (COUNT) { t5 = wave_sum(c_nodes); t6 = wave_sum(c_tris); t7 = wave_sum(c_texels); }
diff --git a/elevenrender_amd/csrc/er_stream_host.cpp b/elevenrender_amd/csrc/er_stream_host.cpp
--- a/elevenrender_amd/csrc/er_stream_host.cpp
+++ b/elevenrender_amd/csrc/er_stream_host.cpp
@@ -165,6 +165,7 @@
     st.ctl = s->d_wf1.p;
     HIP_TRY(hipMemsetAsync(st.ctl, 0, ctl_words * sizeof(uint32_t), s->stream));
     st.spec[0] = st.spec[1] = st.spec[2] = 0;
+    st.dead_steps = 0;
     st.launch_start = st.launch_end = 0; st.wg_end.clear();
     const bool xcd_aware = stream_xcd_aware(owned.size(), st.blocks);
     const uint32_t tiles_x = s->tiles_x();
@@ -276,6 +277,7 @@
     if (st.spec_seen != st.launches) {
         st.spec_seen = st.launches;
         for (int k = 0; k < 3; k++) st.spec[k] += w[ER_SC_SPEC + k];
+        st.dead_steps += (uint64_t)w[ER_SC_DEAD] | ((uint64_t)w[ER_SC_DEAD + 1] << 32);
     }
     if (w[ER_SC_STATUS] != 0)
         return fail(ER_ERR_STATE, std::string(who) + ": the streaming schedule stopped without finishing (watchdog status " + std::to_string(w[ER_SC_STATUS]) + "); the planes are incomplete");
@@ -419,5 +421,7 @@
     out->pixels_per_cu = (uint32_t)((size_t)s->dev.owned_tile_count * 64 / std::max<uint32_t>(1u, st.blocks));
     out->lanes_busy = st.busy; out->launch_ms = st.launch_ms; out->cost_spread = st.cost_spread;
     out->spec_started = st.spec[0]; out->spec_right = st.spec[1]; out->spec_wrong = st.spec[2];
+    out->dead_steps = st.dead_steps;
+    out->dead_rule = s->dev.dead_step;
     out->form = er_stream_launch_form(s->dev.max_bounces, s->tri_count, st.form.waves, st.form.spec, st.form.keep).form;
 }
diff --git a/elevenrender_amd/csrc/er_stream_host.h b/elevenrender_amd/csrc/er_stream_host.h
--- a/elevenrender_amd/csrc/er_stream_host.h
+++ b/elevenrender_amd/csrc/er_stream_host.h
@@ -40,6 +40,7 @@
     double xcd_spread = 0.0;
     double cost_spread = -1.0;
     uint64_t spec[3] = {0, 0, 0};
+    uint64_t dead_steps = 0;
     uint64_t spec_seen = 0;
     uint64_t launches = 0, adapted = 0;
     bool probe_launch = false;
diff --git a/include/eleven_hip_debug.h b/include/eleven_hip_debug.h
--- a/include/eleven_hip_debug.h
+++ b/include/eleven_hip_debug.h
@@ -100,7 +100,8 @@
     double cost_spread;
     uint64_t spec_started, spec_right, spec_wrong;
     uint32_t form;
-    uint32_t reserved;
+    uint32_t dead_rule;
+    uint64_t dead_steps;
 } ErStreamInfo;
 int er_debug_stream_info(struct ErScene* s, ErStreamInfo* out);
 
```

Result: no change. 2118 Msamples/s (-0.1%).
